# av-savchenko/HSE_FaceRec_tf

Measured on AMD Instinct MI355X. Metric: faces/sec embedding-extract (MobileNet-192, bs=256), higher is better.
Workload: dtype f32

## Files before the change

### hse_facerec_tf_amd/_lib.py

```python
from __future__ import annotations

import ctypes
import os
from ctypes import POINTER, c_char_p, c_float, c_int, c_longlong, c_size_t, c_void_p

_HERE = os.path.dirname(os.path.abspath(__file__))
LIB_PATH = os.path.join(_HERE, os.environ.get("HSEFR_LIB", "libhsefr.so"))

OK, ERR_INVALID, ERR_UNSUPPORTED, ERR_HIP, ERR_NOMEM, ERR_SHAPE = 0, -1, -2, -3, -4, -5

_lib = None

_fp = c_void_p
SIGNATURES = {
    "hsefr_version": (c_int, []),
    "hsefr_last_error_string": (c_char_p, []),
    "hsefr_engine_set_graph_batch": (c_int, [c_void_p, c_int]),
    "hsefr_engine_graph_launches": (c_longlong, [c_void_p]),
    "hsefr_engine_create": (c_int, [c_void_p, c_size_t, c_int, POINTER(c_void_p)]),
    "hsefr_plan_validate": (c_int, [c_void_p, c_size_t]),
    "hsefr_plan_describe": (c_int, [c_void_p, c_size_t, c_int, c_char_p, c_size_t]),
    "hsefr_engine_workspace_bytes": (c_size_t, [c_void_p]),
    "hsefr_engine_max_batch": (c_int, [c_void_p]),
    "hsefr_engine_forward": (c_int, [c_void_p, _fp, c_int, _fp, _fp, _fp, c_void_p]),
    "hsefr_engine_buffer": (c_void_p, [c_void_p, c_int]),
    "hsefr_engine_copy_buffer": (c_int, [c_void_p, c_int, _fp, c_size_t, c_void_p]),
    "hsefr_engine_set_profiling": (c_int, [c_void_p, c_int]),
    "hsefr_engine_profiled_calls": (c_longlong, [c_void_p]),
    "hsefr_engine_op_times_ms": (c_int, [c_void_p, c_int, POINTER(c_float), c_int]),
    "hsefr_engine_destroy": (c_int, [c_void_p]),
    "hsefr_conv_c3_bias_act": (c_int, [_fp, _fp, _fp, _fp] + [c_int] * 12 + [c_void_p]),
    "hsefr_dwconv3x3_bn_relu6": (c_int, [_fp, _fp, _fp, _fp, _fp] + [c_int] * 10 + [c_void_p]),
    "hsefr_dwconv3x3_bn_relu6_split": (c_int, [_fp, _fp, _fp, _fp, _fp] + [c_int] * 11 + [c_void_p]),
    "hsefr_pwconv1x1_presplit_gap": (c_int, [_fp, c_void_p, _fp, _fp, _fp, c_longlong, c_int, c_int, c_int, c_int, c_void_p]),
    "hsefr_pwconv1x1_presplit_dw": (c_int, [_fp, c_void_p, _fp, _fp, _fp, _fp, c_longlong] + [c_int] * 7 + [c_void_p]),
    "hsefr_pwconv1x1_presplit": (c_int, [_fp, c_void_p, _fp, _fp, _fp, c_longlong, c_int, c_int, c_int, c_void_p]),
    "hsefr_pwconv1x1_bias_relu6": (c_int, [_fp, _fp, _fp, _fp, c_longlong, c_int, c_int, c_int, c_void_p]),
    "hsefr_stem2_fused": (c_int, [_fp] * 6 + [c_void_p] + [_fp] * 6 + [c_int] * 13 + [c_void_p]),
    "hsefr_stem3_fused": (c_int, [_fp, c_void_p] + [_fp] * 5 + [c_void_p] + [_fp] * 7 + [c_int] * 14 + [c_void_p]),
    "hsefr_stem4_fused": (c_int, [_fp, c_int, c_void_p] + [_fp] * 5 + [c_void_p] + [_fp] * 7 + [c_int] * 6 + [c_void_p]),
    "hsefr_stem5_stream": (c_int, [_fp, c_int, c_void_p] + [_fp] * 5 + [c_void_p] + [_fp] * 7 + [c_int] * 6 + [c_void_p]),
    "hsefr_engine_accepts_u8": (c_int, [c_void_p]),
    "hsefr_engine_forward_u8": (c_int, [c_void_p, _fp, c_int, _fp, _fp, _fp, c_void_p]),
    "hsefr_engine_input_overflow": (c_int, [c_void_p, POINTER(c_int), c_void_p]),
    "hsefr_engine_input_overflow_async": (c_int, [c_void_p, POINTER(c_int), c_void_p]),
    "hsefr_dwpw_f16split": (c_int, [_fp, _fp, _fp, _fp, c_void_p, _fp, _fp, _fp] + [c_int] * 12 + [c_void_p]),
    "hsefr_pwconv1x1_f16split": (c_int, [_fp, c_void_p, _fp, _fp, _fp, c_longlong, c_int, c_int, c_int, c_int, c_void_p]),
    "hsefr_dwpw_fused": (c_int, [_fp] * 7 + [c_int] * 10 + [c_void_p]),
    "hsefr_gap": (c_int, [_fp, _fp, c_int, c_int, c_int, c_void_p]),
    "hsefr_dense": (c_int, [_fp, _fp, _fp, _fp, c_int, c_int, c_int, c_int, c_void_p]),
    "hsefr_softmax": (c_int, [_fp, _fp, c_int, c_int, c_void_p]),
    "hsefr_heads_fused": (c_int, [_fp] * 11 + [c_int] * 3 + [c_void_p]),
    "hsefr_conv_bf16": (c_int, [_fp, _fp, _fp, _fp, _fp, _fp] + [c_int] * 13 + [c_void_p]),
    "hsefr_conv1x1_proj_bf16": (c_int, [_fp] * 9 + [c_int] * 10 + [c_void_p]),
    "hsefr_conv1x1_sres_bf16": (c_int, [_fp] * 6 + [c_int] * 9 + [c_void_p]),
    "hsefr_conv1x1_pair_bf16": (c_int, [_fp] * 14 + [c_longlong] + [c_int] * 6 + [c_void_p]),
    "hsefr_conv1x1_pair_sub2_bf16": (c_int, [_fp] * 14 + [c_int] * 9 + [c_void_p]),
    "hsefr_stem7x7_bf16": (c_int, [_fp, _fp, _fp, _fp, _fp] + [c_int] * 6 + [c_void_p]),
    "hsefr_stem7x7_pool_bf16": (c_int, [_fp, c_void_p, _fp, _fp, c_void_p] + [c_int] * 7 + [c_void_p]),
    "hsefr_maxpool3x3s2_bf16": (c_int, [_fp, _fp] + [c_int] * 8 + [c_void_p]),
    "hsefr_gap_bf16": (c_int, [_fp, _fp, c_int, c_int, c_int, c_void_p]),
    "hsefr_preprocess_pil_u8": (c_int, [_fp, _fp, _fp] + [c_int] * 5 + [_fp, _fp, _fp, c_int, _fp, _fp, _fp, c_int, c_int,
                                        POINTER(ctypes.c_double), c_void_p]),
    "hsefr_preprocess_cv_u8": (c_int, [_fp, _fp] + [c_int] * 5 + [_fp] * 6 + [c_int, POINTER(ctypes.c_double), c_void_p]),
    "hsefr_l2_normalize": (c_int, [_fp, _fp, c_int, c_int, c_void_p]),
    "hsefr_conv2d_direct": (c_int, [_fp] * 5 + [c_int] * 12 + [c_void_p]),
    "hsefr_conv2d_f32": (c_int, [_fp] * 6 + [c_int] * 13 + [c_void_p]),
    "hsefr_conv2d_f32_mfma": (c_int, [_fp] * 6 + [c_int] * 13 + [c_void_p]),
    "hsefr_maxpool_f32": (c_int, [_fp, _fp] + [c_int] * 10 + [c_void_p]),
    "hsefr_mtcnn_pyramid_level": (c_int, [_fp, _fp, c_int, c_int, c_int, c_int, c_void_p]),
    "hsefr_mtcnn_post_capacity": (c_int, []),
    "hsefr_mtcnn_stage1_level": (c_int, [_fp, _fp, c_int, c_int, ctypes.c_double, ctypes.c_float, _fp, _fp, c_void_p]),
    "hsefr_mtcnn_stage1_finish": (c_int, [_fp, _fp, _fp, _fp, c_int, c_int, c_void_p]),
    "hsefr_mtcnn_stage_finish": (c_int, [c_int, _fp, c_int, _fp, _fp, _fp, ctypes.c_float, _fp, _fp, _fp, _fp, c_int, c_int, c_void_p]),
    "hsefr_mtcnn_nms": (c_int, [_fp, c_int, ctypes.c_double, c_int, _fp, _fp, c_void_p]),
    "hsefr_mtcnn_crops": (c_int, [_fp, _fp, _fp, c_int, c_int, c_int, c_int, c_void_p]),
    "hsefr_pairwise_dist": (c_int, [_fp, _fp, c_int, c_int, c_int, _fp, c_void_p]),
    "hsefr_single_linkage": (c_int, [_fp, c_int, c_int, _fp, _fp, _fp, _fp, _fp, _fp, c_void_p]),
    "hsefr_hier_linkage": (c_int, [_fp, c_int, c_int, _fp, _fp, _fp, c_int, _fp, _fp, _fp, _fp, c_void_p]),
    "hsefr_dbscan": (c_int, [_fp, c_int, c_int, _fp, _fp, _fp, ctypes.c_double, c_int, _fp, _fp, c_void_p]),
    "hsefr_rank_order": (c_int, [_fp, c_int, c_int, _fp, _fp, _fp, ctypes.c_double, ctypes.c_double, _fp, POINTER(c_int), c_void_p]),
    "hsefr_rank_order_sweep": (c_int, [_fp, c_int, c_int, _fp, _fp, _fp, POINTER(ctypes.c_double), c_int, _fp, POINTER(c_int), c_void_p]),
    "hsefr_nn1": (c_int, [_fp, _fp, c_int, c_int, c_int, _fp, _fp, c_void_p]),
    "hsefr_knn": (c_int, [_fp, _fp, c_int, c_int, c_int, c_int, _fp, _fp, _fp, _fp, c_void_p]),
    "hsefr_nn1_fallbacks": (c_longlong, []),
}

DEV_SIGNATURES = {
    "hsefr_debug_set": (c_int, [c_char_p, c_int]),
    "hsefr_debug_read_stamps": (c_int, [c_int, c_void_p, ctypes.c_size_t]),
    "hsefr_debug_clock_probe": (c_int, [_fp, c_int, c_int, c_void_p]),
    "hsefr_debug_copy": (c_int, [_fp, _fp, c_size_t, c_void_p]),
    "hsefr_stem_fused": (c_int, [_fp] * 6 + [c_void_p, _fp, _fp, _fp] + [c_int] * 9 + [c_void_p]),
}


class HsefrError(RuntimeError):
    pass

# ... 93 lines not shown
```

### hse_facerec_tf_amd/csrc/common.h

```cpp
#pragma once
#include <hip/hip_runtime.h>
#include <stdarg.h>
#include <stdio.h>

#include "../../include/hsefr.h"
#ifdef HSEFR_DEV
#include "hsefr_dev.h"
#endif

namespace hsefr {

void set_error(const char* fmt, ...);

#define HSEFR_HIP_CHECK(expr)                                                          \
    do {                                                                               \
        hipError_t _e = (expr);                                                        \
        if (_e != hipSuccess) {                                                        \
            ::hsefr::set_error("%s failed: %s (%s:%d)", #expr, hipGetErrorString(_e),  \
                               __FILE__, __LINE__);                                    \
            return HSEFR_ERR_HIP;                                                      \
        }                                                                              \
    } while (0)

#define HSEFR_REQUIRE(cond, code, ...)     \
// ... 190 lines not shown
                             int ph, int pw, int pool_pad_t, int pool_pad_l, hipStream_t s, const void* wfrag = nullptr);
bool stem7s_stream_supported(long long n, int h, int w, int ph, int pw);
int launch_stem7s_stream(const float* x, const void* wt, const float* scale, const float* shift, void* y, int n, int h, int w, int ph, int pw,
                         int pool_pad_t, int pool_pad_l, hipStream_t s, const void* wfrag = nullptr);
constexpr size_t STEM7S_WFRAG_BYTES = 4 * 7 * 64 * 16;
int stem7s_reorder_weights(const void* wt, void* wfrag, hipStream_t s);
int launch_maxpool3x3s2_bf16(const void* x, void* y, int n, int h, int w, int c, int oh, int ow, int pad_t, int pad_l,
                             hipStream_t s);
int launch_gap_bf16(const void* x, float* y, int n, int hw, int c, hipStream_t s);

int launch_pil_resize(const unsigned char* in, unsigned char* tmp, float* out, int n, int H, int W, int oh, int ow, const int* xmin,
                      const int* xcnt, const int* xcoef, int xk, const int* ymin, const int* ycnt, const int* ycoef, int yk,
                      int mode, const double* mean, hipStream_t s);
int launch_cv_resize(const unsigned char* in, float* out, int n, int H, int W, int oh, int ow, const int* x0, const int* x1,
                     const int* wx1, const int* y0, const int* y1, const int* wy1, int mode, const double* mean, hipStream_t s);

int launch_area_level(const unsigned char* src, float* dst, int sh, int sw, int dh, int dw, hipStream_t s);
int launch_area_crops(const unsigned char* src, const int* boxes, float* dst, int sh, int sw, int n, int size, hipStream_t s);
int launch_pairwise_dist(const float* x, const float* y, int n, int m, int d, float* out, hipStream_t s);
struct DistSource {
    const float* x;
    int n, d;
    const float* born;
    const float* year;
    const double* dense;
};
int launch_single_linkage(const DistSource& src, int* edge_a, int* edge_b, double* edge_h, hipStream_t s);
int launch_dbscan(const DistSource& src, double eps, int min_samples, int* labels, unsigned char* core, hipStream_t s);
int launch_rank_order(const DistSource& src, const double* thresholds, int pairs, int* labels, int* iterations, hipStream_t s);
int launch_hier_linkage(const DistSource& src, int method, int* merge_a, int* merge_b, double* merge_h, int* merge_round, hipStream_t s);

bool dwpw_fused_supported(int c, int cout, int stride, int act_dw, int act_pw);
int launch_dwpw_fused(const float* x, const float* wd, const float* dscale, const float* dshift, const float* wp_t,
                      const float* pshift, float* y, int n, int h, int w, int c, int stride, int pad_t, int pad_l, int oh,
                      int ow, int cout, int act_dw, int act_pw, hipStream_t s);

int launch_conv2d_direct(const float* x, const float* w, const float* bias, const float* alpha, float* y, int n, int h, int wd, int c,
                         int oh, int ow, int cout, int kh, int kw, int stride, int pad_t, int pad_l, hipStream_t s);
int launch_conv_f32_mfma(const float* x, const float* w, const float* scale, const float* shift, const float* res, float* y, int n, int h,
                         int wd, int c, int oh, int ow, int cout, int kh, int kw, int stride, int pad_t, int pad_l, int act, hipStream_t s,
                         int res_stride = 0, int res_h = 0, int res_w = 0);
bool conv_f32_mfma_supported(int c, int cout);
int launch_conv2d_f32(const float* x, const float* w, const float* scale, const float* shift, const float* res, float* y, int n, int h,
                      int wd, int c, int oh, int ow, int cout, int kh, int kw, int stride, int pad_t, int pad_l, int act, hipStream_t s);
int launch_maxpool_f32(const float* x, float* y, int n, int h, int w, int c, int oh, int ow, int k, int stride, int pad_t, int pad_l,
                       hipStream_t s);

int launch_dwpw_f16s(const float* x, const float* wd, const float* dscale, const float* dshift, const void* wsplit,
                     const float* descale, const float* pshift, float* y, int n, int h, int w, int c, int stride, int pad_t,
                     int pad_l, int oh, int ow, int cout, int a_log2, int act, hipStream_t s);
bool dwpw_f16s_supported(int c, int cout, int stride);
bool dwpw_s2_covered(int c, int cout, int stride);
bool dwpw_s2_off();
int launch_stem_fused(const float* x, const float* cw, const float* cshift, const float* wd, const float* dscale,
                      const float* dshift, const void* wsplit, const float* descale, const float* pshift, float* y, int n,
                      int h, int w, int cpad_t, int cpad_l, int oh, int ow, int a_log2, int act, hipStream_t s);
int launch_stem2_fused(const float* x, const float* cw, const float* cshift, const float* wd1, const float* d1scale,
                       const float* d1shift, const void* wsplit, const float* descale, const float* pshift, const float* wd2,
                       const float* d2scale, const float* d2shift, float* y, int n, int h, int w, int cpad_t, int cpad_l,
                       int h1, int w1, int pad_t2, int pad_l2, int oh2, int ow2, int a_log2, int act, hipStream_t s);
int launch_stem3_fused(const float* x, const void* cw_split, const float* cdescale, const float* cshift, const float* wd1,
                       const float* d1scale, const float* d1shift, const void* wsplit, const float* descale, const float* pshift,
                       const float* wd2, const float* d2scale, const float* d2shift, float* y, int* overflow, int n, int h, int w,
                       int cpad_t, int cpad_l, int h1, int w1, int pad_t2, int pad_l2, int oh2, int ow2, int in_log2, int a_log2,
                       int act, hipStream_t s);
bool stem3_fused_supported(int cin, int c1, int c2, int conv_stride, int dw1_stride, int dw2_stride, int kh, int kw);
int launch_stem4_fused(const void* x, int x_is_u8, const void* cw4, const float* cdescale, const float* cshift, const float* wd1,
                       const float* d1scale, const float* d1shift, const void* wsplit, const float* descale, const float* pshift,
                       const float* wd2, const float* d2scale, const float* d2shift, float* y, int* overflow, int n, int h, int w,
                       int in_log2, int a_log2, int act, hipStream_t s);
bool stem4_fused_supported(int cin, int c1, int c2, int conv_stride, int dw1_stride, int dw2_stride, int kh, int kw, int h, int w);
int launch_stem5_stream(const void* x, int x_is_u8, const void* cw4, const float* cdescale, const float* cshift, const float* wd1,
                        const float* d1scale, const float* d1shift, const void* wsplit, const float* descale, const float* pshift,
                        const float* wd2, const float* d2scale, const float* d2shift, float* y, int* overflow, int n, int h, int w,
                        int in_log2, int a_log2, int act, hipStream_t s);
bool stem5_stream_supported(int cin, int c1, int c2, int conv_stride, int dw1_stride, int dw2_stride, int kh, int kw, int h, int w);
bool stem2_fused_supported(int cin, int c1, int c2, int conv_stride, int dw1_stride, int dw2_stride, int kh, int kw);
bool stem_fused_supported(int cin, int cmid, int cout, int conv_stride, int dw_stride, int kh, int kw);
int read_pws_stamps(void* host_out, size_t bytes);
int read_stem_stamps(void* host_out, size_t bytes);
#ifdef HSEFR_STEM_STAMPS
unsigned long long* stamp_buffer(hipStream_t s);
#define STEM_STAMP(i) do { const unsigned long long _t = __builtin_amdgcn_s_memtime(); st[i] += _t - tprev; tprev = _t; } while (0)
#define STEM_STAMP_DECL unsigned long long st[8] = {0, 0, 0, 0, 0, 0, 0, 0}; unsigned long long tprev = __builtin_amdgcn_s_memtime(); \
    const unsigned long long tstart = tprev; unsigned npatch = 0
#define STEM_STAMP_COUNT ++npatch
#define STEM_STAMP_FLUSH(buf, lane, wave) do { if ((lane) == 0 && (buf) && blockIdx.x < 512) { unsigned long long* o = (buf) + (blockIdx.x * 4 + (wave)) * 10; \
    for (int i_ = 0; i_ < 8; ++i_) o[i_] = st[i_]; o[8] = __builtin_amdgcn_s_memtime() - tstart; o[9] = npatch; } } while (0)
#else
#define STEM_STAMP(i) do { } while (0)
#define STEM_STAMP_DECL do { } while (0)
#define STEM_STAMP_COUNT do { } while (0)
#define STEM_STAMP_FLUSH(buf, lane, wave) do { } while (0)
#endif
#ifdef HSEFR_DEV
void set_stem4_grid(int v);
void set_stem5_grid(int v);
void set_stem5_segs(int v);
void set_c11(int v);
void set_c11_tile(int v);
void set_c11_bres(int v);
void set_c11_adv(int v);
int read_c11_stamps(void* host_out, size_t bytes);
void set_dwpw_s2_off(int v);
void set_dwpws_tw(int v);
void set_dwpws_bn(int v);
void set_pw_tile(int v);
void set_pws_tile(int v);
void set_ps_mb(int v);
void set_ps_grid(int v);
void set_psdw_mode(int v);
void set_cd_rb(int v);
void set_w3_off(int v);
void set_w2_off(int v);
void set_w4_off(int v);
void set_w4_bres(int v);
void set_pair_off(int v);
void set_stem7s(int v);
void set_pair_ablate(int v);
void set_pair_nt(int v);
void set_nn1_y_mb(int v);
int read_w4_stamps(void* host_out, size_t bytes);
int read_s7_stamps(void* host_out, size_t bytes);
int read_w2_stamps(void* host_out, size_t bytes);
int read_w3_stamps(void* host_out, size_t bytes);
int read_cd_stamps(void* host_out, size_t bytes);
void set_cd_off(int v);
int read_ps_stamps(void* host_out, size_t bytes);
void set_pw_ablate(int v);
void set_pw_dma(int v);
void set_dw_th(int v);
void set_dw_variant(int v);
void set_dw_look(int v);
void set_dw_look2(int v);
void set_copy_variant(int v);
void set_clock_mode(int v);
void set_c3_impl(int v);
int launch_clock_probe(unsigned long long* out, int blocks, int iters, hipStream_t s);
int launch_copy(const void* src, void* dst, size_t bytes, hipStream_t s);
#endif

}
```

### hse_facerec_tf_amd/csrc/dwpw_f16s.hip

```cpp
#include <type_traits>

#include "common.h"

namespace hsefr {

namespace {

typedef float f32x4 __attribute__((ext_vector_type(4)));
typedef float f32x16 __attribute__((ext_vector_type(16)));
typedef _Float16 f16x4 __attribute__((ext_vector_type(4)));
typedef _Float16 f16x8 __attribute__((ext_vector_type(8)));

struct DwPwSParams {
    const float4* x;
    const float4* wd;
    const float4* dscale;
    const float4* dshift;
    const float* wsplit;
    const float* descale;
    const float* pshift;
    float* y;
    int H, W, C4, KT, OH, OW, Cout, pad_t, pad_l, tiles_w, tiles_h, tiles_n;
    unsigned total;
    float a_scale;
    int reverse;
    int nimg;
    unsigned m_n, m_w, m_h;
    unsigned long long* stamps;
};

constexpr int ROWB = 128;
__device__ __forceinline__ int swzb(int row, int chunk) { return row * ROWB + 16 * (chunk ^ ((row >> 1) & 7) ^ ((row & 1) << 2)); }
__device__ __forceinline__ float4 fma4(float4 a, float4 b, float4 c) {
    return make_float4(fmaf(a.x, b.x, c.x), fmaf(a.y, b.y, c.y), fmaf(a.z, b.z, c.z), fmaf(a.w, b.w, c.w));
}
__device__ __forceinline__ float relu6(float v) { return fminf(fmaxf(v, 0.f), 6.f); }
__device__ __forceinline__ unsigned fastdiv(unsigned x, unsigned m) { return m ? __umulhi(x, m) : x; }

template <int STRIDE, int TW, int BN, int OCC, int ACT>
__global__ __launch_bounds__(256, OCC) void dwpw_f16s_kernel(DwPwSParams p) {
    constexpr int TH = 128 / TW;
    constexpr int U = TW * 8;
    constexpr int RG = 256 / U;
    constexpr int RPT = TH / RG;
    static_assert(RPT == 4, "patch shapes 8x16 and 16x8");
    constexpr int WN = BN / 2, NI = WN / 32, BP = BN / 32;
    __shared__ __attribute__((aligned(16))) unsigned char As[128 * ROWB];
    __shared__ __attribute__((aligned(16))) unsigned char Bs[BN * ROWB];

    const int tid = threadIdx.x;
    const int lane = tid & 63, wave = tid >> 6;
    const int wm = wave >> 1, wn = wave & 1;
    const int li = lane & 31, lh = lane >> 5;
    const int srow = tid >> 3, skq = tid & 7;
    const int u = tid % U, tw = u >> 3, c4l = u & 7;
    const int row0 = (tid / U) * RPT;
    const int arow = wm * 64 + li, brow = wn * WN + li;

    for (unsigned t = blockIdx.x; t < p.total; t += gridDim.x) {
        const unsigned lt = xcd_remap_dir(t, p.total, p.reverse);
        const int n0 = (lt % p.tiles_n) * BN;
        const unsigned pt = lt / p.tiles_n;
        const int ow0 = (pt % p.tiles_w) * TW;
        const int oh0 = ((pt / p.tiles_w) % p.tiles_h) * TH;
        const int n = pt / (p.tiles_w * p.tiles_h);

        const int ow = min(ow0 + tw, p.OW - 1);
        const int iw0 = ow * STRIDE - p.pad_l;
        const float ml = iw0 >= 0 ? 1.f : 0.f, mm = (iw0 + 1 >= 0 && iw0 + 1 < p.W) ? 1.f : 0.f, mr = iw0 + 2 < p.W ? 1.f : 0.f;
        const int cl = max(iw0, 0) * p.C4, cm = min(max(iw0 + 1, 0), p.W - 1) * p.C4, cr = min(iw0 + 2, p.W - 1) * p.C4;
        const float4* ximg = p.x + (size_t)n * p.H * p.W * p.C4;
        const int ih0 = (oh0 + row0) * STRIDE - p.pad_t;
        const float* bsrc = p.wsplit + (size_t)(n0 + srow) * p.KT * 32 + 4 * skq;

        f32x16 acc[2][NI];
#pragma unroll
        for (int mi = 0; mi < 2; ++mi)
#pragma unroll
            for (int ni = 0; ni < NI; ++ni)
#pragma unroll
                for (int r = 0; r < 16; ++r) acc[mi][ni][r] = 0.f;
// ... 71 lines not shown
                f16x8 ah[2], al[2], bh[NI], bl[NI];
#pragma unroll
                for (int mi = 0; mi < 2; ++mi) {
                    ah[mi] = *(const f16x8*)(&As[swzb(arow + mi * 32, 2 * s + lh)]);
                    al[mi] = *(const f16x8*)(&As[swzb(arow + mi * 32, 4 + 2 * s + lh)]);
                }
#pragma unroll
                for (int ni = 0; ni < NI; ++ni) {
                    bh[ni] = *(const f16x8*)(&Bs[swzb(brow + ni * 32, 2 * s + lh)]);
                    bl[ni] = *(const f16x8*)(&Bs[swzb(brow + ni * 32, 4 + 2 * s + lh)]);
                }
#pragma unroll
                for (int mi = 0; mi < 2; ++mi)
#pragma unroll
                    for (int ni = 0; ni < NI; ++ni) {
                        acc[mi][ni] = __builtin_amdgcn_mfma_f32_32x32x16_f16(al[mi], bh[ni], acc[mi][ni], 0, 0, 0);
                        acc[mi][ni] = __builtin_amdgcn_mfma_f32_32x32x16_f16(ah[mi], bl[ni], acc[mi][ni], 0, 0, 0);
                        acc[mi][ni] = __builtin_amdgcn_mfma_f32_32x32x16_f16(ah[mi], bh[ni], acc[mi][ni], 0, 0, 0);
                    }
            }
        }
        const bool full = oh0 + TH <= p.OH && ow0 + TW <= p.OW;
        float* ybase = p.y + ((size_t)n * p.OH * p.OW) * p.Cout;
#pragma unroll
        for (int ni = 0; ni < NI; ++ni) {
            const int col = n0 + wn * WN + ni * 32 + li;
            const float ds = p.descale[col], sh = p.pshift[col];
#pragma unroll
            for (int mi = 0; mi < 2; ++mi) {
                const int Rb = wm * 64 + mi * 32 + 4 * lh;
                if (full) {
#pragma unroll
                    for (int r = 0; r < 16; ++r) {
                        const int R = Rb + (r & 3) + 8 * (r >> 2);
                        ybase[((size_t)(oh0 + R / TW) * p.OW + ow0 + (R % TW)) * p.Cout + col] = apply_act<ACT>(fmaf(acc[mi][ni][r], ds, sh));
                    }
                } else {
#pragma unroll
                    for (int r = 0; r < 16; ++r) {
                        const int R = Rb + (r & 3) + 8 * (r >> 2);
                        const int oh = oh0 + R / TW, owc = ow0 + (R % TW);
                        if (oh < p.OH && owc < p.OW)
                            ybase[((size_t)oh * p.OW + owc) * p.Cout + col] = apply_act<ACT>(fmaf(acc[mi][ni][r], ds, sh));
                    }
                }
            }
        }
    }
}

constexpr int HALO_B = 192 * 128;
constexpr int CMAX2 = 512;

template <int TW, int BN, int HS, int ACT>
__global__ __launch_bounds__(256 + 64 * (BN == 256 ? 8 : 4), BN == 256 ? 1 : 2) void dwpw3_f16s_kernel(DwPwSParams p) {
    constexpr int NCW = BN == 256 ? 8 : 4;
    constexpr int CWN = NCW / 2;
    constexpr int NTHR = 256 + 64 * NCW;
    constexpr int TH = 128 / TW, HC = TW + 2;
    constexpr int WCAP = 256;
    constexpr int B_ST = BN * ROWB;
    constexpr int B_OFF = HS * HALO_B, A_OFF = B_OFF + 2 * B_ST, W_OFF = A_OFF + 2 * 128 * ROWB, E_OFF = W_OFF + 11 * WCAP * 4;
    constexpr int WN = BN / CWN, NI = WN / 32;
    constexpr int BPW = BN / 8 / NCW;
    static_assert(BPW == 4 && NI == 2, "a consumer's slice of the weight stage is its 4 KB epilogue scratch");
    constexpr bool HALO_BY_CONSUMER = false;
    constexpr int HPW = 24 / (HALO_BY_CONSUMER ? NCW : 4);
    static_assert(E_OFF + 2 * CMAX2 * 4 <= 160 * 1024, "LDS budget");
    __shared__ __attribute__((aligned(1024))) unsigned char smem[E_OFF + 2 * CMAX2 * 4];

    const int tid = threadIdx.x;
    const int lane = tid & 63;
    const int wave = __builtin_amdgcn_readfirstlane(tid >> 6);
    const int C = p.C4 * 4, KT = p.KT;
    {
        float4* wl = (float4*)(smem + W_OFF);
        for (int i = tid; i < 9 * p.C4; i += NTHR) wl[i] = p.wd[i];
        for (int i = tid; i < p.C4; i += NTHR) { wl[9 * p.C4 + i] = p.dscale[i]; wl[10 * p.C4 + i] = p.dshift[i]; }
        float* el = (float*)(smem + E_OFF);
        for (int i = tid; i < p.Cout; i += NTHR) { el[i] = p.descale[i]; el[CMAX2 + i] = p.pshift[i]; }
    }
    const __amdgpu_buffer_rsrc_t rx = make_rsrc(p.x, (long long)p.nimg * p.H * p.W * C * 4);
    const __amdgpu_buffer_rsrc_t rw = make_rsrc(p.wsplit, (long long)p.Cout * C * 4);
    const __amdgpu_buffer_rsrc_t ry = make_rsrc(p.y, (long long)p.nimg * p.OH * p.OW * p.Cout * 4);
    const unsigned OOB = 0xFFFFFFF0u;
    const unsigned nitem = (p.total - blockIdx.x + gridDim.x - 1) / gridDim.x;
    const int nsteps = (int)(nitem * KT);
    struct Item { int n, oh0, ow0, n0; };
    auto decode = [&](unsigned i) {
        const unsigned lt = xcd_remap_dir(blockIdx.x + (i < nitem ? i : nitem - 1) * gridDim.x, p.total, p.reverse);
        Item it;
        const unsigned pt = fastdiv(lt, p.m_n);
        it.n0 = (lt - pt * p.tiles_n) * BN;
        const unsigned pr = fastdiv(pt, p.m_w);
        it.ow0 = (pt - pr * p.tiles_w) * TW;
        it.n = fastdiv(pr, p.m_h);
        it.oh0 = (pr - it.n * p.tiles_h) * TH;
        return it;
    };
    const unsigned lds0 = (unsigned)(unsigned long long)(__attribute__((address_space(3))) unsigned char*)smem;
    auto piece = [&](const __amdgpu_buffer_rsrc_t& r, unsigned lds_addr, unsigned voff, unsigned soff) {
        asm volatile("s_mov_b32 m0, %0\n\ts_nop 0\n\tbuffer_load_dwordx4 %1, %2, %3 offen lds" ::"s"(__builtin_amdgcn_readfirstlane(lds_addr)), "v"(voff),
                     "s"(r), "s"(__builtin_amdgcn_readfirstlane(soff))
                     : "memory", "m0");
    };
    const int hw = HALO_BY_CONSUMER ? wave - 4 : wave & 3;
    unsigned hv[HPW];
    unsigned pf_i = 0;
    int pf_kc = 0, pf_step = 0;
    auto setup_halo = [&](unsigned i) {
        const Item it = decode(i);
#pragma unroll
        for (int j = 0; j < HPW; ++j) {
            const int q = (hw * HPW + j) * 8 + (lane >> 3);
            const int hr = q / HC, hc = q - hr * HC;
            const int ih = it.oh0 - p.pad_t + hr, iw = it.ow0 - p.pad_l + hc;
            const bool ok = q < (TH + 2) * HC && ih >= 0 && ih < p.H && iw >= 0 && iw < p.W;
            hv[j] = ok ? ((unsigned)((it.n * p.H + ih) * p.W + iw) * (unsigned)C + 4u * (lane & 7)) * 4u : OOB;
        }
    };
    auto halo_dma = [&]() {
        const unsigned base = lds0 + (pf_step % HS) * HALO_B;
        const unsigned so = (unsigned)pf_kc * 128u;
#pragma unroll
        for (int j = 0; j < HPW; ++j) piece(rx, base + (hw * HPW + j) * 1024, hv[j], so);
        ++pf_step;
        if (++pf_kc == KT) {
            pf_kc = 0;
            setup_halo(++pf_i);
        }
    };
    STEM_STAMP_DECL;

    if (wave < 4) {
        const int quad = tid & 7, col = (tid >> 3) % TW, r0 = 4 * (tid / (8 * TW));
        const unsigned char* hsrc0 = smem + ((r0 * HC + col) * 128 + quad * 16);
        if (!HALO_BY_CONSUMER) {
            setup_halo(0);
#pragma unroll
            for (int i = 0; i < HS - 1; ++i)
                if (i < nsteps) halo_dma();
        }
        asm volatile("s_waitcnt vmcnt(0)" ::: "memory");
        __syncthreads();
        int dkc = 0;
        for (int g = -1; g < nsteps; ++g) {
            const bool issued = !HALO_BY_CONSUMER && pf_step < nsteps;
            if (issued) halo_dma();
            STEM_STAMP(1);
            if (g + 1 < nsteps) {
                const f32x4* wl = (const f32x4*)(smem + W_OFF) + dkc * 8 + quad;
                f32x4 wk[9];
#pragma unroll
                for (int i = 0; i < 9; ++i) wk[i] = wl[i * p.C4];
                const f32x4 dsc = wl[9 * p.C4], dsh = wl[10 * p.C4];
                const unsigned char* hs = hsrc0 + ((g + 1) % HS) * HALO_B;
                unsigned char* At = smem + A_OFF + ((g + 1) & 1) * (128 * ROWB);
                f32x4 h[6][3];
#pragma unroll
                for (int a = 0; a < 6; ++a)
#pragma unroll
                    for (int b = 0; b < 3; ++b) h[a][b] = *(const f32x4*)(hs + (a * HC + b) * 128);
                auto row_sum = [&](int a, int b) {
                    f32x4 t = h[a][0] * wk[b];
                    t = __builtin_elementwise_fma(h[a][1], wk[b + 1], t);
                    return __builtin_elementwise_fma(h[a][2], wk[b + 2], t);
                };
#pragma unroll
                for (int j = 0; j < 4; ++j) {
                    const f32x4 sa = row_sum(j, 0), sb = row_sum(j + 1, 3), sc = row_sum(j + 2, 6);
                    const f32x4 sacc = (sa + sb) + sc;
                    const f32x4 o = __builtin_elementwise_fma(sacc, dsc, dsh);
                    f32x4 v;
#pragma unroll
                    for (int e = 0; e < 4; ++e) v[e] = relu6(o[e]);
                    v = v * p.a_scale;
                    const f16x4 hi = __builtin_convertvector(v, f16x4);
                    const f16x4 lo = __builtin_convertvector(v - __builtin_convertvector(hi, f32x4), f16x4);
                    const int R = (r0 + j) * TW + col;
                    *(f16x4*)(At + swzb(R, quad >> 1) + 8 * (quad & 1)) = hi;
                    *(f16x4*)(At + swzb(R, 4 + (quad >> 1)) + 8 * (quad & 1)) = lo;
                }
                if (++dkc == KT) { dkc = 0; STEM_STAMP_COUNT; }
            }
            STEM_STAMP(2);
            if (HS >= 3 && issued) asm volatile("s_waitcnt vmcnt(%0)" ::"n"(HPW) : "memory");
            else asm volatile("s_waitcnt vmcnt(0)" ::: "memory");
            STEM_STAMP(0);
            __syncthreads();
            STEM_STAMP(3);
        }
        STEM_STAMP_FLUSH(p.stamps, lane, wave);
    } else {
        const int cw = wave - 4, wm = cw / CWN, wn = cw % CWN;
        const int li = lane & 31, lh = lane >> 5;
        const int arow = wm * 64 + li, brow = wn * WN + li;
        const int erow = lane >> 3, ech = lane & 7;
        unsigned bv[BPW];
        unsigned pb_i = 0;
        int pb_kc = 0, pb_step = 0;
        auto setup_b = [&](unsigned i) {
            const Item it = decode(i);
#pragma unroll
            for (int j = 0; j < BPW; ++j) {
                const int r = (cw * BPW + j) * 8 + (lane >> 3);
                bv[j] = ((unsigned)(it.n0 + r) * (unsigned)C + 4u * ((lane & 7) ^ ((r >> 1) & 7) ^ ((r & 1) << 2))) * 4u;
            }
        };
        auto b_dma = [&]() {
            const unsigned base = lds0 + B_OFF + (pb_step & 1) * B_ST;
            const unsigned so = (unsigned)pb_kc * 128u;
#pragma unroll
            for (int j = 0; j < BPW; ++j) piece(rw, base + (cw * BPW + j) * 1024, bv[j], so);
            ++pb_step;
            if (++pb_kc == KT) {
                pb_kc = 0;
                setup_b(++pb_i);
            }
        };
        f32x16 acc[2][NI];
        auto zero_acc = [&]() {
#pragma unroll
            for (int mi = 0; mi < 2; ++mi)
#pragma unroll
                for (int ni = 0; ni < NI; ++ni)
#pragma unroll
                    for (int r = 0; r < 16; ++r) acc[mi][ni][r] = 0.f;
        };
        auto epilogue = [&](const Item& cur, int stage) {
            unsigned char* scr = smem + B_OFF + stage * B_ST + cw * (BPW * 1024);
            const float* el = (const float*)(smem + E_OFF);
            unsigned sv[2][4];
#pragma unroll
            for (int mi = 0; mi < 2; ++mi)
#pragma unroll
                for (int i = 0; i < 4; ++i) {
                    const int R = wm * 64 + mi * 32 + erow + 8 * i;
                    const int oh = cur.oh0 + R / TW, ow = cur.ow0 + R % TW;
                    sv[mi][i] = (oh < p.OH && ow < p.OW)
                                    ? ((unsigned)((cur.n * p.OH + oh) * p.OW + ow) * (unsigned)p.Cout + (unsigned)(cur.n0 + wn * WN + 4 * ech)) * 4u
                                    : OOB;
                }
#pragma unroll
            for (int ni = 0; ni < NI; ++ni) {
                const int nl = cur.n0 + wn * WN + ni * 32 + 4 * ech;
                const f32x4 ds = *(const f32x4*)(el + nl), sh = *(const f32x4*)(el + CMAX2 + nl);
// ... 44 lines not shown
                zero_acc();
                cur = decode(++ci);
                pending = false;
                STEM_STAMP_COUNT;
            }
            STEM_STAMP(5);
            if (pb_step < nsteps) b_dma();
            const bool halo_issued = HALO_BY_CONSUMER && pf_step < nsteps;
            if (halo_issued) halo_dma();
            STEM_STAMP(1);
            if (g >= 0) {
                const unsigned char* As = smem + A_OFF + (g & 1) * (128 * ROWB);
                const unsigned char* Bs = smem + B_OFF + (g & 1) * B_ST;
#pragma unroll
                for (int s = 0; s < 2; ++s) {
                    f16x8 ah[2], al[2], bh[NI], bl[NI];
#pragma unroll
                    for (int mi = 0; mi < 2; ++mi) {
                        ah[mi] = *(const f16x8*)(As + swzb(arow + mi * 32, 2 * s + lh));
                        al[mi] = *(const f16x8*)(As + swzb(arow + mi * 32, 4 + 2 * s + lh));
                    }
#pragma unroll
                    for (int ni = 0; ni < NI; ++ni) {
                        bh[ni] = *(const f16x8*)(Bs + swzb(brow + ni * 32, 2 * s + lh));
                        bl[ni] = *(const f16x8*)(Bs + swzb(brow + ni * 32, 4 + 2 * s + lh));
                    }
#pragma unroll
                    for (int mi = 0; mi < 2; ++mi)
#pragma unroll
                        for (int ni = 0; ni < NI; ++ni) {
                            acc[mi][ni] = __builtin_amdgcn_mfma_f32_32x32x16_f16(bh[ni], al[mi], acc[mi][ni], 0, 0, 0);
                            acc[mi][ni] = __builtin_amdgcn_mfma_f32_32x32x16_f16(bl[ni], ah[mi], acc[mi][ni], 0, 0, 0);
                            acc[mi][ni] = __builtin_amdgcn_mfma_f32_32x32x16_f16(bh[ni], ah[mi], acc[mi][ni], 0, 0, 0);
                        }
                }
                if (++ckc == KT) { ckc = 0; pending = true; }
            }
            STEM_STAMP(4);
            if (HS >= 3 && halo_issued) asm volatile("s_waitcnt vmcnt(%0)" ::"n"(HPW) : "memory");
            else asm volatile("s_waitcnt vmcnt(0)" ::: "memory");
            STEM_STAMP(0);
            __syncthreads();
            STEM_STAMP(3);
        }
        if (pending) { epilogue(cur, (nsteps - 1) & 1); STEM_STAMP_COUNT; }
#ifdef HSEFR_STEM_STAMPS
        if (lane == 0 && p.stamps && blockIdx.x < 256 && cw < 4) {
            unsigned long long* o = p.stamps + ((blockIdx.x + 256) * 4 + cw) * 10;
            for (int i_ = 0; i_ < 8; ++i_) o[i_] = st[i_];
            o[8] = __builtin_amdgcn_s_memtime() - tstart;
            o[9] = npatch;
        }
#endif
    }
}

constexpr unsigned S2_GRID = 256;
constexpr int S2_C = 128, S2_COUT = 256, S2_KT = S2_C / 32, S2_T = 8, S2_M = S2_T * S2_T;
constexpr int S2_B_ST = S2_COUT * ROWB;
constexpr int S2_A_ST = S2_M * ROWB;
constexpr int S2_SCR = 16 * ROWB;
constexpr int S2_A_OFF = S2_KT * S2_B_ST, S2_S_OFF = S2_A_OFF + 2 * S2_A_ST, S2_W_OFF = S2_S_OFF + 4 * S2_SCR;
constexpr int S2_E_OFF = S2_W_OFF + 11 * S2_C * 4, S2_LDS = S2_E_OFF + 2 * S2_COUT * 4;
static_assert(S2_LDS <= 160 * 1024, "LDS budget");

template <int ACT>
__global__ __launch_bounds__(512, 1) void dwpws2_f16s_kernel(DwPwSParams p) {
    __shared__ __attribute__((aligned(1024))) unsigned char smem[S2_LDS];
    const int tid = threadIdx.x;
    const int lane = tid & 63;
    const int wave = __builtin_amdgcn_readfirstlane(tid >> 6);
    const __amdgpu_buffer_rsrc_t rx = make_rsrc(p.x, (long long)p.nimg * p.H * p.W * S2_C * 4);
    const __amdgpu_buffer_rsrc_t rw = make_rsrc(p.wsplit, (long long)S2_COUT * S2_C * 4);
    const __amdgpu_buffer_rsrc_t ry = make_rsrc(p.y, (long long)p.nimg * p.OH * p.OW * S2_COUT * 4);
    const unsigned OOB = 0xFFFFFFF0u;
    {
        const unsigned lds0 = (unsigned)(unsigned long long)(__attribute__((address_space(3))) unsigned char*)smem;
#pragma unroll
        for (int j = 0; j < 16; ++j) {
            const int pc = wave * 16 + j;
            const int r = (pc & 31) * 8 + (lane >> 3);
            const unsigned v = ((unsigned)r * (unsigned)S2_C + 4u * ((lane & 7) ^ ((r >> 1) & 7) ^ ((r & 1) << 2))) * 4u;
            asm volatile("s_mov_b32 m0, %0\n\ts_nop 0\n\tbuffer_load_dwordx4 %1, %2, %3 offen lds" ::"s"(__builtin_amdgcn_readfirstlane(lds0 + pc * 1024)),
                         "v"(v), "s"(rw), "s"(__builtin_amdgcn_readfirstlane((unsigned)(pc >> 5) * 128u))
                         : "memory", "m0");
        }
        float4* wl = (float4*)(smem + S2_W_OFF);
        for (int i = tid; i < 11 * (S2_C / 4); i += 512)
            wl[i] = i < 9 * (S2_C / 4) ? p.wd[i] : (i < 10 * (S2_C / 4) ? p.dscale[i - 9 * (S2_C / 4)] : p.dshift[i - 10 * (S2_C / 4)]);
        float* el = (float*)(smem + S2_E_OFF);
        for (int i = tid; i < S2_COUT; i += 512) { el[i] = p.descale[i]; el[S2_COUT + i] = p.pshift[i]; }
        asm volatile("s_waitcnt vmcnt(0)" ::: "memory");
    }
    const unsigned nitem = (p.total - blockIdx.x + gridDim.x - 1) / gridDim.x;
    const int nsteps = (int)(nitem * S2_KT);
    struct Item { int n, oh0, ow0; };
    auto decode = [&](unsigned i) {
        const unsigned lt = xcd_remap_dir(blockIdx.x + (i < nitem ? i : nitem - 1) * gridDim.x, p.total, p.reverse);
        Item it;
        const unsigned pr = fastdiv(lt, p.m_w);
        it.ow0 = (lt - pr * p.tiles_w) * S2_T;
        it.n = fastdiv(pr, p.m_h);
        it.oh0 = (pr - it.n * p.tiles_h) * S2_T;
        return it;
    };
    typedef std::integral_constant<int, 0> S0;
    typedef std::integral_constant<int, 1> S1;
// ... 144 lines not shown
                            const f32x4 z = __builtin_elementwise_fma(rv[i], ds, sh);
                            f32x4 o;
#pragma unroll
                            for (int e = 0; e < 4; ++e) o[e] = apply_act<ACT>(z[e]);
                            bstore16_welded(o, ry, sv[mi][hb][i], __builtin_amdgcn_readfirstlane((unsigned)(ni * 32) * 4u));
                        }
                    }
            }
        };
        zero_acc();
        Item cur = decode(0);
        unsigned ci = 0;
        int ckc = 0;
        bool pending = false;
        for (int g = 0; g < nsteps; ++g) {
            if (pending) {
                epilogue(cur);
                zero_acc();
                cur = decode(++ci);
                pending = false;
            }
            __syncthreads();
            const unsigned char* As = smem + S2_A_OFF + (g & 1) * S2_A_ST;
            const unsigned char* Bs = smem + ckc * S2_B_ST;
#pragma unroll
            for (int s = 0; s < 2; ++s) {
                f16x8 ah[2], al[2], bh[2], bl[2];
#pragma unroll
                for (int mi = 0; mi < 2; ++mi) {
                    ah[mi] = *(const f16x8*)(As + swzb(li + mi * 32, 2 * s + lh));
                    al[mi] = *(const f16x8*)(As + swzb(li + mi * 32, 4 + 2 * s + lh));
                }
#pragma unroll
                for (int ni = 0; ni < 2; ++ni) {
                    bh[ni] = *(const f16x8*)(Bs + swzb(brow + ni * 32, 2 * s + lh));
                    bl[ni] = *(const f16x8*)(Bs + swzb(brow + ni * 32, 4 + 2 * s + lh));
                }
#pragma unroll
                for (int mi = 0; mi < 2; ++mi)
#pragma unroll
                    for (int ni = 0; ni < 2; ++ni) {
                        acc[mi][ni] = __builtin_amdgcn_mfma_f32_32x32x16_f16(bh[ni], al[mi], acc[mi][ni], 0, 0, 0);
                        acc[mi][ni] = __builtin_amdgcn_mfma_f32_32x32x16_f16(bl[ni], ah[mi], acc[mi][ni], 0, 0, 0);
                        acc[mi][ni] = __builtin_amdgcn_mfma_f32_32x32x16_f16(bh[ni], ah[mi], acc[mi][ni], 0, 0, 0);
                    }
            }
            if (++ckc == S2_KT) { ckc = 0; pending = true; }
        }
        epilogue(cur);
    }
}

HSEFR_KNOB(g_s2_off, 0);
HSEFR_KNOB(g_tw, 0);
HSEFR_KNOB(g_bn, 0);

template <int STRIDE, int TW, int BN, int OCC>
int launch_t(DwPwSParams& p, int n, int act, hipStream_t s) {
    constexpr int TH = 128 / TW;
    p.tiles_w = (p.OW + TW - 1) / TW;
    p.tiles_h = (p.OH + TH - 1) / TH;
    p.tiles_n = p.Cout / BN;
    const long long total = (long long)n * p.tiles_w * p.tiles_h * p.tiles_n;
    HSEFR_REQUIRE(total < (1ll << 31), HSEFR_ERR_UNSUPPORTED, "dwpw_f16split: grid too large");
    p.total = (unsigned)total;
    const unsigned cap = 256u * OCC;
    const unsigned g = p.total < cap ? p.total : cap;
#define HSEFR_DWPWS(A) HSEFR_LAUNCH((dwpw_f16s_kernel<STRIDE, TW, BN, OCC, A>), dim3(g), dim3(256), 0, s, p)
    if (act == HSEFR_ACT_RELU6) HSEFR_DWPWS(HSEFR_ACT_RELU6);
    else if (act == HSEFR_ACT_RELU) HSEFR_DWPWS(HSEFR_ACT_RELU);
    else if (act == HSEFR_ACT_NONE) HSEFR_DWPWS(HSEFR_ACT_NONE);
    else { set_error("dwpw_f16split: act %d", act); return HSEFR_ERR_UNSUPPORTED; }
#undef HSEFR_DWPWS
    return launch_status("dwpw_f16split");
}

template <int STRIDE, int TW>
int launch_bn(DwPwSParams& p, int n, int bn, int act, hipStream_t s) {
    if (bn == 64) return launch_t<STRIDE, TW, 64, 2>(p, n, act, s);
#ifdef HSEFR_DEV
    if (bn == 256) return launch_t<STRIDE, TW, 256, 2>(p, n, act, s);
#endif
    return launch_t<STRIDE, TW, 128, 2>(p, n, act, s);
}

template <int TW, int BN, int HS>
int launch_v3(DwPwSParams& p, int n, int act, hipStream_t s) {
    constexpr int TH = 128 / TW;
    p.tiles_w = (p.OW + TW - 1) / TW;
    p.tiles_h = (p.OH + TH - 1) / TH;
    p.tiles_n = p.Cout / BN;
    const long long total = (long long)n * p.tiles_w * p.tiles_h * p.tiles_n;
    HSEFR_REQUIRE(total < (1ll << 31) / 16, HSEFR_ERR_UNSUPPORTED, "dwpw_f16split: grid too large");
    p.total = (unsigned)total;
    auto magic = [](unsigned d) { return d == 1 ? 0u : (unsigned)((0x100000000ull + d - 1) / d); };
    p.m_n = magic(p.tiles_n); p.m_w = magic(p.tiles_w); p.m_h = magic(p.tiles_h);
    HSEFR_REQUIRE(total * (long long)(p.tiles_n > p.tiles_w ? (p.tiles_n > p.tiles_h ? p.tiles_n : p.tiles_h) : (p.tiles_w > p.tiles_h ? p.tiles_w : p.tiles_h)) < (1ll << 32),
                  HSEFR_ERR_UNSUPPORTED, "dwpw_f16split: grid too large for the quotient multipliers");
    const unsigned g = p.total < 256u ? p.total : 256u;
#define HSEFR_DWPW3(A) HSEFR_LAUNCH((dwpw3_f16s_kernel<TW, BN, HS, A>), dim3(g), dim3(256 + 64 * (BN == 256 ? 8 : 4)), 0, s, p)
    if (act == HSEFR_ACT_RELU6) HSEFR_DWPW3(HSEFR_ACT_RELU6);
    else if (act == HSEFR_ACT_RELU) HSEFR_DWPW3(HSEFR_ACT_RELU);
    else if (act == HSEFR_ACT_NONE) HSEFR_DWPW3(HSEFR_ACT_NONE);
    else { set_error("dwpw_f16split: act %d", act); return HSEFR_ERR_UNSUPPORTED; }
#undef HSEFR_DWPW3
    return launch_status("dwpw_f16split");
}

int launch_s2(DwPwSParams& p, int n, int act, hipStream_t s) {
    p.tiles_w = (p.OW + S2_T - 1) / S2_T;
    p.tiles_h = (p.OH + S2_T - 1) / S2_T;
    p.tiles_n = 1;
    const long long total = (long long)n * p.tiles_w * p.tiles_h;
    HSEFR_REQUIRE(total < (1ll << 31) / 16, HSEFR_ERR_UNSUPPORTED, "dwpw_f16split: grid too large");
    p.total = (unsigned)total;
    auto magic = [](unsigned d) { return d == 1 ? 0u : (unsigned)((0x100000000ull + d - 1) / d); };
    p.m_n = 0; p.m_w = magic(p.tiles_w); p.m_h = magic(p.tiles_h);
    HSEFR_REQUIRE(total * (long long)(p.tiles_w > p.tiles_h ? p.tiles_w : p.tiles_h) < (1ll << 32), HSEFR_ERR_UNSUPPORTED,
                  "dwpw_f16split: grid too large for the quotient multipliers");
    const unsigned g = p.total < S2_GRID ? p.total : S2_GRID;
#define HSEFR_DWPWS2(A) HSEFR_LAUNCH((dwpws2_f16s_kernel<A>), dim3(g), dim3(512), 0, s, p)
    if (act == HSEFR_ACT_RELU6) HSEFR_DWPWS2(HSEFR_ACT_RELU6);
    else if (act == HSEFR_ACT_RELU) HSEFR_DWPWS2(HSEFR_ACT_RELU);
    else if (act == HSEFR_ACT_NONE) HSEFR_DWPWS2(HSEFR_ACT_NONE);
    else { set_error("dwpw_f16split: act %d", act); return HSEFR_ERR_UNSUPPORTED; }
#undef HSEFR_DWPWS2
    return launch_status("dwpw_f16split");
}

}

#ifdef HSEFR_DEV
void set_dwpw_s2_off(int v) { g_s2_off = v; }
void set_dwpws_tw(int v) { g_tw = v; }
void set_dwpws_bn(int v) { g_bn = v; }
#endif

bool dwpw_s2_off() { return g_s2_off != 0; }

bool dwpw_s2_covered(int c, int cout, int stride) { return stride == 2 && c == S2_C && cout == S2_COUT; }

bool dwpw_f16s_supported(int c, int cout, int stride) {
    return c > 0 && c % 32 == 0 && cout > 0 && cout % 64 == 0 && (stride == 1 || stride == 2);
}

int launch_dwpw_f16s(const float* x, const float* wd, const float* dscale, const float* dshift, const void* wsplit,
                     const float* descale, const float* pshift, float* y, int n, int h, int w, int c, int stride, int pad_t,
                     int pad_l, int oh, int ow, int cout, int a_log2, int act, hipStream_t s) {
    HSEFR_REQUIRE(dwpw_f16s_supported(c, cout, stride), HSEFR_ERR_UNSUPPORTED,
                  "dwpw_f16split: c=%d cout=%d stride=%d not covered (c %% 32, cout %% 64, stride 1|2)", c, cout, stride);
    HSEFR_REQUIRE(n >= 0 && h > 0 && w > 0 && oh > 0 && ow > 0, HSEFR_ERR_INVALID, "dwpw_f16split: bad shape");
    HSEFR_REQUIRE(a_log2 > 0 && a_log2 <= 12, HSEFR_ERR_INVALID, "dwpw_f16split: a_log2=%d (the depthwise result is in [0,6]: 1..12)", a_log2);
    if (n == 0) return HSEFR_OK;
    DwPwSParams p;
    p.x = (const float4*)x; p.wd = (const float4*)wd; p.dscale = (const float4*)dscale; p.dshift = (const float4*)dshift;
    p.wsplit = (const float*)wsplit; p.descale = descale; p.pshift = pshift; p.y = y;
    p.H = h; p.W = w; p.C4 = c / 4; p.KT = c / 32; p.OH = oh; p.OW = ow; p.Cout = cout; p.pad_t = pad_t; p.pad_l = pad_l;
    p.a_scale = ldexpf(1.f, a_log2);
    p.reverse = sweep_reverse();
    p.nimg = n;
    p.stamps = nullptr;
#ifdef HSEFR_STEM_STAMPS
    p.stamps = stamp_buffer(s);
#endif
    const long long in_bytes = (long long)n * h * w * c * 4, out_bytes = (long long)n * oh * ow * cout * 4;
    if (stride == 1 && c <= 256 && cout <= CMAX2 && cout % 128 == 0 && in_bytes < (1ll << 32) - 16 && out_bytes < (1ll << 32) - 16) {
        auto padded = [&](int tw) { const int th = 128 / tw; return (long long)((ow + tw - 1) / tw * tw) * ((oh + th - 1) / th * th); };
        int tw = padded(16) <= padded(8) ? 16 : 8;
        if (g_tw == 8 || g_tw == 16) tw = g_tw;
        int bn = cout % 256 == 0 ? 256 : 128;
        if ((g_bn == 128 || g_bn == 256) && cout % g_bn == 0) bn = g_bn;
        if (bn == 256) return tw == 16 ? launch_v3<16, 256, 2>(p, n, act, s) : launch_v3<8, 256, 2>(p, n, act, s);
        return tw == 16 ? launch_v3<16, 128, 3>(p, n, act, s) : launch_v3<8, 128, 3>(p, n, act, s);
    }
    if (dwpw_s2_covered(c, cout, stride) && !g_s2_off && in_bytes < (1ll << 32) - 16 && out_bytes < (1ll << 32) - 16)
        return launch_s2(p, n, act, s);
    int bn = cout % 128 == 0 ? 128 : 64;
    if (g_bn && cout % g_bn == 0) bn = g_bn;
    int tw = (ow % 16 == 0 || ow % 8 != 0) ? 16 : 8;
    if (ow <= 8) tw = 8;
    if (g_tw == 8 || g_tw == 16) tw = g_tw;
    if (stride == 1) return tw == 16 ? launch_bn<1, 16>(p, n, bn, act, s) : launch_bn<1, 8>(p, n, bn, act, s);
    return tw == 16 ? launch_bn<2, 16>(p, n, bn, act, s) : launch_bn<2, 8>(p, n, bn, act, s);
}

}
```

### hse_facerec_tf_amd/csrc/engine.hip

```cpp
#include <math.h>
#include <string.h>

#include <cxxabi.h>
#include <dlfcn.h>
#include <elf.h>

#include <map>
#include <new>
#include <string>
#include <vector>

#include "common.h"

namespace hsefr {

static thread_local char g_err[512] = "";

void set_error(const char* fmt, ...) {
    va_list ap;
    va_start(ap, fmt);
    vsnprintf(g_err, sizeof(g_err), fmt, ap);
    va_end(ap);
}

// ... 212 lines not shown
                HSEFR_REQUIRE(o.w_off != HSEFR_NO_OFFSET && o.scale_off != HSEFR_NO_OFFSET && o.shift_off != HSEFR_NO_OFFSET &&
                                  o.aux > 0 && o.aux <= 24,
                              HSEFR_ERR_INVALID, "plan op %u: split-f16 pointwise needs split rows, descale, shift and a_log2 in (0, 24]", i);
                break;
            case HSEFR_OP_STEM3_F16S: {
                const StemAux a = stem_aux(o.aux);
                HSEFR_REQUIRE(stem3_fused_supported(o.cin, 32, o.cout, o.stride, 1, 2, o.kh, stem_kw(o.kw).k) && a.a_log2 > 0 && a.a_log2 <= 12 &&
                                  a.in_log2 >= -8 && a.in_log2 <= 14 &&
                                  o.w_off != HSEFR_NO_OFFSET && o.w2_off != HSEFR_NO_OFFSET && o.shift2_off != HSEFR_NO_OFFSET &&
                                  o.w_off + HSEFR_STEM_PACK_STEM3_END * 4 <= h.blob_bytes && o.w2_off + 64 * 128 <= h.blob_bytes &&
                                  o.shift2_off + 128 * 4 <= h.blob_bytes && o.in_buf == HSEFR_BUF_INPUT,
                              HSEFR_ERR_UNSUPPORTED, "plan op %u: bounded fused stem cin=%d cout=%d stride=%d not covered", i, o.cin, o.cout, o.stride);
                break;
            }
            case HSEFR_OP_STEM2_F16S:
                HSEFR_REQUIRE(stem2_fused_supported(o.cin, 32, o.cout, o.stride, 1, 2, o.kh, stem_kw(o.kw).k) && o.aux > 0 && o.aux <= 12 &&
                                  o.w_off != HSEFR_NO_OFFSET && o.w2_off != HSEFR_NO_OFFSET && o.shift2_off != HSEFR_NO_OFFSET &&
                                  o.w_off + HSEFR_STEM_PACK_STEM2_END * 4 <= h.blob_bytes && o.in_buf == HSEFR_BUF_INPUT,
                              HSEFR_ERR_UNSUPPORTED, "plan op %u: fused stem+dw2 cin=%d cout=%d stride=%d not covered", i, o.cin, o.cout, o.stride);
                break;
            case HSEFR_OP_STEM_F16S:
#ifndef HSEFR_DEV
                set_error("plan op %u: HSEFR_OP_STEM_F16S (round 1's fused stem) runs on development builds of the library only", i);
                return HSEFR_ERR_UNSUPPORTED;
#else
                HSEFR_REQUIRE(stem_fused_supported(o.cin, 32, o.cout, o.stride, 1, o.kh, o.kw) && o.aux > 0 && o.aux <= 12 &&
                                  o.w_off != HSEFR_NO_OFFSET && o.w2_off != HSEFR_NO_OFFSET && o.shift2_off != HSEFR_NO_OFFSET &&
                                  o.w_off + HSEFR_STEM_PACK_DW2 * 4 <= h.blob_bytes && o.in_buf == HSEFR_BUF_INPUT,
                              HSEFR_ERR_UNSUPPORTED, "plan op %u: fused stem cin=%d cout=%d stride=%d not covered", i, o.cin, o.cout, o.stride);
                break;
#endif
            case HSEFR_OP_DWPW_F16S:
                if (!need(o.w_off, 9 * ci * 4, "depthwise kernel") || !need(o.scale_off, ci * 4, "scale") || !need(o.shift_off, ci * 4, "shift") ||
                    !need(o.w2_off, ci * co * 4, "split rows") || !need(o.shift2_off, 2 * co * 4, "descale | shift"))
                    return HSEFR_ERR_INVALID;
                HSEFR_REQUIRE(dwpw_f16s_supported(o.cin, o.cout, o.stride) && o.aux > 0 && o.aux <= 12 &&
                                  o.w_off != HSEFR_NO_OFFSET && o.scale_off != HSEFR_NO_OFFSET && o.shift_off != HSEFR_NO_OFFSET &&
                                  o.w2_off != HSEFR_NO_OFFSET && o.shift2_off != HSEFR_NO_OFFSET,
                              HSEFR_ERR_UNSUPPORTED, "plan op %u: split-f16 fused block cin=%d cout=%d stride=%d a_log2=%d not covered",
                              i, o.cin, o.cout, o.stride, o.aux);
                break;
            case HSEFR_OP_DWPW_F32:
                if (!need(o.w_off, 9 * ci * 4, "depthwise kernel") || !need(o.scale_off, ci * 4, "scale") || !need(o.shift_off, ci * 4, "shift") ||
                    !need(o.w2_off, ci * co * 4, "pointwise kernel") || !need(o.shift2_off, co * 4, "pointwise shift"))
                    return HSEFR_ERR_INVALID;
                HSEFR_REQUIRE(dwpw_fused_supported(o.cin, o.cout, o.stride, HSEFR_ACT_RELU6, (int)o.act), HSEFR_ERR_UNSUPPORTED,
                              "plan op %u: fused depthwise-pointwise block cin=%d cout=%d not covered", i, o.cin, o.cout);
                break;
            default:
                set_error("plan op %u: unknown kind %u", i, o.kind);
                return HSEFR_ERR_UNSUPPORTED;
        }
    }
    for (uint32_t i = 0; i < h.n_ops; ++i) {
        const hsefr_plan_op& o = ops[i];
        HSEFR_REQUIRE((o.flags & ~(HSEFR_OPF_PAIR_NEXT | HSEFR_OPF_HEADS | HSEFR_OPF_OUT_SUB2 | HSEFR_OPF_DWPW_NEXT)) == 0, HSEFR_ERR_INVALID,
                      "plan op %u: unknown flags 0x%x", i, o.flags);
        HSEFR_REQUIRE(!(o.flags & HSEFR_OPF_OUT_SUB2) || (o.flags & HSEFR_OPF_PAIR_NEXT), HSEFR_ERR_INVALID, "plan op %u: OUT_SUB2 without PAIR_NEXT", i);
        if (o.flags & HSEFR_OPF_PAIR_NEXT) {
            HSEFR_REQUIRE(i + 1 < h.n_ops, HSEFR_ERR_INVALID, "plan op %u: PAIR_NEXT on the last op", i);
            const hsefr_plan_op& b = ops[i + 1];
            const bool proj = o.w2_off != HSEFR_NO_OFFSET;
            const Geometry g = geometry(o.aux);
            const int c2 = proj ? g.c2 : 0;
            const bool sub2 = (o.flags & HSEFR_OPF_OUT_SUB2) != 0;
            HSEFR_REQUIRE(o.kind == HSEFR_OP_CONV_BF16 && b.kind == HSEFR_OP_CONV_BF16 && o.kh == 1 && o.kw == 1 && o.stride == 1 && o.pad_t == 0 &&
                              o.pad_l == 0 && (sub2 ? (o.oh == (o.h + 1) / 2 && o.ow == (o.w + 1) / 2 && o.h > 1 && o.w > 1) : (o.oh == o.h && o.ow == o.w)) &&
                              b.kh == 1 && b.kw == 1 && b.stride == 1 && b.pad_t == 0 && b.pad_l == 0 &&
                              b.h == o.h && b.w == o.w && b.oh == b.h && b.ow == b.w && b.cin == o.cout && b.in_buf == o.out_buf &&
                              b.res_buf == HSEFR_BUF_NONE && b.w2_off == HSEFR_NO_OFFSET && b.flags == 0 && o.res_buf >= 0 &&
                              (!proj || (g.stride2 == 1 && g.h2 == o.h && g.w2 == o.w)),
                          HSEFR_ERR_INVALID, "plan op %u: PAIR_NEXT needs two 1x1 stride-1 bf16 convolutions at the same pixels, the first with a residual "
                          "or a same-pixel projected shortcut, the second reading the first", i);
            HSEFR_REQUIRE(b.out_buf != o.in_buf && b.out_buf != o.res_buf && b.out_buf != o.out_buf, HSEFR_ERR_INVALID,
                          "plan op %u: PAIR_NEXT: the second output (buffer %d) aliases an operand of the first", i, b.out_buf);
            HSEFR_REQUIRE(conv1x1_pair_bf16_shape_supported(o.cin, o.cout, b.cout, c2), HSEFR_ERR_UNSUPPORTED,
                          "plan op %u: PAIR_NEXT %d -> %d -> %d (projection from %d) not covered", i, o.cin, o.cout, b.cout, c2);
        }
        if (o.flags & HSEFR_OPF_DWPW_NEXT) {
            HSEFR_REQUIRE(o.flags == HSEFR_OPF_DWPW_NEXT && i + 1 < h.n_ops, HSEFR_ERR_INVALID, "plan op %u: DWPW_NEXT on the last op or beside another flag", i);
            const hsefr_plan_op& b = ops[i + 1];
            HSEFR_REQUIRE(o.kind == HSEFR_OP_DWCONV3X3 && o.stride == 2 && o.act == HSEFR_ACT_RELU6 && o.aux == 0 && o.cout == o.cin &&
                              b.kind == HSEFR_OP_PWCONV_F16S && b.in_buf == o.out_buf && b.flags == 0 && b.h == o.oh && b.w == o.ow && b.oh == b.h &&
                              b.ow == b.w && b.cin == o.cin && b.aux > 0 && b.aux <= 12,
                          HSEFR_ERR_INVALID, "plan op %u: DWPW_NEXT needs a stride-2 depthwise 3x3 with ReLU6 and fp32 output, and behind it a split-f16 "
                          "pointwise op without flags that reads it at the same pixels (a_log2 in [1, 12])", i);
            HSEFR_REQUIRE(dwpw_s2_covered(o.cin, b.cout, o.stride), HSEFR_ERR_INVALID, "plan op %u: DWPW_NEXT %d -> %d channels not covered (128 -> 256)", i,
                          o.cin, b.cout);
            HSEFR_REQUIRE(b.out_buf != o.out_buf, HSEFR_ERR_INVALID, "plan op %u: DWPW_NEXT: the second output (buffer %d) aliases the depthwise tensor", i,
                          b.out_buf);
            HSEFR_REQUIRE(b.out_buf != o.in_buf || (uint64_t)bufs[o.in_buf].elems_per_image * bufs[o.in_buf].elem_bytes ==
                                                       (uint64_t)bufs[o.out_buf].elems_per_image * bufs[o.out_buf].elem_bytes,
                          HSEFR_ERR_INVALID, "plan op %u: DWPW_NEXT: buffers %d and %d exchange roles and must have one size", i, o.in_buf, o.out_buf);
            for (uint32_t k = i + 2; k < h.n_ops; ++k) {
                HSEFR_REQUIRE(ops[k].in_buf != o.out_buf && ops[k].res_buf != o.out_buf, HSEFR_ERR_INVALID,
                              "plan op %u: DWPW_NEXT: op %u also reads the depthwise tensor (buffer %d)", i, k, o.out_buf);
                if (ops[k].out_buf == o.out_buf) break;
            }
            for (int sl = 0; sl < HSEFR_N_OUTPUT_SLOTS; ++sl)
                HSEFR_REQUIRE(h.out_buffer[sl] != o.out_buf && (b.out_buf != o.in_buf || h.out_buffer[sl] != o.in_buf), HSEFR_ERR_INVALID,
                              "plan op %u: DWPW_NEXT: the depthwise tensor (or the buffer it exchanges roles with) is output slot %d", i, sl);
        }
        if (o.flags & HSEFR_OPF_HEADS) {
            HSEFR_REQUIRE(i + 3 < h.n_ops, HSEFR_ERR_INVALID, "plan op %u: HEADS needs three ops behind it", i);
            const hsefr_plan_op &a = ops[i + 1], &sm = ops[i + 2], &g = ops[i + 3];
            HSEFR_REQUIRE(o.kind == HSEFR_OP_DENSE && o.act == HSEFR_ACT_RELU && o.cout == 256 && o.cin > 0 && o.cin % 256 == 0 && o.cin <= 2048 &&
                              o.shift_off != HSEFR_NO_OFFSET && a.kind == HSEFR_OP_DENSE && a.act == HSEFR_ACT_NONE && a.cin == 256 && a.cout >= 1 &&
                              a.cout <= 128 && a.in_buf == o.out_buf && a.shift_off != HSEFR_NO_OFFSET && sm.kind == HSEFR_OP_SOFTMAX &&
                              sm.in_buf == a.out_buf && sm.cout == a.cout && g.kind == HSEFR_OP_DENSE && g.act == HSEFR_ACT_SIGMOID && g.cin == 256 &&
                              g.cout == 1 && g.in_buf == o.out_buf && g.shift_off != HSEFR_NO_OFFSET && a.flags == 0 && sm.flags == 0 && g.flags == 0,
                          HSEFR_ERR_INVALID, "plan op %u: HEADS needs DENSE k -> 256 + ReLU, DENSE 256 -> a (<= 128) + bias, SOFTMAX, DENSE 256 -> 1 + sigmoid", i);
            const int outs[4] = {o.out_buf, a.out_buf, sm.out_buf, g.out_buf};
            for (int x = 0; x < 4; ++x) {
                HSEFR_REQUIRE(outs[x] != o.in_buf, HSEFR_ERR_INVALID, "plan op %u: HEADS: an output aliases the pooled features", i);
                for (int y = x + 1; y < 4; ++y)
                    HSEFR_REQUIRE(outs[x] != outs[y], HSEFR_ERR_INVALID, "plan op %u: HEADS: two of the four tensors share buffer %d", i, outs[x]);
            }
        }
    }
    for (int s = 0; s < HSEFR_N_OUTPUT_SLOTS; ++s) {
        HSEFR_REQUIRE(h.out_buffer[s] == HSEFR_BUF_NONE || (h.out_buffer[s] >= 0 && h.out_buffer[s] < (int)h.n_buffers),
                      HSEFR_ERR_INVALID, "plan: output slot %d names buffer %d", s, h.out_buffer[s]);
        if (h.out_buffer[s] == HSEFR_BUF_NONE) continue;
        const int b = h.out_buffer[s];
        uint32_t producers = 0;
        for (uint32_t i = 0; i < h.n_ops; ++i) producers += (ops[i].out_buf == b);
        HSEFR_REQUIRE(producers == 1, HSEFR_ERR_INVALID, "plan: output slot %d: buffer %d has %u producing ops (must be exactly 1)", s, b,
                      producers);
        HSEFR_REQUIRE((uint64_t)bufs[b].elems_per_image * bufs[b].elem_bytes == (uint64_t)h.out_elems[s] * 4, HSEFR_ERR_INVALID,
                      "plan: output slot %d: buffer %d holds %llu x %u bytes per image, the slot declares %u fp32 elements", s, b,
                      (unsigned long long)bufs[b].elems_per_image, (unsigned)bufs[b].elem_bytes, h.out_elems[s]);
    }
    return HSEFR_OK;
}

namespace hsefr {
#ifdef HSEFR_STEM_STAMPS
static unsigned long long* g_stamp_buf = nullptr;
unsigned long long* stamp_buffer(hipStream_t s) {
    if (!g_stamp_buf && hipMalloc((void**)&g_stamp_buf, 512 * 4 * 10 * 8) != hipSuccess) return nullptr;
    (void)hipMemsetAsync(g_stamp_buf, 0, 512 * 4 * 10 * 8, s);
    return g_stamp_buf;
}
int read_stem_stamps(void* host_out, size_t bytes) {
    HSEFR_REQUIRE(g_stamp_buf && bytes <= 512 * 4 * 10 * 8, HSEFR_ERR_INVALID, "read_stem_stamps: nothing recorded / too many bytes");
    HSEFR_HIP_CHECK(hipMemcpy(host_out, g_stamp_buf, bytes, hipMemcpyDeviceToHost));
    return HSEFR_OK;
}
#else
int read_stem_stamps(void* host_out, size_t bytes) {
    (void)host_out; (void)bytes;
    set_error("read_stem_stamps: library built without -DHSEFR_STEM_STAMPS");
    return HSEFR_ERR_UNSUPPORTED;
}
// ... 56 lines not shown
    if (!g_route_sink->empty() && g_route_sink->back() != '\t') *g_route_sink += " + ";
    *g_route_sink += t;
}
static thread_local int g_sweep_reverse = 0;
int sweep_reverse() { return g_sweep_reverse; }
void set_sweep_reverse(int v) { g_sweep_reverse = v; }
}
HSEFR_KNOB(g_sweep_alternate, 1);
HSEFR_KNOB(g_stem5, 1);
HSEFR_KNOB(g_heads_off, 0);
HSEFR_KNOB(g_stem4, 1);

#pragma GCC visibility push(default)
extern "C" {

int hsefr_version(void) { return HSEFR_VERSION; }

const char* hsefr_last_error_string(void) { return g_err; }

#ifdef HSEFR_DEV
int hsefr_debug_set(const char* key, int value) {
    HSEFR_REQUIRE(key, HSEFR_ERR_INVALID, "debug_set: null key");
    if (!strcmp(key, "pw_tile")) { set_pw_tile(value); return HSEFR_OK; }
    if (!strcmp(key, "pws_tile")) { set_pws_tile(value); return HSEFR_OK; }
    if (!strcmp(key, "ps_mb")) { set_ps_mb(value); return HSEFR_OK; }
    if (!strcmp(key, "ps_grid")) { set_ps_grid(value); return HSEFR_OK; }
    if (!strcmp(key, "psdw_mode")) { set_psdw_mode(value); return HSEFR_OK; }
    if (!strcmp(key, "cd_rb")) { set_cd_rb(value); return HSEFR_OK; }
    if (!strcmp(key, "cd_off")) { set_cd_off(value); return HSEFR_OK; }
    if (!strcmp(key, "w3_off")) { set_w3_off(value); return HSEFR_OK; }
    if (!strcmp(key, "w2_off")) { set_w2_off(value); return HSEFR_OK; }
    if (!strcmp(key, "w4_off")) { set_w4_off(value); return HSEFR_OK; }
    if (!strcmp(key, "w4_bres")) { set_w4_bres(value); return HSEFR_OK; }
    if (!strcmp(key, "nn1_y_mb")) { set_nn1_y_mb(value); return HSEFR_OK; }
    if (!strcmp(key, "c11")) { set_c11(value); return HSEFR_OK; }
    if (!strcmp(key, "c11_tile")) { set_c11_tile(value); return HSEFR_OK; }
    if (!strcmp(key, "c11_bres")) { set_c11_bres(value); return HSEFR_OK; }
    if (!strcmp(key, "c11_adv")) { set_c11_adv(value); return HSEFR_OK; }
    if (!strcmp(key, "stem4_grid")) { set_stem4_grid(value); return HSEFR_OK; }
    if (!strcmp(key, "stem4")) { g_stem4 = value; return HSEFR_OK; }
    if (!strcmp(key, "stem5")) { g_stem5 = value; return HSEFR_OK; }
    if (!strcmp(key, "stem5_grid")) { set_stem5_grid(value); return HSEFR_OK; }
    if (!strcmp(key, "stem5_segs")) { set_stem5_segs(value); return HSEFR_OK; }
    if (!strcmp(key, "pair_off")) { set_pair_off(value); return HSEFR_OK; }
    if (!strcmp(key, "stem7s")) { set_stem7s(value); return HSEFR_OK; }
    if (!strcmp(key, "pair_ablate")) { set_pair_ablate(value); return HSEFR_OK; }
    if (!strcmp(key, "pair_nt")) { set_pair_nt(value); return HSEFR_OK; }
    if (!strcmp(key, "heads_off")) { g_heads_off = value; return HSEFR_OK; }
    if (!strcmp(key, "dw_look")) { set_dw_look(value); return HSEFR_OK; }
    if (!strcmp(key, "dw_look2")) { set_dw_look2(value); return HSEFR_OK; }
    if (!strcmp(key, "sweep_alternate")) { g_sweep_alternate = value; return HSEFR_OK; }
    if (!strcmp(key, "clock_mode")) { set_clock_mode(value); return HSEFR_OK; }
    if (!strcmp(key, "dwpw_s2_off")) { set_dwpw_s2_off(value); return HSEFR_OK; }
    if (!strcmp(key, "dwpws_tw")) { set_dwpws_tw(value); return HSEFR_OK; }
    if (!strcmp(key, "dwpws_bn")) { set_dwpws_bn(value); return HSEFR_OK; }
    if (!strcmp(key, "pw_ablate")) { set_pw_ablate(value); return HSEFR_OK; }
    if (!strcmp(key, "pw_dma")) { set_pw_dma(value); return HSEFR_OK; }
    if (!strcmp(key, "dw_th")) { set_dw_th(value); return HSEFR_OK; }
    if (!strcmp(key, "dw_variant")) { set_dw_variant(value); return HSEFR_OK; }
    if (!strcmp(key, "copy_variant")) { set_copy_variant(value); return HSEFR_OK; }
    if (!strcmp(key, "c3_impl")) { set_c3_impl(value); return HSEFR_OK; }
    set_error("debug_set: unknown key %s", key);
    return HSEFR_ERR_INVALID;
}

int hsefr_debug_copy(const void* d_src, void* d_dst, size_t bytes, hsefr_stream_t stream) {
    HSEFR_REQUIRE(bytes == 0 || (d_src && d_dst), HSEFR_ERR_INVALID, "debug_copy: null pointer");
    return launch_copy(d_src, d_dst, bytes, (hipStream_t)stream);
}

int hsefr_debug_read_stamps(int kernel, void* host_out, size_t bytes) {
    switch (kernel) {
        case HSEFR_STAMPS_PWS: return read_pws_stamps(host_out, bytes);
        case HSEFR_STAMPS_STEM: return read_stem_stamps(host_out, bytes);
        case HSEFR_STAMPS_PS: return read_ps_stamps(host_out, bytes);
        case HSEFR_STAMPS_CD: return read_cd_stamps(host_out, bytes);
        case HSEFR_STAMPS_C11: return read_c11_stamps(host_out, bytes);
        case HSEFR_STAMPS_W4: return read_w4_stamps(host_out, bytes);
        case HSEFR_STAMPS_W2: return read_w2_stamps(host_out, bytes);
        case HSEFR_STAMPS_W3: return read_w3_stamps(host_out, bytes);
        case HSEFR_STAMPS_S7: return read_s7_stamps(host_out, bytes);
        default: set_error("debug_read_stamps: unknown kernel id %d", kernel); return HSEFR_ERR_INVALID;
    }
}

int hsefr_debug_clock_probe(unsigned long long* d_out, int blocks, int iters, hsefr_stream_t stream) {
    return launch_clock_probe(d_out, blocks, iters, (hipStream_t)stream);
}
#endif

static int check_plan_blob(const void* plan, size_t plan_bytes, hsefr_plan_header& h, std::vector<hsefr_plan_buffer>& bufs,
                           std::vector<hsefr_plan_op>& ops, const char*& blob) {
    HSEFR_REQUIRE(plan, HSEFR_ERR_INVALID, "plan: null pointer");
    HSEFR_REQUIRE(plan_bytes >= sizeof(hsefr_plan_header), HSEFR_ERR_INVALID, "engine_create: plan too short");
    memcpy(&h, plan, sizeof(h));
    HSEFR_REQUIRE(h.magic == HSEFR_PLAN_MAGIC && h.version == 2, HSEFR_ERR_INVALID, "engine_create: bad plan magic/version");
    const unsigned long long tables = sizeof(h) + (unsigned long long)h.n_buffers * sizeof(hsefr_plan_buffer) +
                                      (unsigned long long)h.n_ops * sizeof(hsefr_plan_op);
    HSEFR_REQUIRE(tables <= plan_bytes && h.blob_bytes == plan_bytes - tables, HSEFR_ERR_INVALID,
                  "engine_create: plan is %zu bytes, header implies %llu + %llu", plan_bytes, tables, (unsigned long long)h.blob_bytes);
    HSEFR_REQUIRE(h.n_buffers > 0 && h.n_ops > 0, HSEFR_ERR_INVALID, "engine_create: plan without %s", h.n_ops ? "buffers" : "ops");
    const char* p = (const char*)plan + sizeof(h);
    try {
        bufs.resize(h.n_buffers);
        ops.resize(h.n_ops);
    } catch (const std::bad_alloc&) {
// ... 63 lines not shown
            set_error("engine_create: hipMalloc(%zu) for activation buffer %u failed", bytes, i);
            return fail(HSEFR_ERR_NOMEM);
        }
        e->device_bytes += bytes;
    }
    *out = e;
    return HSEFR_OK;
}

size_t hsefr_engine_workspace_bytes(const hsefr_engine* e) { return e ? e->device_bytes : 0; }
int hsefr_engine_max_batch(const hsefr_engine* e) { return e ? e->max_batch : 0; }

void* hsefr_engine_buffer(hsefr_engine* e, int buffer) {
    if (!e || buffer < 0 || buffer >= (int)e->d_bufs.size()) return nullptr;
    return e->d_bufs[buffer];
}

int hsefr_engine_copy_buffer(hsefr_engine* e, int buffer, void* d_dst, size_t bytes, hsefr_stream_t stream) {
    HSEFR_REQUIRE(e && d_dst, HSEFR_ERR_INVALID, "copy_buffer: null argument");
    HSEFR_REQUIRE(buffer >= 0 && buffer < (int)e->d_bufs.size(), HSEFR_ERR_INVALID, "copy_buffer: buffer %d", buffer);
    const size_t cap = (size_t)e->bufs[buffer].elems_per_image * e->bufs[buffer].elem_bytes * e->max_batch;
    HSEFR_REQUIRE(bytes <= cap, HSEFR_ERR_SHAPE, "copy_buffer: %zu bytes exceed buffer %d (%zu)", bytes, buffer, cap);
    HSEFR_HIP_CHECK(hipMemcpyAsync(d_dst, e->d_bufs[buffer], bytes, hipMemcpyDeviceToDevice, (hipStream_t)stream));
    return HSEFR_OK;
}

int hsefr_engine_set_profiling(hsefr_engine* e, int depth) {
    HSEFR_REQUIRE(e && depth >= 0, HSEFR_ERR_INVALID, "set_profiling: bad argument");
    for (auto ev : e->events) (void)hipEventDestroy(ev);
    e->events.clear();
    e->prof_depth = 0;
    e->prof_calls = 0;
    if (depth > 0) {
        e->events.resize((size_t)depth * (e->ops.size() + 1));
        for (auto& ev : e->events) HSEFR_HIP_CHECK(hipEventCreate(&ev));
        e->prof_depth = depth;
    }
    return HSEFR_OK;
}

long long hsefr_engine_profiled_calls(const hsefr_engine* e) { return e ? e->prof_calls : 0; }

int hsefr_engine_op_times_ms(hsefr_engine* e, int slot, float* ms, int n_ops) {
    HSEFR_REQUIRE(e && ms, HSEFR_ERR_INVALID, "op_times: null argument");
    HSEFR_REQUIRE(e->prof_depth > 0 && slot >= 0 && slot < e->prof_depth && slot < e->prof_calls, HSEFR_ERR_INVALID,
                  "op_times: slot %d has no profiled forward (depth %d, calls %lld)", slot, e->prof_depth, e->prof_calls);
    HSEFR_REQUIRE(n_ops == (int)e->ops.size(), HSEFR_ERR_INVALID, "op_times: expected %zu ops", e->ops.size());
    hipEvent_t* ev = e->events.data() + (size_t)slot * (e->ops.size() + 1);
    HSEFR_HIP_CHECK(hipEventSynchronize(ev[n_ops]));
    for (int i = 0; i < n_ops; ++i) HSEFR_HIP_CHECK(hipEventElapsedTime(&ms[i], ev[i], ev[i + 1]));
    return HSEFR_OK;
}

static int run_ops(hsefr_engine* e, const std::vector<void*>& tab_in, const void* d_input, int n, const std::vector<char>& needed,
                   hipStream_t s, hipEvent_t* pev, bool input_u8 = false, bool every_tensor = false) {
    std::vector<void*> tab(tab_in);
    const bool prof = pev != nullptr;
    unsigned launches = 0;
    if (prof) HSEFR_HIP_CHECK(hipEventRecord(pev[0], s));
    for (size_t i = 0; i < e->ops.size(); ++i) {
        const hsefr_plan_op& o = e->ops[i];
        if (!needed[i]) {
            if (prof) HSEFR_HIP_CHECK(hipEventRecord(pev[i + 1], s));
            continue;
        }
        const void* in = buf_ptr(tab, o.in_buf, d_input);
        void* out = buf_ptr(tab, o.out_buf, d_input);
        int rc = HSEFR_OK;
        size_t covered = 0;
        set_sweep_reverse(g_sweep_alternate ? (int)(launches++ & 1) : 0);
        const bool sub2 = (o.flags & HSEFR_OPF_OUT_SUB2) != 0;
        const Geometry g = geometry(o.aux);
        const int c2 = o.w2_off != HSEFR_NO_OFFSET ? g.c2 : 0;
        const bool pair_ok = (o.flags & HSEFR_OPF_PAIR_NEXT) && needed[i + 1] &&
                             conv1x1_pair_bf16_supported((long long)n * o.h * o.w, o.cin, o.cout, e->ops[i + 1].cout, c2);
        HSEFR_REQUIRE(!sub2 || pair_ok, HSEFR_ERR_UNSUPPORTED, "forward: op %zu stores its output at every second pixel (OUT_SUB2) and cannot run without the pair launch", i);
        if (pair_ok) {
            const hsefr_plan_op& b = e->ops[i + 1];
            const bool proj = o.w2_off != HSEFR_NO_OFFSET;
            const float* ssp = (const float*)blob_ptr(e, o.shift2_off);
            rc = launch_conv1x1_pair_bf16(in, blob_ptr(e, o.w_off), (const float*)blob_ptr(e, o.scale_off), (const float*)blob_ptr(e, o.shift_off),
                                          proj ? nullptr : tab[o.res_buf], proj ? tab[o.res_buf] : nullptr, proj ? blob_ptr(e, o.w2_off) : nullptr,
                                          proj ? ssp : nullptr, proj ? ssp + o.cout : nullptr, out, blob_ptr(e, b.w_off),
                                          (const float*)blob_ptr(e, b.scale_off), (const float*)blob_ptr(e, b.shift_off), tab[b.out_buf],
                                          (long long)n * o.h * o.w, o.cin, o.cout, b.cout, c2, o.act, b.act, s, sub2 ? 2 : 1, o.h, o.w);
            covered = 1;
        } else if ((o.flags & HSEFR_OPF_HEADS) && !g_heads_off && needed[i + 1] && needed[i + 2] && needed[i + 3]) {
            const hsefr_plan_op &a = e->ops[i + 1], &sm = e->ops[i + 2], &g = e->ops[i + 3];
            rc = launch_heads_fused((const float*)in, (const float*)blob_ptr(e, o.w_off), (const float*)blob_ptr(e, o.shift_off),
                                    (const float*)blob_ptr(e, a.w_off), (const float*)blob_ptr(e, a.shift_off), (const float*)blob_ptr(e, g.w_off),
                                    (const float*)blob_ptr(e, g.shift_off), (float*)out, (float*)tab[a.out_buf], (float*)tab[sm.out_buf],
                                    (float*)tab[g.out_buf], n, o.cin, a.cout, s);
            covered = 3;
        } else if ((o.flags & HSEFR_OPF_DWPW_NEXT) && !every_tensor && !dwpw_s2_off() && needed[i + 1]) {
            const hsefr_plan_op& b = e->ops[i + 1];
            if (b.out_buf == o.in_buf) std::swap(tab[o.in_buf], tab[o.out_buf]);
            rc = launch_dwpw_f16s((const float*)in, (const float*)blob_ptr(e, o.w_off), (const float*)blob_ptr(e, o.scale_off),
                                  (const float*)blob_ptr(e, o.shift_off), blob_ptr(e, b.w_off), (const float*)blob_ptr(e, b.scale_off),
                                  (const float*)blob_ptr(e, b.shift_off), (float*)tab[b.out_buf], n, o.h, o.w, o.cin, o.stride, o.pad_t, o.pad_l,
                                  o.oh, o.ow, b.cout, b.aux, b.act, s);
            covered = 1;
        } else
        switch (o.kind) {
            case HSEFR_OP_CONV_C3:
                rc = launch_conv_c3((const float*)in, (const float*)blob_ptr(e, o.w_off),
                                    (const float*)blob_ptr(e, o.shift_off), (float*)out, n, o.h, o.w, o.kh, o.kw,
                                    o.stride, o.pad_t, o.pad_l, o.oh, o.ow, o.cout, o.act, s);
                break;
            case HSEFR_OP_DWCONV3X3:
                if (o.aux > 0)
                    rc = launch_dwconv3x3_split((const float*)in, (const float*)blob_ptr(e, o.w_off),
                                                (const float*)blob_ptr(e, o.scale_off), (const float*)blob_ptr(e, o.shift_off),
                                                out, n, o.h, o.w, o.cin, o.stride, o.pad_t, o.pad_l, o.oh, o.ow, o.act, o.aux, s);
                else
                    rc = launch_dwconv3x3((const float*)in, (const float*)blob_ptr(e, o.w_off),
                                          (const float*)blob_ptr(e, o.scale_off), (const float*)blob_ptr(e, o.shift_off),
                                          (float*)out, n, o.h, o.w, o.cin, o.stride, o.pad_t, o.pad_l, o.oh, o.ow, o.act, s);
                break;
            case HSEFR_OP_PWCONV_PS_GAP:
                rc = launch_pwconv_ps_gap(in, blob_ptr(e, o.w_off), (const float*)blob_ptr(e, o.scale_off), (const float*)blob_ptr(e, o.shift_off),
                                          (float*)out, (long long)n * o.h * o.w, o.cin, o.cout, o.act, o.h * o.w, s);
                break;
            case HSEFR_OP_PWCONV_PS_DW:
                rc = launch_pwconv_ps_dw(in, blob_ptr(e, o.w_off), (const float*)blob_ptr(e, o.scale_off), (const float*)blob_ptr(e, o.shift_off),
                                         (const float*)blob_ptr(e, o.w2_off), out, (long long)n * o.h * o.w, o.cin, o.cout, o.act, o.w,
                                         o.h * o.w, o.stride, ps_dw_aux(o.aux).out_log2, s);
                break;
            case HSEFR_OP_PWCONV_PS:
                rc = launch_pwconv_ps(in, blob_ptr(e, o.w_off), (const float*)blob_ptr(e, o.scale_off),
                                      (const float*)blob_ptr(e, o.shift_off), (float*)out, (long long)n * o.h * o.w, o.cin, o.cout,
                                      o.act, s);
                break;
            case HSEFR_OP_PWCONV_F32:
                rc = launch_pwconv_f32((const float*)in, (const float*)blob_ptr(e, o.w_off),
                                       (const float*)blob_ptr(e, o.shift_off), (float*)out,
                                       (long long)n * o.h * o.w, o.cin, o.cout, o.act, s);
                break;
            case HSEFR_OP_PWCONV_F16S:
                rc = launch_pwconv_f16s((const float*)in, blob_ptr(e, o.w_off), (const float*)blob_ptr(e, o.scale_off),
                                        (const float*)blob_ptr(e, o.shift_off), (float*)out, (long long)n * o.h * o.w,
                                        o.cin, o.cout, o.aux, o.act, s);
                break;
            case HSEFR_OP_GAP:
                rc = launch_gap((const float*)in, (float*)out, n, o.h * o.w, o.cin, s);
                break;
            case HSEFR_OP_DENSE:
                rc = launch_dense((const float*)in, (const float*)blob_ptr(e, o.w_off),
                                  (const float*)blob_ptr(e, o.shift_off), (float*)out, n, o.cin, o.cout, o.act, s);
                break;
            case HSEFR_OP_SOFTMAX:
                rc = launch_softmax((const float*)in, (float*)out, n, o.cout, s);
                break;
            case HSEFR_OP_CONV_BF16:
// ... 183 lines not shown
            e->graphs.push_back({n, mask, exec});
        }
        HSEFR_HIP_CHECK(hipMemcpyAsync(e->d_in_stage, d_input, in_bytes * n, hipMemcpyDeviceToDevice, s));
        HSEFR_HIP_CHECK(hipGraphLaunch(exec, s));
        e->graph_launches++;
        for (int sl = 0; sl < HSEFR_N_OUTPUT_SLOTS; ++sl) {
            if (!outs[sl]) continue;
            const size_t bytes = (size_t)e->hdr.out_elems[sl] * sizeof(float) * n;
            HSEFR_HIP_CHECK(hipMemcpyAsync(outs[sl], e->d_bufs[e->hdr.out_buffer[sl]], bytes, hipMemcpyDeviceToDevice, s));
        }
    } else {
        std::vector<void*> tab(e->d_bufs);
        const void* src_of[HSEFR_N_OUTPUT_SLOTS] = {nullptr, nullptr, nullptr};
        for (int sl = 0; sl < HSEFR_N_OUTPUT_SLOTS; ++sl) {
            if (!outs[sl]) continue;
            const int b = e->hdr.out_buffer[sl];
            if (tab[b] != e->d_bufs[b]) { src_of[sl] = tab[b]; continue; }
            if (((uintptr_t)outs[sl] & 15) == 0) tab[b] = outs[sl];
            else src_of[sl] = e->d_bufs[b];
        }
        for (int sl = 0; sl < HSEFR_N_OUTPUT_SLOTS; ++sl)
            if (outs[sl] && src_of[sl] == e->d_bufs[e->hdr.out_buffer[sl]]) src_of[sl] = tab[e->hdr.out_buffer[sl]];
        const int rc = run_ops(e, tab, d_input, n, needed, s, prof ? pev : nullptr, input_u8, mask == 0);
        if (rc != HSEFR_OK) return rc;
        for (int sl = 0; sl < HSEFR_N_OUTPUT_SLOTS; ++sl)
            if (outs[sl] && src_of[sl])
                HSEFR_HIP_CHECK(hipMemcpyAsync(outs[sl], src_of[sl], (size_t)e->hdr.out_elems[sl] * sizeof(float) * n,
                                               hipMemcpyDeviceToDevice, s));
    }
    if (prof) e->prof_calls++;
    return HSEFR_OK;
}

int hsefr_plan_describe(const void* plan, size_t plan_bytes, int n, char* out, size_t out_bytes) {
    HSEFR_REQUIRE(out && out_bytes > 0 && n > 0, HSEFR_ERR_INVALID, "plan_describe: bad argument");
    out[0] = 0;
    hsefr_engine e;
    const char* blob = nullptr;
    int rc = check_plan_blob(plan, plan_bytes, e.hdr, e.bufs, e.ops, blob);
    if (rc != HSEFR_OK) return rc;
    e.max_batch = n;
    e.d_blob = reinterpret_cast<char*>(uintptr_t(1) << 40);
    e.d_overflow = reinterpret_cast<int*>(uintptr_t(1) << 39);
    e.d_bufs.resize(e.hdr.n_buffers);
    for (uint32_t i = 0; i < e.hdr.n_buffers; ++i) e.d_bufs[i] = reinterpret_cast<void*>((uintptr_t(2) << 40) + (uintptr_t(i) << 32));
    std::string text;
    std::vector<char> only(e.ops.size(), 0);
    for (size_t i = 0; i < e.ops.size(); ++i) {
        std::fill(only.begin(), only.end(), 0);
        only[i] = 1;
        const size_t span = (e.ops[i].flags & HSEFR_OPF_PAIR_NEXT)                      ? 1
                            : (e.ops[i].flags & HSEFR_OPF_HEADS)                        ? 3
                            : ((e.ops[i].flags & HSEFR_OPF_DWPW_NEXT) && !dwpw_s2_off()) ? 1
                                                                                        : 0;
        for (size_t k = 1; k <= span && i + k < e.ops.size(); ++k) only[i + k] = 1;
        std::string line = std::to_string(i) + "\t" + std::to_string(e.ops[i].kind) + "\t";
        g_route_sink = &line;
        rc = run_ops(&e, e.d_bufs, reinterpret_cast<const void*>(uintptr_t(3) << 40), n, only, nullptr, nullptr,
                     false);
        g_route_sink = nullptr;
        if (rc != HSEFR_OK) { e.d_blob = nullptr; e.d_overflow = nullptr; e.d_bufs.clear(); return rc; }
        text += line + "\n";
        for (size_t k = 1; k <= span && i + k < e.ops.size(); ++k)
            text += std::to_string(i + k) + "\t" + std::to_string(e.ops[i + k].kind) + "\t(inside op " + std::to_string(i) + ")\n";
        i += span;
    }
    e.d_blob = nullptr; e.d_overflow = nullptr; e.d_bufs.clear();
    HSEFR_REQUIRE(text.size() + 1 <= out_bytes, HSEFR_ERR_INVALID, "plan_describe: the table needs %zu bytes, the buffer holds %zu", text.size() + 1, out_bytes);
    memcpy(out, text.c_str(), text.size() + 1);
    return HSEFR_OK;
}

int hsefr_engine_input_overflow(hsefr_engine* e, int* host_flag, hsefr_stream_t stream) {
    HSEFR_REQUIRE(e && host_flag, HSEFR_ERR_INVALID, "input_overflow: null argument");
    HSEFR_HIP_CHECK(hipMemcpyAsync(host_flag, e->d_overflow, sizeof(int), hipMemcpyDeviceToHost, (hipStream_t)stream));
    HSEFR_HIP_CHECK(hipMemsetAsync(e->d_overflow, 0, sizeof(int), (hipStream_t)stream));
    HSEFR_HIP_CHECK(hipStreamSynchronize((hipStream_t)stream));
    return HSEFR_OK;
}

int hsefr_engine_input_overflow_async(hsefr_engine* e, int* pinned_host_flag, hsefr_stream_t stream) {
    HSEFR_REQUIRE(e && pinned_host_flag, HSEFR_ERR_INVALID, "input_overflow_async: null argument");
    HSEFR_HIP_CHECK(hipMemcpyAsync(pinned_host_flag, e->d_overflow, sizeof(int), hipMemcpyDeviceToHost, (hipStream_t)stream));
    HSEFR_HIP_CHECK(hipMemsetAsync(e->d_overflow, 0, sizeof(int), (hipStream_t)stream));
    return HSEFR_OK;
}

int hsefr_engine_set_graph_batch(hsefr_engine* e, int max_n) {
    HSEFR_REQUIRE(e && max_n >= 0 && max_n <= e->max_batch, HSEFR_ERR_INVALID, "set_graph_batch: bad argument");
    for (auto& g : e->graphs) (void)hipGraphExecDestroy(g.exec);
    e->graphs.clear();
    if (e->d_in_stage) {
        (void)hipFree(e->d_in_stage);
        e->d_in_stage = nullptr;
        e->device_bytes -= (size_t)e->hdr.in_h * e->hdr.in_w * e->hdr.in_c * sizeof(float) * e->graph_max_n;
        (void)hipStreamDestroy(e->cap_stream);
        e->cap_stream = nullptr;
    }
    e->graph_max_n = max_n;
    return HSEFR_OK;
}

long long hsefr_engine_graph_launches(const hsefr_engine* e) { return e ? e->graph_launches : 0; }

int hsefr_engine_destroy(hsefr_engine* e) {
    if (!e) return HSEFR_OK;
// ... 75 lines not shown
}

int hsefr_stem3_fused(const float* x, const void* cw_split, const float* cdescale, const float* conv_shift, const float* wd1,
                      const float* d1scale, const float* d1shift, const void* w_split, const float* descale, const float* pshift,
                      const float* wd2, const float* d2scale, const float* d2shift, float* y, int* d_overflow, int n, int h, int w,
                      int cpad_t, int cpad_l, int h1, int w1, int pad_t2, int pad_l2, int oh2, int ow2, int in_log2, int a_log2,
                      int act, hsefr_stream_t stream) {
    HSEFR_REQUIRE(n == 0 || (x && cw_split && cdescale && conv_shift && wd1 && d1scale && d1shift && w_split && descale && pshift && wd2 &&
                             d2scale && d2shift && y), HSEFR_ERR_INVALID, "stem3_fused: null pointer");
    return launch_stem3_fused(x, cw_split, cdescale, conv_shift, wd1, d1scale, d1shift, w_split, descale, pshift, wd2, d2scale, d2shift, y,
                              d_overflow, n, h, w, cpad_t, cpad_l, h1, w1, pad_t2, pad_l2, oh2, ow2, in_log2, a_log2, act, (hipStream_t)stream);
}

int hsefr_stem4_fused(const void* x, int x_is_u8, const void* cw4, const float* cdescale, const float* conv_shift, const float* wd1,
                      const float* d1scale, const float* d1shift, const void* w_split, const float* descale, const float* pshift,
                      const float* wd2, const float* d2scale, const float* d2shift, float* y, int* d_overflow, int n, int h, int w,
                      int in_log2, int a_log2, int act, hsefr_stream_t stream) {
    HSEFR_REQUIRE(n == 0 || (x && cw4 && cdescale && conv_shift && wd1 && d1scale && d1shift && w_split && descale && pshift && wd2 &&
                             d2scale && d2shift && y), HSEFR_ERR_INVALID, "stem4_fused: null pointer");
    return launch_stem4_fused(x, x_is_u8, cw4, cdescale, conv_shift, wd1, d1scale, d1shift, w_split, descale, pshift, wd2, d2scale, d2shift, y,
                              d_overflow, n, h, w, in_log2, a_log2, act, (hipStream_t)stream);
}

int hsefr_stem5_stream(const void* x, int x_is_u8, const void* cw4, const float* cdescale, const float* conv_shift, const float* wd1,
                       const float* d1scale, const float* d1shift, const void* w_split, const float* descale, const float* pshift,
                       const float* wd2, const float* d2scale, const float* d2shift, float* y, int* d_overflow, int n, int h, int w,
                       int in_log2, int a_log2, int act, hsefr_stream_t stream) {
    HSEFR_REQUIRE(n == 0 || (x && cw4 && cdescale && conv_shift && wd1 && d1scale && d1shift && w_split && descale && pshift && wd2 &&
                             d2scale && d2shift && y), HSEFR_ERR_INVALID, "stem5_stream: null pointer");
    return launch_stem5_stream(x, x_is_u8, cw4, cdescale, conv_shift, wd1, d1scale, d1shift, w_split, descale, pshift, wd2, d2scale, d2shift, y,
                               d_overflow, n, h, w, in_log2, a_log2, act, (hipStream_t)stream);
}

#ifdef HSEFR_DEV
int hsefr_stem_fused(const float* x, const float* conv_w, const float* conv_shift, const float* wd, const float* dscale,
                     const float* dshift, const void* w_split, const float* descale, const float* pshift, float* y, int n,
                     int h, int w, int cpad_t, int cpad_l, int oh, int ow, int a_log2, int act, hsefr_stream_t stream) {
    HSEFR_REQUIRE(n == 0 || (x && conv_w && conv_shift && wd && dscale && dshift && w_split && descale && pshift && y),
                  HSEFR_ERR_INVALID, "stem_fused: null pointer");
    return launch_stem_fused(x, conv_w, conv_shift, wd, dscale, dshift, w_split, descale, pshift, y, n, h, w, cpad_t, cpad_l,
                             oh, ow, a_log2, act, (hipStream_t)stream);
}
#endif

int hsefr_dwpw_f16split(const float* x, const float* wd, const float* dscale, const float* dshift, const void* w_split,
                        const float* descale, const float* pshift, float* y, int n, int h, int w, int c, int stride,
                        int pad_t, int pad_l, int oh, int ow, int cout, int a_log2, int act, hsefr_stream_t stream) {
    HSEFR_REQUIRE(n == 0 || (x && wd && dscale && dshift && w_split && descale && pshift && y), HSEFR_ERR_INVALID,
                  "dwpw_f16split: null pointer");
    return launch_dwpw_f16s(x, wd, dscale, dshift, w_split, descale, pshift, y, n, h, w, c, stride, pad_t, pad_l, oh, ow, cout,
                            a_log2, act, (hipStream_t)stream);
}

int hsefr_dwpw_fused(const float* x, const float* wd, const float* dscale, const float* dshift, const float* wp_t,
                     const float* pshift, float* y, int n, int h, int w, int c, int stride, int pad_t, int pad_l, int oh,
                     int ow, int cout, hsefr_stream_t stream) {
    HSEFR_REQUIRE(n == 0 || (x && wd && dscale && dshift && wp_t && pshift && y), HSEFR_ERR_INVALID, "dwpw_fused: null pointer");
    return launch_dwpw_fused(x, wd, dscale, dshift, wp_t, pshift, y, n, h, w, c, stride, pad_t, pad_l, oh, ow, cout,
                             HSEFR_ACT_RELU6, HSEFR_ACT_RELU6, (hipStream_t)stream);
}

int hsefr_gap(const float* x, float* y, int n, int hw, int c, hsefr_stream_t stream) {
    HSEFR_REQUIRE(n == 0 || (x && y), HSEFR_ERR_INVALID, "gap: null pointer");
    return launch_gap(x, y, n, hw, c, (hipStream_t)stream);
}

int hsefr_dense(const float* x, const float* wgt, const float* bias, float* y, int n, int k, int cout, int act,
                hsefr_stream_t stream) {
    HSEFR_REQUIRE(n == 0 || (x && wgt && y), HSEFR_ERR_INVALID, "dense: null pointer");
    return launch_dense(x, wgt, bias, y, n, k, cout, act, (hipStream_t)stream);
}

int hsefr_heads_fused(const float* x, const float* w1, const float* b1, const float* wa, const float* ba, const float* wg, const float* bg,
                      float* hidden, float* logits, float* age_probs, float* gender, int n, int k, int a, hsefr_stream_t stream) {
    HSEFR_REQUIRE(n == 0 || (x && w1 && b1 && wa && ba && wg && bg && hidden && logits && age_probs && gender), HSEFR_ERR_INVALID,
                  "heads_fused: null pointer");
    return launch_heads_fused(x, w1, b1, wa, ba, wg, bg, hidden, logits, age_probs, gender, n, k, a, (hipStream_t)stream);
}

int hsefr_softmax(const float* x, float* y, int n, int c, hsefr_stream_t stream) {
    HSEFR_REQUIRE(n == 0 || (x && y), HSEFR_ERR_INVALID, "softmax: null pointer");
    return launch_softmax(x, y, n, c, (hipStream_t)stream);
}

int hsefr_conv_bf16(const void* x, const void* wgt_t, const float* scale, const float* shift, const void* res, void* y,
                    int n, int h, int w, int c, int oh, int ow, int cout, int kh, int kw, int stride, int pad_t,
                    int pad_l, int act, hsefr_stream_t stream) {
    HSEFR_REQUIRE(n == 0 || (x && wgt_t && scale && shift && y), HSEFR_ERR_INVALID, "conv_bf16: null pointer");
    return launch_conv_bf16(x, wgt_t, scale, shift, res, y, n, h, w, c, oh, ow, cout, kh, kw, stride, pad_t, pad_l, act,
                            (hipStream_t)stream);
}

int hsefr_conv1x1_proj_bf16(const void* x, const void* wgt_t, const float* scale, const float* shift, const void* x2, const void* wgt2_t,
                            const float* scale2, const float* shift2, void* y, int n, int oh, int ow, int c, int cout, int c2, int stride2,
                            int h2, int w2, int act, hsefr_stream_t stream) {
    HSEFR_REQUIRE(n == 0 || (x && wgt_t && scale && shift && x2 && wgt2_t && scale2 && shift2 && y), HSEFR_ERR_INVALID, "conv1x1_proj_bf16: null pointer");
    return launch_conv1x1_proj_bf16(x, wgt_t, scale, shift, x2, wgt2_t, scale2, shift2, y, n, oh, ow, c, cout, c2, stride2, h2, w2, act,
                                    (hipStream_t)stream);
}

int hsefr_conv1x1_sres_bf16(const void* x, const void* wgt_t, const float* scale, const float* shift, const void* res, void* y, int n, int oh,
                            int ow, int c, int cout, int res_stride, int h2, int w2, int act, hsefr_stream_t stream) {
    HSEFR_REQUIRE(n == 0 || (x && wgt_t && scale && shift && res && y), HSEFR_ERR_INVALID, "conv1x1_sres_bf16: null pointer");
    return launch_conv1x1_sres_bf16(x, wgt_t, scale, shift, res, y, n, oh, ow, c, cout, res_stride, h2, w2, act, (hipStream_t)stream);
}

// ... 216 lines not shown
```

### hse_facerec_tf_amd/csrc/fuzz_plan.cc

```cpp
#include <stdint.h>
#include <stdio.h>
#include <stdlib.h>
#include <string.h>

#include <string>
#include <vector>

#include "../../include/hsefr.h"

static uint64_t rng_state = 0x9E3779B97F4A7C15ull;
static uint64_t rnd() {
    rng_state ^= rng_state << 13;
    rng_state ^= rng_state >> 7;
    rng_state ^= rng_state << 17;
    return rng_state;
}

static long long n_ok = 0, n_err = 0, n_silent = 0;

static void run_one(const void* blob, size_t bytes, const char* what) {
    int rc = hsefr_plan_validate(blob, bytes);
    if (rc == HSEFR_OK) {
        ++n_ok;
        static char table[1 << 18];
        const int rd = hsefr_plan_describe(blob, bytes, 4, table, sizeof(table));
        if (rd != HSEFR_OK && !hsefr_last_error_string()[0]) { ++n_silent; fprintf(stderr, "no message for status %d (%s, plan_describe)\n", rd, what); }
        hsefr_engine* e = nullptr;
        rc = hsefr_engine_create(blob, bytes, 4, &e);
        if (rc == HSEFR_OK) hsefr_engine_destroy(e);
        else if (!hsefr_last_error_string()[0]) { ++n_silent; fprintf(stderr, "no message for status %d (%s, engine_create)\n", rc, what); }
        return;
    }
    ++n_err;
    if (rc > 0 || rc < HSEFR_ERR_SHAPE || !hsefr_last_error_string()[0]) {
        ++n_silent;
        fprintf(stderr, "status %d without a message / outside hsefr_status (%s)\n", rc, what);
    }
    hsefr_engine* e = nullptr;
    const int rc2 = hsefr_engine_create(blob, bytes, 4, &e);
    if (rc2 == HSEFR_OK) { fprintf(stderr, "engine_create accepted what plan_validate refused (%s)\n", what); abort(); }
}

int main(int argc, char** argv) {
    if (argc < 3) { fprintf(stderr, "usage: fuzz_plan <mutants per seed> <plan file>...\n"); return 2; }
    const long long per_seed = atoll(argv[1]);
    static const int32_t edge32[] = {0, 1, -1, -2, -3, 2, 3, 7, 8, 63, 64, 65, 127, 128, 255, 256, 511, 512, 4095, 4096, 65535, 65536, 0x7fffffff,
                                     (int32_t)0x80000000, (int32_t)0xffff0000, 1 << 20, 1 << 24, 1 << 30};
    static const uint64_t edge64[] = {0ull, 1ull, 15ull, 16ull, 17ull, 0xffffffffull, 0x100000000ull, 0x7fffffffffffffffull, 0x8000000000000000ull,
                                      0xffffffffffffffffull, 0xfffffffffffffff0ull};
    for (int f = 2; f < argc; ++f) {
        FILE* fp = fopen(argv[f], "rb");
        if (!fp) { perror(argv[f]); return 2; }
        fseek(fp, 0, SEEK_END);
        const size_t bytes = (size_t)ftell(fp);
        fseek(fp, 0, SEEK_SET);
        std::vector<unsigned char> seed(bytes);
        if (fread(seed.data(), 1, bytes, fp) != bytes) { fprintf(stderr, "short read\n"); return 2; }
        fclose(fp);
        if (bytes < sizeof(hsefr_plan_header)) { fprintf(stderr, "%s: not a plan\n", argv[f]); return 2; }
        hsefr_plan_header h;
        memcpy(&h, seed.data(), sizeof(h));
        const size_t tables = sizeof(h) + (size_t)h.n_buffers * sizeof(hsefr_plan_buffer) + (size_t)h.n_ops * sizeof(hsefr_plan_op);
        if (hsefr_plan_validate(seed.data(), bytes) != HSEFR_OK) {
            fprintf(stderr, "%s: the seed itself is refused: %s\n", argv[f], hsefr_last_error_string());
            return 1;
        }
        unsigned char* w = (unsigned char*)malloc(bytes);
        memcpy(w, seed.data(), bytes);
        char what[160];
        for (long long it = 0; it < per_seed; ++it) {
            const unsigned mode = (unsigned)(rnd() % 10);
            if (mode == 0) {
                size_t cut = (rnd() & 1) ? (size_t)(rnd() % (tables + 64 < bytes ? tables + 64 : bytes)) : (size_t)(rnd() % bytes);
                unsigned char* t = (unsigned char*)malloc(cut ? cut : 1);
                memcpy(t, seed.data(), cut);
                snprintf(what, sizeof(what), "%s truncated to %zu", argv[f], cut);
                run_one(t, cut, what);
                free(t);
                continue;
            }
            const int nmut = 1 + (int)(rnd() % 3);
            size_t where[3];
            unsigned char saved[3][8];
            size_t len[3];
            for (int m = 0; m < nmut; ++m) {
                size_t off;
                if (mode == 1) {
                    off = (size_t)(rnd() % tables);
                    len[m] = 1;
                    memcpy(saved[m], w + off, 1);
                    w[off] ^= (unsigned char)(1u << (rnd() % 8));
                } else if (mode == 2 && bytes > tables) {
                    off = tables + (size_t)(rnd() % (bytes - tables));
                    len[m] = 1;
                    memcpy(saved[m], w + off, 1);
                    w[off] = (unsigned char)rnd();
                } else if (mode <= 6) {
                    off = (size_t)(rnd() % (tables / 4)) * 4;
                    len[m] = 4;
// ... 31 lines not shown
```

### hse_facerec_tf_amd/lowering.py

```python
from __future__ import annotations

import struct
from dataclasses import dataclass, field
from typing import Dict, List, Optional, Sequence, Tuple

import numpy as np

from .graphdef import Graph, GraphNode

ACT_NONE, ACT_RELU, ACT_RELU6, ACT_SIGMOID = 0, 1, 2, 3
OP_CONV_C3, OP_DWCONV3X3, OP_PWCONV_F32, OP_GAP, OP_DENSE, OP_SOFTMAX = 1, 2, 3, 4, 5, 6
OP_CONV_BF16, OP_MAXPOOL_BF16, OP_GAP_BF16, OP_STEM7X7_BF16, OP_DWPW_F32 = 7, 8, 9, 10, 11
OP_PWCONV_F16S = 12
OP_DWPW_F16S = 13
OP_STEM_F16S = 14
OP_STEM2_F16S = 15
OP_STEM3_F16S = 17
OP_CONV_F32, OP_MAXPOOL_F32 = 18, 19
OP_STEM7X7_POOL_BF16 = 20
OP_PWDW_PS = 21
OP_PWGAP_PS = 22
OP_PWCONV_PS = 16
_BF16_OUT = (OP_CONV_BF16, OP_MAXPOOL_BF16, OP_STEM7X7_BF16, OP_STEM7X7_POOL_BF16)
OUT_FEATURES, OUT_AGE, OUT_GENDER = 0, 1, 2
BUF_INPUT, BUF_NONE = -1, -2
PLAN_MAGIC = 0x314C505246455348
NO_OFFSET = 0xFFFFFFFFFFFFFFFF

_HEADER = struct.Struct("<QIIIIII3i3IQ")
_BUFFER = struct.Struct("<QII")
_OP = struct.Struct("<II3i3i3i3i2iii5Q")
OPF_PAIR_NEXT, OPF_HEADS, OPF_OUT_SUB2, OPF_DWPW_NEXT = 1, 2, 4, 8
AUX_C2_SHIFT, AUX_C2_BITS, AUX_STRIDE2_SHIFT, AUX_STRIDE2_BITS = 0, 12, 12, 2
AUX_H2_SHIFT, AUX_H2_BITS, AUX_W2_SHIFT, AUX_W2_BITS = 14, 9, 23, 9
AUX_LOG2_BITS, AUX_OUT_LOG2_SHIFT, AUX_IN_LOG2_SHIFT, AUX_IN_LOG2_BIAS, AUX_U8_BIT = 8, 8, 8, 64, 16
AUX_POOL_PAD_L_SHIFT = 4
STEM_KW_PAD_T2_BIT, STEM_KW_PAD_L2_BIT = 4, 5
STEM_PACK_CONV, STEM_PACK_CONV_SHIFT, STEM_PACK_DW1, STEM_PACK_DW1_SCALE, STEM_PACK_DW1_SHIFT = 0, 864, 896, 1184, 1216
STEM_PACK_DW2, STEM_PACK_DW2_SCALE, STEM_PACK_DW2_SHIFT, STEM_PACK_STEM2_END = 1248, 1824, 1888, 1952
STEM_PACK_CONV_SPLIT, STEM_PACK_CONV_DESCALE, STEM_PACK_CONV4, STEM_PACK_CONV4_U8 = 1952, 2976, 3008, 5056
STEM_PACK_U8_SHIFT, STEM_PACK_U8_DESCALE, STEM_PACK_STEM3_END = 7104, 7232, 7264
STEM_SHIFT2_DESCALE, STEM_SHIFT2_SHIFT = 0, 64


PRODUCT_KERNEL_FAMILIES = frozenset({
    "stem5_stream_kernel", "stem4_fused_kernel", "stem3_fused_kernel", "stem2_fused_kernel", "conv3x3_c3_kernel", "conv3x3_c3_mfma_kernel",
    "dwconv3x3_kernel", "pwconv_f32_dma_kernel", "pwconv_f32_kernel", "pwconv_f16s_kernel", "pwconv_ps_kernel", "dwpw_fused_kernel",
    "dwpw_f16s_kernel", "dwpw2_f16s_kernel", "dwpw3_f16s_kernel", "dwpws2_f16s_kernel", "gap_kernel", "dense_kernel", "softmax_kernel", "heads_kernel",
    "stem7s_stream_kernel", "stem7x7_pool_bf16_kernel", "stem7x7_bf16_kernel", "maxpool3x3s2_bf16_kernel", "conv_bf16_kernel", "conv1x1_bf16_kernel",
    "conv1x1_w4_bf16_kernel", "conv1x1_pair_bf16_kernel", "conv3x3_w2_bf16_kernel", "conv_dma_bf16_kernel", "gap_bf16_kernel",
    "conv_f32_mfma_kernel", "conv2d_f32_kernel", "maxpool_f32_kernel"})


class LoweringError(NotImplementedError):
    """The graph uses a construct the engine has no kernel for (analogue of TF's
    'No OpKernel was registered' error)."""


def dequantize_min_first_u8(q: np.ndarray, range_min, range_max) -> np.ndarray:
    lo = np.float32(range_min)
    hi = np.float32(range_max)
    if lo == hi:
        return np.full(q.shape, lo, dtype=np.float32)
    step = np.float32(np.float64(hi - lo) / 255.0)
    lo_snapped = np.float32(np.round(lo / step) * step)
    return q.astype(np.float32) * step + lo_snapped


def tf_same_padding(size: int, k: int, stride: int) -> Tuple[int, int]:
    out = (size + stride - 1) // stride
    total = max((out - 1) * stride + k - size, 0)
    return out, total // 2


F16S_ACT_LOG2_RELU6 = 12


def split_pointwise_weights(w_t: np.ndarray, a_log2: int = F16S_ACT_LOG2_RELU6) -> Tuple[np.ndarray, np.ndarray]:
    w = np.ascontiguousarray(w_t, dtype=np.float32)
    cout, k = w.shape
    if k % 32:
        raise LoweringError("split_pointwise_weights: k=%d must be a multiple of 32" % k)
    amax = np.abs(w).max(axis=1).astype(np.float64)
    e = np.zeros(cout, np.int64)
    nz = amax > 0
    e[nz] = 14 - np.frexp(amax[nz])[1]
    e = np.clip(e, -100, 100)
    ws = np.ldexp(w.astype(np.float64), e[:, None]).astype(np.float32)
    hi = ws.astype(np.float16)
    lo = (ws - hi.astype(np.float32)).astype(np.float16)
    assert np.isfinite(hi.astype(np.float32)).all()
    img = np.empty((cout, k // 32, 64), np.uint16)
    img[:, :, :32] = hi.view(np.uint16).reshape(cout, k // 32, 32)
    img[:, :, 32:] = lo.view(np.uint16).reshape(cout, k // 32, 32)
    descale = np.ldexp(np.ones(cout, np.float64), -(e + a_log2)).astype(np.float32)
    return img, descale


def stem4_conv_image(w_hwio: np.ndarray, in_log2: int, reverse_channels: bool = False) -> Tuple[np.ndarray, np.ndarray]:
    w = np.asarray(w_hwio, dtype=np.float32).reshape(3, 3, 3, 32)
    if reverse_channels:
# ... 624 lines not shown
            L.shift = (beta - mean * k) if L.shift is None else (L.shift * k + beta - mean * k)
        elif op == "Relu" and not L.sealed and L.act == ACT_NONE:
            L.act = ACT_RELU
        elif op == "Relu6" and not L.sealed and L.act == ACT_NONE:
            L.act = ACT_RELU6
        elif op == "Minimum" and not L.sealed and L.act == ACT_RELU and float(np.asarray(consts[0]).reshape(-1)[0]) == 6.0:
            L.act = ACT_RELU6
        elif op == "Maximum" and L.act in (ACT_RELU, ACT_RELU6) and float(np.asarray(consts[0]).reshape(-1)[0]) == 0.0:
            pass
        elif op == "Sigmoid" and not L.sealed and L.act == ACT_NONE and L.kind == OP_DENSE:
            L.act = ACT_SIGMOID
        else:
            raise LoweringError("%s: cannot fuse op %s into layer %s (act=%d sealed=%s)" %
                                (node.name, op, L.name, L.act, L.sealed))
        L.version += 1
        self.where[node.name] = idx
        return idx

    def is_final(self, name: str) -> bool:
        li = self.where[name]
        return li >= 0 and self.ver.get(name, 0) == self.layers[li].version


def assign_buffers(layers: List[Layer], pinned) -> List[int]:
    last_use = list(range(len(layers)))
    for i, L in enumerate(layers):
        for s in (L.src, L.res):
            if s >= 0:
                last_use[s] = i
    for i, L in enumerate(layers):
        span = 1 if L.flags & OPF_PAIR_NEXT else 3 if L.flags & OPF_HEADS else 0
        for j in range(i, min(i + span, len(layers) - 1) + 1 if span else i):
            for s in (layers[j].src, layers[j].res, j):
                if s >= 0:
                    last_use[s] = max(last_use[s], i + span)
    buffers: List[int] = []
    free: List[int] = []
    for i, L in enumerate(layers):
        need = L.out_bytes
        pick = None
        if i not in pinned and free:
            fits = [b for b in free if buffers[b] >= need]
            pick = min(fits, key=lambda b: buffers[b]) if fits else max(free, key=lambda b: buffers[b])
            free.remove(pick)
            buffers[pick] = max(buffers[pick], need)
        if pick is None:
            buffers.append(need)
            pick = len(buffers) - 1
        L.out_buf = pick
        for j in range(i + 1):
            if last_use[j] == i and j not in pinned and layers[j].out_buf not in free:
                free.append(layers[j].out_buf)
    for i, L in enumerate(layers):
        if L.flags & OPF_DWPW_NEXT and L.src >= 0 and i + 1 < len(layers) and layers[i + 1].out_buf == layers[L.src].out_buf:
            a, b = layers[L.src].out_buf, L.out_buf
            buffers[a] = buffers[b] = max(buffers[a], buffers[b])
    return buffers


def consumers_of(layers: List[Layer]) -> Dict[int, List[Tuple[int, str]]]:
    consumers: Dict[int, List[Tuple[int, str]]] = {}
    for i, L in enumerate(layers):
        for how in ("src", "res"):
            s = getattr(L, how)
            if s >= 0:
                consumers.setdefault(s, []).append((i, how))
    return consumers


def sole_reader(consumers: Dict[int, List[Tuple[int, str]]], i: int, keep: Sequence[int]) -> int:
    cons = consumers.get(i, [])
    return cons[0][0] if i not in keep and len(cons) == 1 and cons[0][1] == "src" else -1


def rebuild(layers: List[Layer], drop, put: Dict[int, Layer]) -> Tuple[List[Layer], Dict[int, int]]:
    new_layers: List[Layer] = []
    remap: Dict[int, int] = {}
    for i, L in enumerate(layers):
        if i in drop:
            remap[i] = -1
        else:
            remap[i] = len(new_layers)
            new_layers.append(put.get(i, L))
    for L in new_layers:
        for how in ("src", "res"):
            s = getattr(L, how)
            if s >= 0:
                if remap[s] < 0:
                    raise LoweringError("%s still reads %s (as %s), which a fusion pass removed" % (L.name, layers[s].name, how))
                setattr(L, how, remap[s])
    return new_layers, remap


def dwpw_fusable(dw: Layer, pw: Layer) -> bool:
    return (dw.kind == OP_DWCONV3X3 and pw.kind == OP_PWCONV_F32 and dw.act == ACT_RELU6 and pw.act == ACT_RELU6 and
            dw.in_shape[2] in (32, 64) and pw.out_shape[2] in (64, 128) and dw.stride in (1, 2))


def fuse_dwpw(layers: List[Layer], keep: Sequence[int]) -> Tuple[List[Layer], Dict[int, int]]:
    consumers = consumers_of(layers)
    put: Dict[int, Layer] = {}
    drop = set()
    for i, dw in enumerate(layers):
        j = sole_reader(consumers, i, keep)
        if dw.kind == OP_DWCONV3X3 and j >= 0 and dwpw_fusable(dw, layers[j]):
            pw = layers[j]
            put[j] = Layer(OP_DWPW_F32, pw.name, dw.src, dw.in_shape, pw.out_shape, w=dw.w, scale=dw.scale, shift=dw.shift,
# ... 179 lines not shown
        L1, L2, L3 = layers[i1], layers[i2], layers[i3]
        S = Layer(OP_STEM2_F16S, L3.name, -1, L0.in_shape, L3.out_shape, w=L1.w, scale=L1.scale, shift=L1.shift, act=L3.act, kh=3, kw=3,
                  stride=2, pad_t=L0.pad_t, pad_l=L0.pad_l, sealed=True, w2=L2.w, shift2=L2.shift, a_log2=F16S_ACT_LOG2_RELU6,
                  w0=L0.w, shift0=L0.shift, w3=L3.w, scale3=L3.scale, shift3=L3.shift, pad3=(L3.pad_t, L3.pad_l))
        return rebuild(layers, {i0, i1, i2}, {i3: S})
    return rebuild(layers, set(), {})


BLOCK_F16S_AUTO = ((128, 128), (256, 256))


def block_f16s_fusable(dw: Layer, pw: Layer, which: str) -> bool:
    c, cout = dw.in_shape[2], pw.out_shape[2]
    if not (dw.kind == OP_DWCONV3X3 and pw.kind == OP_PWCONV_F32 and pw.a_log2 > 0 and dw.act == ACT_RELU6 and
            pw.act in (ACT_NONE, ACT_RELU, ACT_RELU6) and dw.stride in (1, 2) and c % 32 == 0 and cout % 64 == 0):
        return False
    return which == "all" or (dw.stride == 1 and (c, cout) in BLOCK_F16S_AUTO)


def fuse_block_f16s(layers: List[Layer], keep: Sequence[int], which: str) -> Tuple[List[Layer], Dict[int, int]]:
    consumers = consumers_of(layers)
    put: Dict[int, Layer] = {}
    drop = set()
    for i, dw in enumerate(layers):
        j = sole_reader(consumers, i, keep)
        if dw.kind == OP_DWCONV3X3 and j >= 0 and block_f16s_fusable(dw, layers[j], which):
            pw = layers[j]
            put[j] = Layer(OP_DWPW_F16S, pw.name, dw.src, dw.in_shape, pw.out_shape, w=dw.w, scale=dw.scale, shift=dw.shift,
                           act=pw.act, kh=3, kw=3, stride=dw.stride, pad_t=dw.pad_t, pad_l=dw.pad_l, sealed=True,
                           w2=pw.w, shift2=pw.shift, a_log2=pw.a_log2)
            drop.add(i)
    return rebuild(layers, drop, put)


def dwpw_pair_covered(dw: Layer, pw: Layer) -> bool:
    return dw.stride == 2 and dw.in_shape[2] == 128 and pw.out_shape[2] == 256


def mark_dwpw_pairs(layers: List[Layer], keep: Sequence[int]) -> int:
    consumers = consumers_of(layers)
    n = 0
    for i, dw in enumerate(layers):
        j = sole_reader(consumers, i, keep)
        if not (dw.kind == OP_DWCONV3X3 and dw.act == ACT_RELU6 and dw.out_split == 0 and dw.flags == 0 and j == i + 1):
            continue
        pw = layers[j]
        if (pw.kind == OP_PWCONV_F32 and 0 < pw.a_log2 <= 12 and not pw.in_split and pw.flags == 0 and pw.res < 0 and
                tuple(pw.in_shape) == tuple(dw.out_shape) and dwpw_pair_covered(dw, pw)):
            dw.flags |= OPF_DWPW_NEXT
            n += 1
    return n


def choose_pointwise_math(layers: List[Layer], pw_math: str) -> None:
    if pw_math not in ("auto", "f32", "f16split"):
        raise ValueError("pw_math must be 'auto', 'f32' or 'f16split', not %r" % (pw_math,))
    if pw_math == "f32":
        return
    for L in layers:
        if L.kind != OP_PWCONV_F32:
            continue
        bounded = L.src >= 0 and layers[L.src].act == ACT_RELU6 and layers[L.src].kind not in _BF16_OUT
        if bounded and L.in_shape[2] % 32 == 0 and L.out_shape[2] % 64 == 0:
            L.a_log2 = F16S_ACT_LOG2_RELU6
        elif pw_math == "f16split":
            raise LoweringError("%s: split-f16 pointwise needs a ReLU6-bounded input, k %% 32 == 0 and cout %% 64 == 0" % L.name)


PRESPLIT_MIN_K = 256


def presplit_activations(layers: List[Layer], keep: Sequence[int]) -> int:
    consumers = consumers_of(layers)
    n = 0
    for i, L in enumerate(layers):
        if not (L.kind == OP_PWCONV_F32 and L.a_log2 > 0 and L.src >= 0):
            continue
        P = layers[L.src]
        k, cout = L.in_shape[2], L.out_shape[2]
        if (P.kind == OP_DWCONV3X3 and P.act == ACT_RELU6 and L.src not in keep and consumers.get(L.src) == [(i, "src")] and
                k % 32 == 0 and k >= PRESPLIT_MIN_K and cout % 128 == 0 and 0 < L.a_log2 <= 12):
            P.out_split = L.a_log2
            L.in_split = True
            n += 1
    return n


def pwdw_fusable(pw: Layer, dw: Layer) -> bool:
    h, w, _ = dw.in_shape
    if not (pw.kind == OP_PWCONV_F32 and pw.a_log2 > 0 and pw.in_split and pw.out_shape[2] % 128 == 0 and
            dw.kind == OP_DWCONV3X3 and dw.act == ACT_RELU6 and 0 < dw.out_split <= 12 and h * w <= 288):
        return False
    if dw.stride == 1:
        return dw.pad_t == 1 and dw.pad_l == 1 and dw.out_shape == dw.in_shape
    return (dw.stride == 2 and (h, w) in ((12, 12), (14, 14)) and (dw.pad_t, dw.pad_l) == (0, 0) and dw.out_shape[:2] == (h // 2, w // 2) and
            pw.act == ACT_RELU6)


def fuse_pwgap(layers: List[Layer], keep: Sequence[int]) -> Tuple[List[Layer], Dict[int, int]]:
    consumers = consumers_of(layers)
    for i, L in enumerate(layers):
        j = sole_reader(consumers, i, keep)
        h, w, c = L.out_shape
        if not (L.kind == OP_PWCONV_F32 and L.a_log2 > 0 and L.in_split and c % 128 == 0 and j >= 0 and
                layers[j].kind == OP_GAP and 33 <= h * w <= 288):
            continue
        G = layers[j]
        F = Layer(OP_PWGAP_PS, G.name, L.src, L.in_shape, G.out_shape, w=L.w, shift=L.shift, act=L.act, sealed=True, a_log2=L.a_log2,
                  in_split=True, tensors=list(G.tensors))
        return rebuild(layers, {i}, {j: F})
    return rebuild(layers, set(), {})


def fuse_pwdw(layers: List[Layer], keep: Sequence[int]) -> Tuple[List[Layer], Dict[int, int]]:
    consumers = consumers_of(layers)
    put: Dict[int, Layer] = {}
    drop = set()
    for i, pw in enumerate(layers):
        j = sole_reader(consumers, i, keep)
        if j >= 0 and pwdw_fusable(pw, layers[j]):
            dw = layers[j]
            put[j] = Layer(OP_PWDW_PS, dw.name, pw.src, pw.in_shape, dw.out_shape, w=pw.w, shift=pw.shift, act=pw.act, sealed=True,
                           a_log2=pw.a_log2, in_split=True, w3=dw.w, scale3=dw.scale, shift3=dw.shift, out_split=dw.out_split, kh=3, kw=3,
                           stride=dw.stride, pad_t=dw.pad_t, pad_l=dw.pad_l, tensors=list(dw.tensors))
            drop.add(i)
    return rebuild(layers, drop, put)


def lower_graph(g: Graph, input_tensor: str, outputs: Dict[int, str], input_hw: Optional[Tuple[int, int]] = None,
                feeds: Optional[Dict[str, object]] = None, fuse: bool = True, dtype: str = "f32",
                pw_math: Optional[str] = None, fuse_stem_block: Optional[bool] = None, stem_fusion: Optional[str] = None,
                block_fusion: Optional[str] = None, presplit: Optional[str] = None, input_bound: Optional[float] = None,
                pwdw_fusion: Optional[str] = None, u8_mean_bgr: Optional[Sequence[float]] = None, launch_fusion: bool = True,
                s2_fusion: Optional[str] = None) -> Plan:
    if dtype not in ("f32", "bf16", "f32g"):
        raise ValueError("dtype must be 'f32', 'bf16' or 'f32g', not %r" % (dtype,))
    in_node, _ = g.get_tensor_by_name(input_tensor)
    shape = g.placeholder_shape(in_node.name)
    if input_hw is None:
        if shape is None or len(shape) != 4 or shape[1] <= 0 or shape[2] <= 0:
            raise ValueError("input tensor %s has no static HxW; pass input_hw" % input_tensor)
        input_hw = (int(shape[1]), int(shape[2]))
    feeds_n = {}
    for k, v in (feeds or {}).items():
        feeds_n[g.get_tensor_by_name(k)[0].name] = v
    low = _Lowerer(g, in_node.name, input_hw, feeds_n, dtype)
    if shape is not None and len(shape) == 4 and shape[3] > 0:
        low.in_c = int(shape[3])
    out_layers: Dict[int, Tuple[int, int]] = {}
    low.mark_live([g.get_tensor_by_name(t)[0] for t in outputs.values()])
    for slot, tname in outputs.items():
        node, _ = g.get_tensor_by_name(tname)
        li = low.lower_node(node)
        if li < 0:
            raise LoweringError("output %s is the graph input" % tname)
        out_layers[slot] = (li, int(np.prod(low.layers[li].out_shape)))
    layers = low.layers

    for L in layers:
        if L.kind in (OP_CONV_C3, OP_PWCONV_F32, OP_DENSE) and L.scale is not None:
            L.w = (L.w * L.scale.reshape((1,) * (L.w.ndim - 1) + (-1,))).astype(np.float32)
            L.scale = None
        if L.kind in (OP_CONV_C3, OP_PWCONV_F32, OP_DWCONV3X3, OP_DENSE) and L.shift is None:
            L.shift = np.zeros(L.out_shape[2], np.float32)
        if L.kind == OP_DWCONV3X3 and L.scale is None:
            L.scale = np.ones(L.out_shape[2], np.float32)
        if L.kind == OP_CONV_F32 and L.act not in (ACT_NONE, ACT_RELU, ACT_RELU6):
            raise LoweringError("%s: activation %d on a general convolution" % (L.name, L.act))
        if L.kind in (OP_CONV_BF16, OP_STEM7X7_BF16):
            cout = L.out_shape[2]
            L.scale = np.ones(cout, np.float32) if L.scale is None else L.scale.astype(np.float32)
            L.shift = np.zeros(cout, np.float32) if L.shift is None else L.shift.astype(np.float32)
            if L.act not in (ACT_NONE, ACT_RELU, ACT_RELU6):
                raise LoweringError("%s: activation %d on a bf16 convolution" % (L.name, L.act))
            from .resnet50 import pack_conv_weight, pack_stem_weight
            L.w = pack_stem_weight(L.w) if L.kind == OP_STEM7X7_BF16 else pack_conv_weight(L.w)

    for slot, tname in outputs.items():
        nm = g.get_tensor_by_name(tname)[0].name
        if not low.is_final(nm):
            raise LoweringError("output %s is an intermediate of fused layer %s; fetch the layer's final tensor"
                                % (tname, layers[low.where[nm]].name))
    tensor_layer = {name: li for name, li in low.where.items() if li >= 0 and low.is_final(name)}

    def keep() -> List[int]:
        return [li for li, _ in out_layers.values()]

# ... 14 lines not shown
        if input_bound is not None:
            if not (input_bound > 0 and np.isfinite(input_bound)):
                raise ValueError("input_bound must be a positive finite number, not %r" % (input_bound,))
            in_log2 = int(np.floor(np.log2(32768.0 / float(input_bound))))
            in_log2 = max(-8, min(14, in_log2))
            if float(input_bound) * 2.0 ** in_log2 <= 32768.0:
                for L in layers:
                    if L.kind == OP_STEM2_F16S:
                        L.kind, L.in_log2 = OP_STEM3_F16S, in_log2
                        if u8_mean_bgr is not None:
                            if len(u8_mean_bgr) != 3 or not all(0.0 <= float(m) <= 255.0 for m in u8_mean_bgr):
                                raise ValueError("u8_mean_bgr must be three means in [0, 255], not %r" % (u8_mean_bgr,))
                            if float(input_bound) < 256.0:
                                raise ValueError("uint8 input needs input_bound >= 256 (pixels minus a mean), not %r" % (input_bound,))
                            L.u8_mean_bgr = tuple(float(m) for m in u8_mean_bgr)
    if fuse and dtype == "bf16":
        for fuse_pass in (fuse_stem_pool, fuse_proj):
            apply(fuse_pass)
        subsample_stage_tails(layers, keep())
    if fuse:
        apply(fuse_dwpw)

    if dtype == "f32":
        choose_pointwise_math(layers, pw_math)
        if want_stem:
            apply(fuse_stem)
        block_fusion = block_fusion or "auto"
        if block_fusion not in ("auto", "none", "all"):
            raise ValueError("block_fusion must be 'auto', 'none' or 'all', not %r" % (block_fusion,))
        if fuse and block_fusion != "none":
            apply(fuse_block_f16s, block_fusion)
        presplit = presplit or "auto"
        if presplit not in ("auto", "none"):
            raise ValueError("presplit must be 'auto' or 'none', not %r" % (presplit,))
        if presplit == "auto":
            presplit_activations(layers, keep())
            pwdw_fusion = pwdw_fusion or "auto"
            if pwdw_fusion not in ("auto", "none"):
                raise ValueError("pwdw_fusion must be 'auto' or 'none', not %r" % (pwdw_fusion,))
            if fuse and pwdw_fusion == "auto":
                apply(fuse_pwdw)
                apply(fuse_pwgap)
    if fuse and launch_fusion:
        if dtype == "bf16":
            mark_pairs(layers)
            compact_pair_outputs(layers, keep())
        if dtype == "f32":
            mark_heads(layers)
    s2_fusion = s2_fusion or "auto"
    if s2_fusion not in ("auto", "none"):
        raise ValueError("s2_fusion must be 'auto' or 'none', not %r" % (s2_fusion,))
    if fuse and launch_fusion and dtype == "f32" and s2_fusion == "auto":
        mark_dwpw_pairs(layers, keep())
    buffers = assign_buffers(layers, set(keep()))
    return Plan(layers, (input_hw[0], input_hw[1], low.in_c), buffers, out_layers, tensor_layer)
```

### hse_facerec_tf_amd/ops.py

```python
from __future__ import annotations

import ctypes
from typing import Optional, Tuple

import numpy as np

from . import _lib
from .lowering import ACT_NONE, ACT_RELU, ACT_RELU6, ACT_SIGMOID, tf_same_padding


def _device_guarded(fn):
    import functools

    @functools.wraps(fn)
    def wrapper(*args, **kw):
        devs = [a.device for a in list(args) + list(kw.values()) if hasattr(a, "is_cuda") and a.is_cuda]
        if not devs:
            return fn(*args, **kw)
        if any(d != devs[0] for d in devs):
            raise ValueError("%s: tensors live on different devices: %s" % (fn.__name__, sorted({str(d) for d in devs})))
        with _lib.on_device(devs[0]):
            return fn(*args, **kw)
    return wrapper

# ... 120 lines not shown
    return ys


@_device_guarded
def pwconv1x1(x, w_t, shift, act: int = ACT_RELU6):
    torch = _lib.require_gpu()
    _f32c(x, "x"), _f32c(w_t, "w_t"), _f32c(shift, "shift")
    k = x.shape[-1]
    cout = w_t.shape[0]
    m = x.numel() // k
    y = torch.empty(tuple(x.shape[:-1]) + (cout,), dtype=torch.float32, device=x.device)
    _lib.check(_lib.lib().hsefr_pwconv1x1_bias_relu6(x.data_ptr(), w_t.data_ptr(), shift.data_ptr(), y.data_ptr(),
                                                     m, k, cout, act, _lib.current_stream_ptr()),
               "hsefr_pwconv1x1_bias_relu6")
    return y


def split_weights_device(w_t, device, a_log2: int = 12):
    torch = _lib.require_gpu()
    from . import lowering
    w_np = w_t.detach().cpu().numpy() if hasattr(w_t, "detach") else w_t
    img, descale = lowering.split_pointwise_weights(w_np, a_log2)
    return torch.from_numpy(img.view(np.int16)).to(device), torch.from_numpy(descale).to(device)


@_device_guarded
def pwconv1x1_f16split(x, w_t, shift, act: int = ACT_RELU6, a_log2: int = 12, prepared=None):
    torch = _lib.require_gpu()
    _f32c(x, "x"), _f32c(shift, "shift")
    d_img, d_ds = prepared if prepared is not None else split_weights_device(w_t, x.device, a_log2)
    k = x.shape[-1]
    cout = d_img.shape[0]
    m = x.numel() // k
    y = torch.empty(tuple(x.shape[:-1]) + (cout,), dtype=torch.float32, device=x.device)
    _lib.check(_lib.lib().hsefr_pwconv1x1_f16split(x.data_ptr(), d_img.data_ptr(), d_ds.data_ptr(), shift.data_ptr(),
                                                   y.data_ptr(), m, k, cout, a_log2, act, _lib.current_stream_ptr()),
               "hsefr_pwconv1x1_f16split")
    return y


@_device_guarded
def dwpw_f16split(x, w_hwc, dscale, dshift, wp_t, pshift, stride: int = 1, act: int = ACT_RELU6, a_log2: int = 12, prepared=None):
    torch = _lib.require_gpu()
    for t, nm in ((x, "x"), (w_hwc, "w"), (dscale, "dscale"), (dshift, "dshift"), (pshift, "pshift")):
        _f32c(t, nm)
    d_img, d_ds = prepared if prepared is not None else split_weights_device(wp_t, x.device, a_log2)
    n, h, w, c = x.shape
    cout = d_img.shape[0]
    oh, ow, pt, pl = _same(h, w, 3, stride)
    y = torch.empty((n, oh, ow, cout), dtype=torch.float32, device=x.device)
    _lib.check(_lib.lib().hsefr_dwpw_f16split(x.data_ptr(), w_hwc.data_ptr(), dscale.data_ptr(), dshift.data_ptr(), d_img.data_ptr(),
                                              d_ds.data_ptr(), pshift.data_ptr(), y.data_ptr(), n, h, w, c, stride, pt, pl, oh, ow,
                                              cout, a_log2, act, _lib.current_stream_ptr()), "hsefr_dwpw_f16split")
    return y


@_device_guarded
def stem_fused(x, conv_w, conv_shift, w_hwc, dscale, dshift, wp_t, pshift, act: int = ACT_RELU6, a_log2: int = 12, prepared=None):
    torch = _lib.require_gpu()
    if not hasattr(_lib.lib(), "hsefr_stem_fused"):
        raise NotImplementedError("round 1's fused stem is part of DEVELOPMENT builds of the library only (HSEFR_LIB=libhsefr_dev.so)")
    for t, nm in ((x, "x"), (conv_w, "conv_w"), (conv_shift, "conv_shift"), (w_hwc, "w"), (dscale, "dscale"), (dshift, "dshift"),
                  (pshift, "pshift")):
        _f32c(t, nm)
    d_img, d_ds = prepared if prepared is not None else split_weights_device(wp_t, x.device, a_log2)
    n, h, w, c = x.shape
    if c != 3 or tuple(conv_w.shape) != (3, 3, 3, 32) or tuple(w_hwc.shape) != (3, 3, 32) or d_img.shape[0] != 64:
        raise NotImplementedError("stem_fused covers 3 -> 32 -> 64 channels")
    oh, ow, pt, pl = _same(h, w, 3, 2)
    y = torch.empty((n, oh, ow, 64), dtype=torch.float32, device=x.device)
    _lib.check(_lib.lib().hsefr_stem_fused(x.data_ptr(), conv_w.data_ptr(), conv_shift.data_ptr(), w_hwc.data_ptr(), dscale.data_ptr(),
                                           dshift.data_ptr(), d_img.data_ptr(), d_ds.data_ptr(), pshift.data_ptr(), y.data_ptr(),
                                           n, h, w, pt, pl, oh, ow, a_log2, act, _lib.current_stream_ptr()), "hsefr_stem_fused")
    return y


@_device_guarded
def stem2_fused(x, conv_w, conv_shift, w1_hwc, d1scale, d1shift, wp_t, pshift, w2_hwc, d2scale, d2shift, act: int = ACT_RELU6,
                a_log2: int = 12, prepared=None):
    torch = _lib.require_gpu()
    for t, nm in ((x, "x"), (conv_w, "conv_w"), (conv_shift, "conv_shift"), (w1_hwc, "w1"), (d1scale, "d1scale"), (d1shift, "d1shift"),
                  (pshift, "pshift"), (w2_hwc, "w2"), (d2scale, "d2scale"), (d2shift, "d2shift")):
        _f32c(t, nm)
    d_img, d_ds = prepared if prepared is not None else split_weights_device(wp_t, x.device, a_log2)
    n, h, w, c = x.shape
    if c != 3 or tuple(conv_w.shape) != (3, 3, 3, 32) or tuple(w1_hwc.shape) != (3, 3, 32) or d_img.shape[0] != 64 or \
            tuple(w2_hwc.shape) != (3, 3, 64):
        raise NotImplementedError("stem2_fused covers 3 -> 32 -> 64 channels")
    h1, w1, pt, pl = _same(h, w, 3, 2)
    oh2, ow2, pt2, pl2 = _same(h1, w1, 3, 2)
    y = torch.empty((n, oh2, ow2, 64), dtype=torch.float32, device=x.device)
    _lib.check(_lib.lib().hsefr_stem2_fused(x.data_ptr(), conv_w.data_ptr(), conv_shift.data_ptr(), w1_hwc.data_ptr(), d1scale.data_ptr(),
                                            d1shift.data_ptr(), d_img.data_ptr(), d_ds.data_ptr(), pshift.data_ptr(), w2_hwc.data_ptr(),
                                            d2scale.data_ptr(), d2shift.data_ptr(), y.data_ptr(), n, h, w, pt, pl, h1, w1, pt2, pl2,
                                            oh2, ow2, a_log2, act, _lib.current_stream_ptr()), "hsefr_stem2_fused")
    return y


@_device_guarded
def stem3_fused(x, conv_w, conv_shift, w1_hwc, d1scale, d1shift, wp_t, pshift, w2_hwc, d2scale, d2shift, act: int = ACT_RELU6,
                a_log2: int = 12, in_log2: int = 7, prepared=None, overflow=None):
    torch = _lib.require_gpu()
    from . import lowering
    for t, nm in ((x, "x"), (conv_shift, "conv_shift"), (w1_hwc, "w1"), (d1scale, "d1scale"), (d1shift, "d1shift"),
                  (pshift, "pshift"), (w2_hwc, "w2"), (d2scale, "d2scale"), (d2shift, "d2shift")):
        _f32c(t, nm)
# ... 506 lines not shown
```

### include/hsefr.h

```cpp
#ifndef HSEFR_H
#define HSEFR_H

#include <stddef.h>
#include <stdint.h>

#ifdef __cplusplus
extern "C" {
#endif

#define HSEFR_VERSION 141

typedef enum hsefr_status {
    HSEFR_OK = 0,
    HSEFR_ERR_INVALID = -1,
    HSEFR_ERR_UNSUPPORTED = -2,
    HSEFR_ERR_HIP = -3,
    HSEFR_ERR_NOMEM = -4,
    HSEFR_ERR_SHAPE = -5
} hsefr_status;

typedef enum hsefr_act {
    HSEFR_ACT_NONE = 0,
    HSEFR_ACT_RELU = 1,
    HSEFR_ACT_RELU6 = 2,
// ... 13 lines not shown
typedef enum hsefr_op_kind {
    HSEFR_OP_CONV_C3 = 1,
    HSEFR_OP_DWCONV3X3 = 2,
    HSEFR_OP_PWCONV_F32 = 3,
    HSEFR_OP_GAP = 4,
    HSEFR_OP_DENSE = 5,
    HSEFR_OP_SOFTMAX = 6,
    HSEFR_OP_CONV_BF16 = 7,
    HSEFR_OP_MAXPOOL_BF16 = 8,
    HSEFR_OP_GAP_BF16 = 9,
    HSEFR_OP_STEM7X7_BF16 = 10,
    HSEFR_OP_DWPW_F32 = 11,
    HSEFR_OP_PWCONV_F16S = 12,
    HSEFR_OP_DWPW_F16S = 13,
    HSEFR_OP_STEM_F16S = 14,
    HSEFR_OP_CONV_F32 = 18,
    HSEFR_OP_MAXPOOL_F32 = 19,
    HSEFR_OP_STEM7X7_POOL_BF16 = 20,
    HSEFR_OP_PWCONV_PS_DW = 21,
    HSEFR_OP_PWCONV_PS_GAP = 22,
    HSEFR_OP_STEM3_F16S = 17,
    HSEFR_OP_PWCONV_PS = 16,
    HSEFR_OP_STEM2_F16S = 15
} hsefr_op_kind;

typedef enum hsefr_output_slot {
    HSEFR_OUT_FEATURES = 0,
    HSEFR_OUT_AGE = 1,
    HSEFR_OUT_GENDER = 2,
    HSEFR_N_OUTPUT_SLOTS = 3
} hsefr_output_slot;

typedef struct hsefr_plan_header {
    uint64_t magic;
    uint32_t version;
    uint32_t n_buffers;
    uint32_t n_ops;
    uint32_t in_h, in_w, in_c;
    int32_t out_buffer[HSEFR_N_OUTPUT_SLOTS];
    uint32_t out_elems[HSEFR_N_OUTPUT_SLOTS];
    uint64_t blob_bytes;
} hsefr_plan_header;

typedef struct hsefr_plan_buffer {
    uint64_t elems_per_image;
    uint32_t elem_bytes;
    uint32_t reserved;
} hsefr_plan_buffer;

typedef enum hsefr_op_flags {
    HSEFR_OPF_PAIR_NEXT = 1,
    HSEFR_OPF_HEADS = 2,
    HSEFR_OPF_OUT_SUB2 = 4,
    HSEFR_OPF_DWPW_NEXT = 8
} hsefr_op_flags;

enum {
    HSEFR_AUX_C2_SHIFT = 0, HSEFR_AUX_C2_BITS = 12,
    HSEFR_AUX_STRIDE2_SHIFT = 12, HSEFR_AUX_STRIDE2_BITS = 2,
    HSEFR_AUX_H2_SHIFT = 14, HSEFR_AUX_H2_BITS = 9,
    HSEFR_AUX_W2_SHIFT = 23, HSEFR_AUX_W2_BITS = 9,
    HSEFR_AUX_LOG2_BITS = 8,
    HSEFR_AUX_OUT_LOG2_SHIFT = 8,
    HSEFR_AUX_IN_LOG2_SHIFT = 8,
    HSEFR_AUX_IN_LOG2_BIAS = 64,
    HSEFR_AUX_U8_BIT = 16,
    HSEFR_AUX_POOL_PAD_L_SHIFT = 4
};

enum { HSEFR_STEM_KW_PAD_T2_BIT = 4, HSEFR_STEM_KW_PAD_L2_BIT = 5 };

enum {
    HSEFR_STEM_PACK_CONV = 0,
    HSEFR_STEM_PACK_CONV_SHIFT = 864,
    HSEFR_STEM_PACK_DW1 = 896,
    HSEFR_STEM_PACK_DW1_SCALE = 1184,
    HSEFR_STEM_PACK_DW1_SHIFT = 1216,
    HSEFR_STEM_PACK_DW2 = 1248,
    HSEFR_STEM_PACK_DW2_SCALE = 1824,
    HSEFR_STEM_PACK_DW2_SHIFT = 1888,
    HSEFR_STEM_PACK_STEM2_END = 1952,
    HSEFR_STEM_PACK_CONV_SPLIT = 1952,
    HSEFR_STEM_PACK_CONV_DESCALE = 2976,
    HSEFR_STEM_PACK_CONV4 = 3008,
    HSEFR_STEM_PACK_CONV4_U8 = 5056,
    HSEFR_STEM_PACK_U8_SHIFT = 7104,
    HSEFR_STEM_PACK_U8_DESCALE = 7232,
    HSEFR_STEM_PACK_STEM3_END = 7264
};

enum { HSEFR_STEM_SHIFT2_DESCALE = 0, HSEFR_STEM_SHIFT2_SHIFT = 64 };

typedef struct hsefr_plan_op {
    uint32_t kind;
    uint32_t act;
    int32_t in_buf, out_buf, res_buf;
    int32_t h, w, cin;
    int32_t oh, ow, cout;
    int32_t kh, kw, stride;
    int32_t pad_t, pad_l;
    int32_t aux;
    int32_t flags;
    uint64_t w_off;
    uint64_t scale_off;
    uint64_t shift_off;
    uint64_t w2_off;
    uint64_t shift2_off;
// ... 14 lines not shown
int hsefr_engine_max_batch(const hsefr_engine* e);

int hsefr_engine_forward(hsefr_engine* e, const void* d_input, int n, void* d_features,
                         void* d_age_probs, void* d_gender, hsefr_stream_t stream);

int hsefr_engine_accepts_u8(const hsefr_engine* e);
int hsefr_engine_forward_u8(hsefr_engine* e, const void* d_input_u8, int n, void* d_features, void* d_age_probs, void* d_gender,
                            hsefr_stream_t stream);

void* hsefr_engine_buffer(hsefr_engine* e, int buffer);
int hsefr_engine_copy_buffer(hsefr_engine* e, int buffer, void* d_dst, size_t bytes, hsefr_stream_t stream);

int hsefr_engine_set_profiling(hsefr_engine* e, int depth);
long long hsefr_engine_profiled_calls(const hsefr_engine* e);
int hsefr_engine_op_times_ms(hsefr_engine* e, int slot, float* ms, int n_ops);

int hsefr_engine_input_overflow(hsefr_engine* e, int* host_flag, hsefr_stream_t stream);
int hsefr_engine_input_overflow_async(hsefr_engine* e, int* pinned_host_flag, hsefr_stream_t stream);
int hsefr_engine_destroy(hsefr_engine* e);


int hsefr_conv_c3_bias_act(const float* x, const float* wgt, const float* shift, float* y, int n, int h,
                           int w, int kh, int kw, int stride, int pad_t, int pad_l, int oh, int ow,
                           int cout, int act, hsefr_stream_t stream);

int hsefr_dwconv3x3_bn_relu6(const float* x, const float* wgt, const float* scale, const float* shift,
                             float* y, int n, int h, int w, int c, int stride, int pad_t, int pad_l,
                             int oh, int ow, int act, hsefr_stream_t stream);

int hsefr_dwconv3x3_bn_relu6_split(const float* x, const float* wgt, const float* scale, const float* shift, void* y_split,
                                   int n, int h, int w, int c, int stride, int pad_t, int pad_l, int oh, int ow, int act,
                                   int a_log2, hsefr_stream_t stream);

int hsefr_pwconv1x1_bias_relu6(const float* x, const float* wgt_t, const float* shift, float* y,
                               long long m, int k, int cout, int act, hsefr_stream_t stream);

int hsefr_pwconv1x1_f16split(const float* x, const void* w_split, const float* descale, const float* shift, float* y,
                             long long m, int k, int cout, int a_log2, int act, hsefr_stream_t stream);

int hsefr_pwconv1x1_presplit(const void* x_split, const void* w_split, const float* descale, const float* shift, float* y,
                             long long m, int k, int cout, int act, hsefr_stream_t stream);

int hsefr_pwconv1x1_presplit_gap(const void* x_split, const void* w_split, const float* descale, const float* shift, float* y,
                                 long long m, int k, int cout, int act, int map_hw, hsefr_stream_t stream);

int hsefr_pwconv1x1_presplit_dw(const void* x_split, const void* w_split, const float* descale, const float* shift, const float* dw_consts,
                                void* y_split, long long m, int k, int cout, int act, int map_w, int map_hw, int dw_stride, int out_log2,
                                hsefr_stream_t stream);

int hsefr_dwpw_f16split(const float* x, const float* wd, const float* dscale, const float* dshift, const void* w_split,
                        const float* descale, const float* pshift, float* y, int n, int h, int w, int c, int stride,
                        int pad_t, int pad_l, int oh, int ow, int cout, int a_log2, int act, hsefr_stream_t stream);

int hsefr_stem2_fused(const float* x, const float* conv_w, const float* conv_shift, const float* wd1, const float* d1scale,
                      const float* d1shift, const void* w_split, const float* descale, const float* pshift, const float* wd2,
                      const float* d2scale, const float* d2shift, float* y, int n, int h, int w, int cpad_t, int cpad_l,
                      int h1, int w1, int pad_t2, int pad_l2, int oh2, int ow2, int a_log2, int act, hsefr_stream_t stream);

int hsefr_stem3_fused(const float* x, const void* cw_split, const float* cdescale, const float* conv_shift, const float* wd1,
                      const float* d1scale, const float* d1shift, const void* w_split, const float* descale, const float* pshift,
                      const float* wd2, const float* d2scale, const float* d2shift, float* y, int* d_overflow, int n, int h, int w,
                      int cpad_t, int cpad_l, int h1, int w1, int pad_t2, int pad_l2, int oh2, int ow2, int in_log2, int a_log2,
                      int act, hsefr_stream_t stream);

int hsefr_stem4_fused(const void* x, int x_is_u8, const void* cw4, const float* cdescale, const float* conv_shift, const float* wd1,
                      const float* d1scale, const float* d1shift, const void* w_split, const float* descale, const float* pshift,
                      const float* wd2, const float* d2scale, const float* d2shift, float* y, int* d_overflow, int n, int h, int w,
                      int in_log2, int a_log2, int act, hsefr_stream_t stream);
int hsefr_stem5_stream(const void* x, int x_is_u8, const void* cw4, const float* cdescale, const float* conv_shift, const float* wd1,
                      const float* d1scale, const float* d1shift, const void* w_split, const float* descale, const float* pshift,
                      const float* wd2, const float* d2scale, const float* d2shift, float* y, int* d_overflow, int n, int h, int w,
                      int in_log2, int a_log2, int act, hsefr_stream_t stream);

int hsefr_dwpw_fused(const float* x, const float* wd, const float* dscale, const float* dshift, const float* wp_t,
                     const float* pshift, float* y, int n, int h, int w, int c, int stride, int pad_t, int pad_l, int oh,
                     int ow, int cout, hsefr_stream_t stream);

int hsefr_gap(const float* x, float* y, int n, int hw, int c, hsefr_stream_t stream);

int hsefr_dense(const float* x, const float* wgt, const float* bias, float* y, int n, int k, int cout,
                int act, hsefr_stream_t stream);

int hsefr_softmax(const float* x, float* y, int n, int c, hsefr_stream_t stream);

int hsefr_heads_fused(const float* x, const float* w1, const float* b1, const float* wa, const float* ba, const float* wg, const float* bg,
                      float* hidden, float* logits, float* age_probs, float* gender, int n, int k, int a, hsefr_stream_t stream);


int hsefr_conv_bf16(const void* x, const void* wgt_t, const float* scale, const float* shift, const void* res, void* y,
                    int n, int h, int w, int c, int oh, int ow, int cout, int kh, int kw, int stride, int pad_t,
                    int pad_l, int act, hsefr_stream_t stream);

int hsefr_conv1x1_proj_bf16(const void* x, const void* wgt_t, const float* scale, const float* shift, const void* x2, const void* wgt2_t,
                            const float* scale2, const float* shift2, void* y, int n, int oh, int ow, int c, int cout, int c2, int stride2,
                            int h2, int w2, int act, hsefr_stream_t stream);

int hsefr_conv1x1_sres_bf16(const void* x, const void* wgt_t, const float* scale, const float* shift, const void* res, void* y, int n, int oh,
                            int ow, int c, int cout, int res_stride, int h2, int w2, int act, hsefr_stream_t stream);

int hsefr_conv1x1_pair_bf16(const void* x, const void* w1_t, const float* scale1, const float* shift1, const void* res, const void* x2,
                            const void* wp_t, const float* scale_p, const float* shift_p, void* y1, const void* w2_t, const float* scale2,
                            const float* shift2, void* y2, long long pixels, int c, int cout1, int cout2, int c2, int act1, int act2,
                            hsefr_stream_t stream);

int hsefr_conv1x1_pair_sub2_bf16(const void* x, const void* w1_t, const float* scale1, const float* shift1, const void* res, const void* x2,
                                 const void* wp_t, const float* scale_p, const float* shift_p, void* y1, const void* w2_t, const float* scale2,
// ... 88 lines not shown
```

Before: 254,700.

## Fuse preceding pointwise conv into the dw+pw kernel for 64->128->128 blocks

Adds a pwdwpw kernel in which extra waves compute the 1x1 expansion GEMM (64->128 channels, f16 split precision) directly into the LDS halo ring. The existing dw+pw consumer waves then read that ring, so the intermediate 128-channel activation never goes through global memory and one launch is removed. The lowering marks eligible pw->dwpw pairs by default. The cost is a larger LDS footprint and a block of 768 threads. Halo rows are recomputed at tile edges.

```diff
diff --git a/hse_facerec_tf_amd/_lib.py b/hse_facerec_tf_amd/_lib.py
--- a/hse_facerec_tf_amd/_lib.py
+++ b/hse_facerec_tf_amd/_lib.py
@@ -45,6 +45,7 @@
     "hsefr_engine_input_overflow": (c_int, [c_void_p, POINTER(c_int), c_void_p]),
     "hsefr_engine_input_overflow_async": (c_int, [c_void_p, POINTER(c_int), c_void_p]),
     "hsefr_dwpw_f16split": (c_int, [_fp, _fp, _fp, _fp, c_void_p, _fp, _fp, _fp] + [c_int] * 12 + [c_void_p]),
+    "hsefr_pwdwpw_f16split": (c_int, [_fp, c_void_p, _fp, _fp, _fp, _fp, _fp, c_void_p, _fp, _fp, _fp] + [c_int] * 9 + [c_void_p]),
     "hsefr_pwconv1x1_f16split": (c_int, [_fp, c_void_p, _fp, _fp, _fp, c_longlong, c_int, c_int, c_int, c_int, c_void_p]),
     "hsefr_dwpw_fused": (c_int, [_fp] * 7 + [c_int] * 10 + [c_void_p]),
     "hsefr_gap": (c_int, [_fp, _fp, c_int, c_int, c_int, c_void_p]),
diff --git a/hse_facerec_tf_amd/csrc/common.h b/hse_facerec_tf_amd/csrc/common.h
--- a/hse_facerec_tf_amd/csrc/common.h
+++ b/hse_facerec_tf_amd/csrc/common.h
@@ -266,6 +266,13 @@
 bool dwpw_f16s_supported(int c, int cout, int stride);
 bool dwpw_s2_covered(int c, int cout, int stride);
 bool dwpw_s2_off();
+int launch_pwdwpw_f16s(const float* x0, const void* w0split, const float* descale0, const float* shift0, const float* wd, const float* dscale,
+                       const float* dshift, const void* wsplit, const float* descale, const float* pshift, float* y, int n, int h, int w,
+                       int c0, int c, int cout, int a0_log2, int a_log2, int act, hipStream_t s);
+bool pwdwpw_covered(int c0, int c, int cout, int stride);
+bool pwdwpw_launchable(int n, int h, int w, int c0, int c, int cout);
+bool pwdwpw_worth(int n, int h, int w);
+bool pwdwpw_off();
 int launch_stem_fused(const float* x, const float* cw, const float* cshift, const float* wd, const float* dscale,
                       const float* dshift, const void* wsplit, const float* descale, const float* pshift, float* y, int n,
                       int h, int w, int cpad_t, int cpad_l, int oh, int ow, int a_log2, int act, hipStream_t s);
@@ -317,6 +324,8 @@
 void set_c11_adv(int v);
 int read_c11_stamps(void* host_out, size_t bytes);
 void set_dwpw_s2_off(int v);
+void set_pwdwpw_off(int v);
+void set_pwdwpw_min_items(int v);
 void set_dwpws_tw(int v);
 void set_dwpws_bn(int v);
 void set_pw_tile(int v);
diff --git a/hse_facerec_tf_amd/csrc/dwpw_f16s.hip b/hse_facerec_tf_amd/csrc/dwpw_f16s.hip
--- a/hse_facerec_tf_amd/csrc/dwpw_f16s.hip
+++ b/hse_facerec_tf_amd/csrc/dwpw_f16s.hip
@@ -27,6 +27,11 @@
     int nimg;
     unsigned m_n, m_w, m_h;
     unsigned long long* stamps;
+    const float* x0;
+    const float* w0split;
+    const float* descale0;
+    const float* shift0;
+    float a_scale0;
 };
 
 constexpr int ROWB = 128;
@@ -204,22 +209,28 @@
 constexpr int HALO_B = 192 * 128;
 constexpr int CMAX2 = 512;
 
-template <int TW, int BN, int HS, int ACT>
-__global__ __launch_bounds__(256 + 64 * (BN == 256 ? 8 : 4), BN == 256 ? 1 : 2) void dwpw3_f16s_kernel(DwPwSParams p) {
+constexpr int FR_C0 = 64, FR_C = 128, FR_WAVES = 4;
+template <int TW, int BN, int HS, int ACT, bool FRONT>
+__device__ __forceinline__ void dwpw3_body(const DwPwSParams& p) {
     constexpr int NCW = BN == 256 ? 8 : 4;
     constexpr int CWN = NCW / 2;
-    constexpr int NTHR = 256 + 64 * NCW;
+    constexpr int NTHR = 256 + 64 * NCW + (FRONT ? 64 * FR_WAVES : 0);
     constexpr int TH = 128 / TW, HC = TW + 2;
-    constexpr int WCAP = 256;
+    constexpr int WCAP = FRONT ? FR_C : 256;
     constexpr int B_ST = BN * ROWB;
     constexpr int B_OFF = HS * HALO_B, A_OFF = B_OFF + 2 * B_ST, W_OFF = A_OFF + 2 * 128 * ROWB, E_OFF = W_OFF + 11 * WCAP * 4;
+    constexpr int E0_OFF = E_OFF + 2 * CMAX2 * 4, F_OFF = E0_OFF + 2 * FR_C * 4;
+    constexpr int F_ST = FR_C * ROWB;
+    constexpr int LDS_BYTES = FRONT ? F_OFF + (FR_C0 / 32) * F_ST : E0_OFF;
+    static_assert(!FRONT || (HS == 2 && BN == FR_C && TW == 16), "the front GEMM fills a two-slot ring of 8 x 16 patches");
     constexpr int WN = BN / CWN, NI = WN / 32;
     constexpr int BPW = BN / 8 / NCW;
     static_assert(BPW == 4 && NI == 2, "a consumer's slice of the weight stage is its 4 KB epilogue scratch");
     constexpr bool HALO_BY_CONSUMER = false;
+    constexpr bool HALO_BY_PRODUCER = !HALO_BY_CONSUMER && !FRONT;
     constexpr int HPW = 24 / (HALO_BY_CONSUMER ? NCW : 4);
-    static_assert(E_OFF + 2 * CMAX2 * 4 <= 160 * 1024, "LDS budget");
-    __shared__ __attribute__((aligned(1024))) unsigned char smem[E_OFF + 2 * CMAX2 * 4];
+    static_assert(LDS_BYTES <= 160 * 1024, "LDS budget");
+    __shared__ __attribute__((aligned(1024))) unsigned char smem[LDS_BYTES];
 
     const int tid = threadIdx.x;
     const int lane = tid & 63;
@@ -231,6 +242,15 @@
         for (int i = tid; i < p.C4; i += NTHR) { wl[9 * p.C4 + i] = p.dscale[i]; wl[10 * p.C4 + i] = p.dshift[i]; }
         float* el = (float*)(smem + E_OFF);
         for (int i = tid; i < p.Cout; i += NTHR) { el[i] = p.descale[i]; el[CMAX2 + i] = p.pshift[i]; }
+        if (FRONT) {
+            float* e0 = (float*)(smem + E0_OFF);
+            for (int i = tid; i < FR_C; i += NTHR) { e0[i] = p.descale0[i]; e0[FR_C + i] = p.shift0[i]; }
+            for (int i = tid; i < FR_C * (FR_C0 / 32) * 8; i += NTHR) {
+                const int r = i >> 4, kt = (i >> 3) & 1, c = i & 7;
+                *(f32x4*)(smem + F_OFF + kt * F_ST + swzb(r, c)) = *(const f32x4*)(p.w0split + (r * (FR_C0 / 32) + kt) * 32 + 4 * c);
+            }
+            __syncthreads();
+        }
     }
     const __amdgpu_buffer_rsrc_t rx = make_rsrc(p.x, (long long)p.nimg * p.H * p.W * C * 4);
     const __amdgpu_buffer_rsrc_t rw = make_rsrc(p.wsplit, (long long)p.Cout * C * 4);
@@ -287,7 +307,7 @@
     if (wave < 4) {
         const int quad = tid & 7, col = (tid >> 3) % TW, r0 = 4 * (tid / (8 * TW));
         const unsigned char* hsrc0 = smem + ((r0 * HC + col) * 128 + quad * 16);
-        if (!HALO_BY_CONSUMER) {
+        if (HALO_BY_PRODUCER) {
             setup_halo(0);
 #pragma unroll
             for (int i = 0; i < HS - 1; ++i)
@@ -297,7 +317,7 @@
         __syncthreads();
         int dkc = 0;
         for (int g = -1; g < nsteps; ++g) {
-            const bool issued = !HALO_BY_CONSUMER && pf_step < nsteps;
+            const bool issued = HALO_BY_PRODUCER && pf_step < nsteps;
             if (issued) halo_dma();
             STEM_STAMP(1);
             if (g + 1 < nsteps) {
@@ -343,7 +363,7 @@
             STEM_STAMP(3);
         }
         STEM_STAMP_FLUSH(p.stamps, lane, wave);
-    } else {
+    } else if (!FRONT || wave < 4 + NCW) {
         const int cw = wave - 4, wm = cw / CWN, wn = cw % CWN;
         const int li = lane & 31, lh = lane >> 5;
         const int arow = wm * 64 + li, brow = wn * WN + li;
@@ -494,7 +514,126 @@
             o[9] = npatch;
         }
 #endif
+    } else {
+        const int fw = wave - 4 - NCW;
+        const bool two = fw < FR_WAVES / 2;
+        const int li = lane & 31, lh = lane >> 5;
+        const __amdgpu_buffer_rsrc_t rx0 = make_rsrc(p.x0, (long long)p.nimg * p.H * p.W * FR_C0 * 4);
+        unsigned vo[2] = {OOB, OOB}, inside[2] = {0, 0}, inside_next[2] = {0, 0};
+        int hq0 = fw * 32 + li;
+        auto setup = [&](unsigned i) {
+            const Item it = decode(i);
+            asm volatile("" : "+v"(hq0));
+#pragma unroll
+            for (int b = 0; b < 2; ++b) {
+                const int hq = hq0 + 128 * b, hr = hq / HC, hc = hq - hr * HC;
+                const int ih = it.oh0 - p.pad_t + hr, iw = it.ow0 - p.pad_l + hc;
+                const bool ok = hq < (TH + 2) * HC && ih >= 0 && ih < p.H && iw >= 0 && iw < p.W;
+                vo[b] = ok ? (unsigned)((it.n * p.H + ih) * p.W + iw) * (unsigned)(FR_C0 * 4) + 32u * lh : OOB;
+                inside_next[b] = (unsigned)__ballot(ok);
+            }
+        };
+        f32x4 raw[4][2];
+        f16x8 ah[2][4], al[2][4];
+        auto issue = [&](int b) {
+#pragma unroll
+            for (int s = 0; s < 4; ++s) {
+                raw[s][0] = bload16(rx0, vo[b], 64u * s);
+                raw[s][1] = bload16(rx0, vo[b], 64u * s + 16u);
+            }
+        };
+        auto split = [&](auto BLK) {
+            constexpr int b = decltype(BLK)::value;
+#pragma unroll
+            for (int s = 0; s < 4; ++s) {
+                f16x4 hi[2], lo[2];
+#pragma unroll
+                for (int e = 0; e < 2; ++e) {
+                    const f32x4 v = raw[s][e] * p.a_scale0;
+                    hi[e] = __builtin_convertvector(v, f16x4);
+                    lo[e] = __builtin_convertvector(v - __builtin_convertvector(hi[e], f32x4), f16x4);
+                }
+                ah[b][s] = __builtin_shufflevector(hi[0], hi[1], 0, 1, 2, 3, 4, 5, 6, 7);
+                al[b][s] = __builtin_shufflevector(lo[0], lo[1], 0, 1, 2, 3, 4, 5, 6, 7);
+                __builtin_amdgcn_sched_barrier(0);
+            }
+            inside[b] = inside_next[b];
+        };
+        auto gemm = [&](auto B_FROM, auto B_TO, int kc, unsigned char* slot) {
+            constexpr int b0 = decltype(B_FROM)::value, b1 = decltype(B_TO)::value, nb = 2;
+            const int brow = kc * 32 + li;
+            f32x16 acc[nb];
+#pragma unroll
+            for (int b = b0; b < b1; ++b)
+#pragma unroll
+                for (int r = 0; r < 16; ++r) acc[b][r] = 0.f;
+#pragma unroll
+            for (int s = 0; s < 4; ++s) {
+                const unsigned char* Fs = smem + F_OFF + (s >> 1) * F_ST;
+                const f16x8 bh = *(const f16x8*)(Fs + swzb(brow, 2 * (s & 1) + lh));
+                const f16x8 bl = *(const f16x8*)(Fs + swzb(brow, 4 + 2 * (s & 1) + lh));
+#pragma unroll
+                for (int b = b0; b < b1; ++b) acc[b] = __builtin_amdgcn_mfma_f32_32x32x16_f16(al[b][s], bh, acc[b], 0, 0, 0);
+#pragma unroll
+                for (int b = b0; b < b1; ++b) acc[b] = __builtin_amdgcn_mfma_f32_32x32x16_f16(ah[b][s], bl, acc[b], 0, 0, 0);
+#pragma unroll
+                for (int b = b0; b < b1; ++b) acc[b] = __builtin_amdgcn_mfma_f32_32x32x16_f16(ah[b][s], bh, acc[b], 0, 0, 0);
+                __builtin_amdgcn_sched_barrier(0);
+            }
+            const float* e0 = (const float*)(smem + E0_OFF);
+            const float ds = e0[brow], sh = e0[FR_C + brow];
+#pragma unroll
+            for (int b = b0; b < b1; ++b) {
+                float* out = (float*)(slot + ((fw + 4 * b) * 32 + 4 * lh) * 128) + li;
+                const unsigned ins = inside[b] >> (4 * lh);
+#pragma unroll
+                for (int r = 0; r < 16; ++r) {
+                    const int row = 8 * (r >> 2) + (r & 3);
+                    const float v = apply_act<HSEFR_ACT_RELU6>(fmaf(acc[b][r], ds, sh));
+                    out[row * 32] = ((ins >> row) & 1u) ? v : 0.f;
+                }
+            }
+        };
+        typedef std::integral_constant<int, 0> B0;
+        typedef std::integral_constant<int, 1> B1;
+        unsigned fi = 0;
+        int fkc = 0;
+        auto fstep = [&](unsigned char* slot) {
+            typedef std::integral_constant<int, 2> B2;
+            gemm(B0(), B1(), fkc, slot);
+            if (fkc == 0) {
+                if (two) split(B1());
+                setup(++fi);
+                issue(0);
+            }
+            if (fkc == KT - 1) {
+                split(B0());
+                if (two) issue(1);
+            }
+            if (two) gemm(B1(), B2(), fkc, slot);
+            if (++fkc == KT) fkc = 0;
+        };
+        setup(0);
+        issue(0);
+        split(B0());
+        if (two) issue(1);
+        fstep(smem);
+        __syncthreads();
+        for (int g = -1; g < nsteps; ++g) {
+            if (g + 2 < nsteps) fstep(smem + ((g + 2) & 1) * HALO_B);
+            __syncthreads();
+        }
     }
+}
+
+template <int TW, int BN, int HS, int ACT>
+__global__ __launch_bounds__(256 + 64 * (BN == 256 ? 8 : 4), BN == 256 ? 1 : 2) void dwpw3_f16s_kernel(DwPwSParams p) {
+    dwpw3_body<TW, BN, HS, ACT, false>(p);
+}
+
+template <int ACT>
+__global__ __launch_bounds__(512 + 64 * FR_WAVES, 1) void pwdwpw_f16s_kernel(DwPwSParams p) {
+    dwpw3_body<16, FR_C, 2, ACT, true>(p);
 }
 
 constexpr unsigned S2_GRID = 256;
@@ -745,6 +884,8 @@
 }
 
 HSEFR_KNOB(g_s2_off, 0);
+HSEFR_KNOB(g_front_off, 0);
+HSEFR_KNOB(g_front_min, 128);
 HSEFR_KNOB(g_tw, 0);
 HSEFR_KNOB(g_bn, 0);
 
@@ -800,6 +941,27 @@
     return launch_status("dwpw_f16split");
 }
 
+int launch_front(DwPwSParams& p, int n, int act, hipStream_t s) {
+    p.tiles_w = (p.OW + 15) / 16;
+    p.tiles_h = (p.OH + 7) / 8;
+    p.tiles_n = 1;
+    const long long total = (long long)n * p.tiles_w * p.tiles_h;
+    HSEFR_REQUIRE(total < (1ll << 31) / 16, HSEFR_ERR_UNSUPPORTED, "pwdwpw_f16split: grid too large");
+    p.total = (unsigned)total;
+    auto magic = [](unsigned d) { return d == 1 ? 0u : (unsigned)((0x100000000ull + d - 1) / d); };
+    p.m_n = 0; p.m_w = magic(p.tiles_w); p.m_h = magic(p.tiles_h);
+    HSEFR_REQUIRE(total * (long long)(p.tiles_w > p.tiles_h ? p.tiles_w : p.tiles_h) < (1ll << 32), HSEFR_ERR_UNSUPPORTED,
+                  "pwdwpw_f16split: grid too large for the quotient multipliers");
+    const unsigned g = p.total < 256u ? p.total : 256u;
+#define HSEFR_PWDWPW(A) HSEFR_LAUNCH((pwdwpw_f16s_kernel<A>), dim3(g), dim3(512 + 64 * FR_WAVES), 0, s, p)
+    if (act == HSEFR_ACT_RELU6) HSEFR_PWDWPW(HSEFR_ACT_RELU6);
+    else if (act == HSEFR_ACT_RELU) HSEFR_PWDWPW(HSEFR_ACT_RELU);
+    else if (act == HSEFR_ACT_NONE) HSEFR_PWDWPW(HSEFR_ACT_NONE);
+    else { set_error("pwdwpw_f16split: act %d", act); return HSEFR_ERR_UNSUPPORTED; }
+#undef HSEFR_PWDWPW
+    return launch_status("pwdwpw_f16split");
+}
+
 int launch_s2(DwPwSParams& p, int n, int act, hipStream_t s) {
     p.tiles_w = (p.OW + S2_T - 1) / S2_T;
     p.tiles_h = (p.OH + S2_T - 1) / S2_T;
@@ -825,6 +987,8 @@
 
 #ifdef HSEFR_DEV
 void set_dwpw_s2_off(int v) { g_s2_off = v; }
+void set_pwdwpw_off(int v) { g_front_off = v; }
+void set_pwdwpw_min_items(int v) { g_front_min = v; }
 void set_dwpws_tw(int v) { g_tw = v; }
 void set_dwpws_bn(int v) { g_bn = v; }
 #endif
@@ -832,6 +996,10 @@
 bool dwpw_s2_off() { return g_s2_off != 0; }
 
 bool dwpw_s2_covered(int c, int cout, int stride) { return stride == 2 && c == S2_C && cout == S2_COUT; }
+
+bool pwdwpw_off() { return g_front_off != 0; }
+
+bool pwdwpw_covered(int c0, int c, int cout, int stride) { return stride == 1 && c0 == FR_C0 && c == FR_C && cout == FR_C; }
 
 bool dwpw_f16s_supported(int c, int cout, int stride) {
     return c > 0 && c % 32 == 0 && cout > 0 && cout % 64 == 0 && (stride == 1 || stride == 2);
@@ -853,6 +1021,7 @@
     p.reverse = sweep_reverse();
     p.nimg = n;
     p.stamps = nullptr;
+    p.x0 = nullptr; p.w0split = nullptr; p.descale0 = nullptr; p.shift0 = nullptr; p.a_scale0 = 0.f;
 #ifdef HSEFR_STEM_STAMPS
     p.stamps = stamp_buffer(s);
 #endif
@@ -877,4 +1046,35 @@
     return tw == 16 ? launch_bn<2, 16>(p, n, bn, act, s) : launch_bn<2, 8>(p, n, bn, act, s);
 }
 
-}
+bool pwdwpw_launchable(int n, int h, int w, int c0, int c, int cout) {
+    const long long px = (long long)n * h * w;
+    return pwdwpw_covered(c0, c, cout, 1) && px * c * 4 < (1ll << 32) - 16 && px * cout * 4 < (1ll << 32) - 16;
+}
+
+bool pwdwpw_worth(int n, int h, int w) { return (long long)n * ((h + 7) / 8) * ((w + 15) / 16) >= g_front_min; }
+
+int launch_pwdwpw_f16s(const float* x0, const void* w0split, const float* descale0, const float* shift0, const float* wd, const float* dscale,
+                       const float* dshift, const void* wsplit, const float* descale, const float* pshift, float* y, int n, int h, int w,
+                       int c0, int c, int cout, int a0_log2, int a_log2, int act, hipStream_t s) {
+    HSEFR_REQUIRE(pwdwpw_launchable(n, h, w, c0, c, cout), HSEFR_ERR_UNSUPPORTED,
+                  "pwdwpw_f16split: %d -> %d -> %d channels at %d x %d x %d not covered (64 -> 128 -> 128, tensors below 4 GB)", c0, c, cout, n, h, w);
+    HSEFR_REQUIRE(n >= 0 && h > 0 && w > 0, HSEFR_ERR_INVALID, "pwdwpw_f16split: bad shape");
+    HSEFR_REQUIRE(a0_log2 > 0 && a0_log2 <= 12 && a_log2 > 0 && a_log2 <= 12, HSEFR_ERR_INVALID,
+                  "pwdwpw_f16split: a_log2 = %d, %d (both tensors are in [0,6]: 1..12)", a0_log2, a_log2);
+    if (n == 0) return HSEFR_OK;
+    DwPwSParams p;
+    p.x = nullptr; p.wd = (const float4*)wd; p.dscale = (const float4*)dscale; p.dshift = (const float4*)dshift;
+    p.wsplit = (const float*)wsplit; p.descale = descale; p.pshift = pshift; p.y = y;
+    p.H = h; p.W = w; p.C4 = c / 4; p.KT = c / 32; p.OH = h; p.OW = w; p.Cout = cout; p.pad_t = 1; p.pad_l = 1;
+    p.a_scale = ldexpf(1.f, a_log2);
+    p.reverse = sweep_reverse();
+    p.nimg = n;
+    p.stamps = nullptr;
+#ifdef HSEFR_STEM_STAMPS
+    p.stamps = stamp_buffer(s);
+#endif
+    p.x0 = x0; p.w0split = (const float*)w0split; p.descale0 = descale0; p.shift0 = shift0; p.a_scale0 = ldexpf(1.f, a0_log2);
+    return launch_front(p, n, act, s);
+}
+
+}
diff --git a/hse_facerec_tf_amd/csrc/engine.hip b/hse_facerec_tf_amd/csrc/engine.hip
--- a/hse_facerec_tf_amd/csrc/engine.hip
+++ b/hse_facerec_tf_amd/csrc/engine.hip
@@ -288,9 +288,26 @@
                 return HSEFR_ERR_UNSUPPORTED;
         }
     }
+    auto unwritten_ok = [&](uint32_t i, const char* flag) -> int {
+        const hsefr_plan_op &o = ops[i], &b = ops[i + 1];
+        HSEFR_REQUIRE(b.out_buf != o.out_buf, HSEFR_ERR_INVALID, "plan op %u: %s: the second output (buffer %d) aliases the first op's tensor", i, flag,
+                      b.out_buf);
+        HSEFR_REQUIRE(b.out_buf != o.in_buf || (uint64_t)bufs[o.in_buf].elems_per_image * bufs[o.in_buf].elem_bytes ==
+                                                   (uint64_t)bufs[o.out_buf].elems_per_image * bufs[o.out_buf].elem_bytes,
+                      HSEFR_ERR_INVALID, "plan op %u: %s: buffers %d and %d exchange roles and must have one size", i, flag, o.in_buf, o.out_buf);
+        for (uint32_t k = i + 2; k < h.n_ops; ++k) {
+            HSEFR_REQUIRE(ops[k].in_buf != o.out_buf && ops[k].res_buf != o.out_buf, HSEFR_ERR_INVALID,
+                          "plan op %u: %s: op %u also reads the first op's tensor (buffer %d)", i, flag, k, o.out_buf);
+            if (ops[k].out_buf == o.out_buf) break;
+        }
+        for (int sl = 0; sl < HSEFR_N_OUTPUT_SLOTS; ++sl)
+            HSEFR_REQUIRE(h.out_buffer[sl] != o.out_buf && (b.out_buf != o.in_buf || h.out_buffer[sl] != o.in_buf), HSEFR_ERR_INVALID,
+                          "plan op %u: %s: the first op's tensor (or the buffer it exchanges roles with) is output slot %d", i, flag, sl);
+        return HSEFR_OK;
+    };
     for (uint32_t i = 0; i < h.n_ops; ++i) {
         const hsefr_plan_op& o = ops[i];
-        HSEFR_REQUIRE((o.flags & ~(HSEFR_OPF_PAIR_NEXT | HSEFR_OPF_HEADS | HSEFR_OPF_OUT_SUB2 | HSEFR_OPF_DWPW_NEXT)) == 0, HSEFR_ERR_INVALID,
+        HSEFR_REQUIRE((o.flags & ~(HSEFR_OPF_PAIR_NEXT | HSEFR_OPF_HEADS | HSEFR_OPF_OUT_SUB2 | HSEFR_OPF_DWPW_NEXT | HSEFR_OPF_PWDW_NEXT)) == 0, HSEFR_ERR_INVALID,
                       "plan op %u: unknown flags 0x%x", i, o.flags);
         HSEFR_REQUIRE(!(o.flags & HSEFR_OPF_OUT_SUB2) || (o.flags & HSEFR_OPF_PAIR_NEXT), HSEFR_ERR_INVALID, "plan op %u: OUT_SUB2 without PAIR_NEXT", i);
         if (o.flags & HSEFR_OPF_PAIR_NEXT) {
@@ -323,19 +340,20 @@
                           "pointwise op without flags that reads it at the same pixels (a_log2 in [1, 12])", i);
             HSEFR_REQUIRE(dwpw_s2_covered(o.cin, b.cout, o.stride), HSEFR_ERR_INVALID, "plan op %u: DWPW_NEXT %d -> %d channels not covered (128 -> 256)", i,
                           o.cin, b.cout);
-            HSEFR_REQUIRE(b.out_buf != o.out_buf, HSEFR_ERR_INVALID, "plan op %u: DWPW_NEXT: the second output (buffer %d) aliases the depthwise tensor", i,
-                          b.out_buf);
-            HSEFR_REQUIRE(b.out_buf != o.in_buf || (uint64_t)bufs[o.in_buf].elems_per_image * bufs[o.in_buf].elem_bytes ==
-                                                       (uint64_t)bufs[o.out_buf].elems_per_image * bufs[o.out_buf].elem_bytes,
-                          HSEFR_ERR_INVALID, "plan op %u: DWPW_NEXT: buffers %d and %d exchange roles and must have one size", i, o.in_buf, o.out_buf);
-            for (uint32_t k = i + 2; k < h.n_ops; ++k) {
-                HSEFR_REQUIRE(ops[k].in_buf != o.out_buf && ops[k].res_buf != o.out_buf, HSEFR_ERR_INVALID,
-                              "plan op %u: DWPW_NEXT: op %u also reads the depthwise tensor (buffer %d)", i, k, o.out_buf);
-                if (ops[k].out_buf == o.out_buf) break;
-            }
-            for (int sl = 0; sl < HSEFR_N_OUTPUT_SLOTS; ++sl)
-                HSEFR_REQUIRE(h.out_buffer[sl] != o.out_buf && (b.out_buf != o.in_buf || h.out_buffer[sl] != o.in_buf), HSEFR_ERR_INVALID,
-                              "plan op %u: DWPW_NEXT: the depthwise tensor (or the buffer it exchanges roles with) is output slot %d", i, sl);
+            if (const int rc = unwritten_ok(i, "DWPW_NEXT")) return rc;
+        }
+        if (o.flags & HSEFR_OPF_PWDW_NEXT) {
+            HSEFR_REQUIRE(o.flags == HSEFR_OPF_PWDW_NEXT && i + 1 < h.n_ops, HSEFR_ERR_INVALID, "plan op %u: PWDW_NEXT on the last op or beside another flag", i);
+            const hsefr_plan_op& b = ops[i + 1];
+            HSEFR_REQUIRE(o.kind == HSEFR_OP_PWCONV_F16S && o.act == HSEFR_ACT_RELU6 && o.aux > 0 && o.aux <= 12 && o.res_buf == HSEFR_BUF_NONE &&
+                              o.oh == o.h && o.ow == o.w && b.kind == HSEFR_OP_DWPW_F16S && b.in_buf == o.out_buf && b.flags == 0 &&
+                              b.res_buf == HSEFR_BUF_NONE && b.h == o.h && b.w == o.w && b.oh == b.h && b.ow == b.w && b.stride == 1 && b.pad_t == 1 &&
+                              b.pad_l == 1 && b.cin == o.cout && b.act == HSEFR_ACT_RELU6 && b.aux > 0 && b.aux <= 12,
+                          HSEFR_ERR_INVALID, "plan op %u: PWDW_NEXT needs a split-f16 pointwise op with ReLU6 and no residual (a_log2 in [1, 12]), and behind it "
+                          "a stride-1 split-f16 block op with ReLU6, without flags, that reads it at the same pixels", i);
+            HSEFR_REQUIRE(pwdwpw_covered(o.cin, o.cout, b.cout, b.stride), HSEFR_ERR_INVALID,
+                          "plan op %u: PWDW_NEXT %d -> %d -> %d channels not covered (64 -> 128 -> 128)", i, o.cin, o.cout, b.cout);
+            if (const int rc = unwritten_ok(i, "PWDW_NEXT")) return rc;
         }
         if (o.flags & HSEFR_OPF_HEADS) {
             HSEFR_REQUIRE(i + 3 < h.n_ops, HSEFR_ERR_INVALID, "plan op %u: HEADS needs three ops behind it", i);
@@ -498,6 +516,8 @@
     if (!strcmp(key, "sweep_alternate")) { g_sweep_alternate = value; return HSEFR_OK; }
     if (!strcmp(key, "clock_mode")) { set_clock_mode(value); return HSEFR_OK; }
     if (!strcmp(key, "dwpw_s2_off")) { set_dwpw_s2_off(value); return HSEFR_OK; }
+    if (!strcmp(key, "pwdwpw_off")) { set_pwdwpw_off(value); return HSEFR_OK; }
+    if (!strcmp(key, "pwdwpw_min_items")) { set_pwdwpw_min_items(value); return HSEFR_OK; }
     if (!strcmp(key, "dwpws_tw")) { set_dwpws_tw(value); return HSEFR_OK; }
     if (!strcmp(key, "dwpws_bn")) { set_dwpws_bn(value); return HSEFR_OK; }
     if (!strcmp(key, "pw_ablate")) { set_pw_ablate(value); return HSEFR_OK; }
@@ -667,9 +687,20 @@
     return HSEFR_OK;
 }
 
+
+static bool pwdw_one_launch(const hsefr_engine* e, size_t i, int n) {
+    const hsefr_plan_op& o = e->ops[i];
+    return (o.flags & HSEFR_OPF_PWDW_NEXT) && !pwdwpw_off() && pwdwpw_launchable(n, o.h, o.w, o.cin, o.cout, e->ops[i + 1].cout) &&
+           pwdwpw_worth(n, o.h, o.w);
+}
+
 static int run_ops(hsefr_engine* e, const std::vector<void*>& tab_in, const void* d_input, int n, const std::vector<char>& needed,
                    hipStream_t s, hipEvent_t* pev, bool input_u8 = false, bool every_tensor = false) {
     std::vector<void*> tab(tab_in);
+    auto exchanged_out = [&](const hsefr_plan_op& o, const hsefr_plan_op& b) {
+        if (b.out_buf == o.in_buf) std::swap(tab[o.in_buf], tab[o.out_buf]);
+        return tab[b.out_buf];
+    };
     const bool prof = pev != nullptr;
     unsigned launches = 0;
     if (prof) HSEFR_HIP_CHECK(hipEventRecord(pev[0], s));
@@ -709,11 +740,19 @@
             covered = 3;
         } else if ((o.flags & HSEFR_OPF_DWPW_NEXT) && !every_tensor && !dwpw_s2_off() && needed[i + 1]) {
             const hsefr_plan_op& b = e->ops[i + 1];
-            if (b.out_buf == o.in_buf) std::swap(tab[o.in_buf], tab[o.out_buf]);
+            float* dst = (float*)exchanged_out(o, b);
             rc = launch_dwpw_f16s((const float*)in, (const float*)blob_ptr(e, o.w_off), (const float*)blob_ptr(e, o.scale_off),
                                   (const float*)blob_ptr(e, o.shift_off), blob_ptr(e, b.w_off), (const float*)blob_ptr(e, b.scale_off),
-                                  (const float*)blob_ptr(e, b.shift_off), (float*)tab[b.out_buf], n, o.h, o.w, o.cin, o.stride, o.pad_t, o.pad_l,
+                                  (const float*)blob_ptr(e, b.shift_off), dst, n, o.h, o.w, o.cin, o.stride, o.pad_t, o.pad_l,
                                   o.oh, o.ow, b.cout, b.aux, b.act, s);
+            covered = 1;
+        } else if ((o.flags & HSEFR_OPF_PWDW_NEXT) && !every_tensor && needed[i + 1] && pwdw_one_launch(e, i, n)) {
+            const hsefr_plan_op& b = e->ops[i + 1];
+            const float* ds2 = (const float*)blob_ptr(e, b.shift2_off);
+            float* dst = (float*)exchanged_out(o, b);
+            rc = launch_pwdwpw_f16s((const float*)in, blob_ptr(e, o.w_off), (const float*)blob_ptr(e, o.scale_off), (const float*)blob_ptr(e, o.shift_off),
+                                    (const float*)blob_ptr(e, b.w_off), (const float*)blob_ptr(e, b.scale_off), (const float*)blob_ptr(e, b.shift_off),
+                                    blob_ptr(e, b.w2_off), ds2, ds2 + b.cout, dst, n, o.h, o.w, o.cin, o.cout, b.cout, o.aux, b.aux, b.act, s);
             covered = 1;
         } else
         switch (o.kind) {
@@ -1003,6 +1042,7 @@
         const size_t span = (e.ops[i].flags & HSEFR_OPF_PAIR_NEXT)                      ? 1
                             : (e.ops[i].flags & HSEFR_OPF_HEADS)                        ? 3
                             : ((e.ops[i].flags & HSEFR_OPF_DWPW_NEXT) && !dwpw_s2_off()) ? 1
+                            : (i + 1 < e.ops.size() && pwdw_one_launch(&e, i, n))         ? 1
                                                                                         : 0;
         for (size_t k = 1; k <= span && i + k < e.ops.size(); ++k) only[i + k] = 1;
         std::string line = std::to_string(i) + "\t" + std::to_string(e.ops[i].kind) + "\t";
@@ -1184,6 +1224,15 @@
                             a_log2, act, (hipStream_t)stream);
 }
 
+int hsefr_pwdwpw_f16split(const float* x, const void* w0_split, const float* descale0, const float* shift0, const float* wd, const float* dscale,
+                          const float* dshift, const void* w_split, const float* descale, const float* pshift, float* y, int n, int h, int w,
+                          int c0, int c, int cout, int a0_log2, int a_log2, int act, hsefr_stream_t stream) {
+    HSEFR_REQUIRE(n == 0 || (x && w0_split && descale0 && shift0 && wd && dscale && dshift && w_split && descale && pshift && y), HSEFR_ERR_INVALID,
+                  "pwdwpw_f16split: null pointer");
+    return launch_pwdwpw_f16s(x, w0_split, descale0, shift0, wd, dscale, dshift, w_split, descale, pshift, y, n, h, w, c0, c, cout, a0_log2,
+                              a_log2, act, (hipStream_t)stream);
+}
+
 int hsefr_dwpw_fused(const float* x, const float* wd, const float* dscale, const float* dshift, const float* wp_t,
                      const float* pshift, float* y, int n, int h, int w, int c, int stride, int pad_t, int pad_l, int oh,
                      int ow, int cout, hsefr_stream_t stream) {
diff --git a/hse_facerec_tf_amd/csrc/fuzz_plan.cc b/hse_facerec_tf_amd/csrc/fuzz_plan.cc
--- a/hse_facerec_tf_amd/csrc/fuzz_plan.cc
+++ b/hse_facerec_tf_amd/csrc/fuzz_plan.cc
@@ -44,7 +44,7 @@
 int main(int argc, char** argv) {
     if (argc < 3) { fprintf(stderr, "usage: fuzz_plan <mutants per seed> <plan file>...\n"); return 2; }
     const long long per_seed = atoll(argv[1]);
-    static const int32_t edge32[] = {0, 1, -1, -2, -3, 2, 3, 7, 8, 63, 64, 65, 127, 128, 255, 256, 511, 512, 4095, 4096, 65535, 65536, 0x7fffffff,
+    static const int32_t edge32[] = {0, 1, -1, -2, -3, 2, 3, 7, 8, 16, 63, 64, 65, 127, 128, 255, 256, 511, 512, 4095, 4096, 65535, 65536, 0x7fffffff,
                                      (int32_t)0x80000000, (int32_t)0xffff0000, 1 << 20, 1 << 24, 1 << 30};
     static const uint64_t edge64[] = {0ull, 1ull, 15ull, 16ull, 17ull, 0xffffffffull, 0x100000000ull, 0x7fffffffffffffffull, 0x8000000000000000ull,
                                       0xffffffffffffffffull, 0xfffffffffffffff0ull};
diff --git a/hse_facerec_tf_amd/lowering.py b/hse_facerec_tf_amd/lowering.py
--- a/hse_facerec_tf_amd/lowering.py
+++ b/hse_facerec_tf_amd/lowering.py
@@ -30,7 +30,7 @@
 _HEADER = struct.Struct("<QIIIIII3i3IQ")
 _BUFFER = struct.Struct("<QII")
 _OP = struct.Struct("<II3i3i3i3i2iii5Q")
-OPF_PAIR_NEXT, OPF_HEADS, OPF_OUT_SUB2, OPF_DWPW_NEXT = 1, 2, 4, 8
+OPF_PAIR_NEXT, OPF_HEADS, OPF_OUT_SUB2, OPF_DWPW_NEXT, OPF_PWDW_NEXT = 1, 2, 4, 8, 16
 AUX_C2_SHIFT, AUX_C2_BITS, AUX_STRIDE2_SHIFT, AUX_STRIDE2_BITS = 0, 12, 12, 2
 AUX_H2_SHIFT, AUX_H2_BITS, AUX_W2_SHIFT, AUX_W2_BITS = 14, 9, 23, 9
 AUX_LOG2_BITS, AUX_OUT_LOG2_SHIFT, AUX_IN_LOG2_SHIFT, AUX_IN_LOG2_BIAS, AUX_U8_BIT = 8, 8, 8, 64, 16
@@ -46,7 +46,7 @@
 PRODUCT_KERNEL_FAMILIES = frozenset({
     "stem5_stream_kernel", "stem4_fused_kernel", "stem3_fused_kernel", "stem2_fused_kernel", "conv3x3_c3_kernel", "conv3x3_c3_mfma_kernel",
     "dwconv3x3_kernel", "pwconv_f32_dma_kernel", "pwconv_f32_kernel", "pwconv_f16s_kernel", "pwconv_ps_kernel", "dwpw_fused_kernel",
-    "dwpw_f16s_kernel", "dwpw2_f16s_kernel", "dwpw3_f16s_kernel", "dwpws2_f16s_kernel", "gap_kernel", "dense_kernel", "softmax_kernel", "heads_kernel",
+    "dwpw_f16s_kernel", "dwpw2_f16s_kernel", "dwpw3_f16s_kernel", "dwpws2_f16s_kernel", "pwdwpw_f16s_kernel", "gap_kernel", "dense_kernel", "softmax_kernel", "heads_kernel",
     "stem7s_stream_kernel", "stem7x7_pool_bf16_kernel", "stem7x7_bf16_kernel", "maxpool3x3s2_bf16_kernel", "conv_bf16_kernel", "conv1x1_bf16_kernel",
     "conv1x1_w4_bf16_kernel", "conv1x1_pair_bf16_kernel", "conv3x3_w2_bf16_kernel", "conv_dma_bf16_kernel", "gap_bf16_kernel",
     "conv_f32_mfma_kernel", "conv2d_f32_kernel", "maxpool_f32_kernel"})
@@ -777,7 +777,7 @@
             if last_use[j] == i and j not in pinned and layers[j].out_buf not in free:
                 free.append(layers[j].out_buf)
     for i, L in enumerate(layers):
-        if L.flags & OPF_DWPW_NEXT and L.src >= 0 and i + 1 < len(layers) and layers[i + 1].out_buf == layers[L.src].out_buf:
+        if L.flags & (OPF_DWPW_NEXT | OPF_PWDW_NEXT) and L.src >= 0 and i + 1 < len(layers) and layers[i + 1].out_buf == layers[L.src].out_buf:
             a, b = layers[L.src].out_buf, L.out_buf
             buffers[a] = buffers[b] = max(buffers[a], buffers[b])
     return buffers
@@ -1063,6 +1063,27 @@
     return n
 
 
+def pwdw_pair_covered(pw: Layer, blk: Layer) -> bool:
+    return blk.stride == 1 and pw.in_shape[2] == 64 and pw.out_shape[2] == 128 and blk.out_shape[2] == 128
+
+
+def mark_pwdw_pairs(layers: List[Layer], keep: Sequence[int]) -> int:
+    consumers = consumers_of(layers)
+    n = 0
+    for i, pw in enumerate(layers):
+        j = sole_reader(consumers, i, keep)
+        if not (pw.kind == OP_PWCONV_F32 and 0 < pw.a_log2 <= 12 and pw.act == ACT_RELU6 and not pw.in_split and pw.out_split == 0 and
+                pw.flags == 0 and pw.res < 0 and j == i + 1):
+            continue
+        blk = layers[j]
+        if (blk.kind == OP_DWPW_F16S and blk.act == ACT_RELU6 and 0 < blk.a_log2 <= 12 and blk.flags == 0 and blk.res < 0 and
+                (blk.pad_t, blk.pad_l) == (1, 1) and tuple(blk.in_shape) == tuple(pw.out_shape) and
+                tuple(blk.out_shape[:2]) == tuple(blk.in_shape[:2]) and pwdw_pair_covered(pw, blk)):
+            pw.flags |= OPF_PWDW_NEXT
+            n += 1
+    return n
+
+
 def choose_pointwise_math(layers: List[Layer], pw_math: str) -> None:
     if pw_math not in ("auto", "f32", "f16split"):
         raise ValueError("pw_math must be 'auto', 'f32' or 'f16split', not %r" % (pw_math,))
@@ -1143,7 +1164,7 @@
                 pw_math: Optional[str] = None, fuse_stem_block: Optional[bool] = None, stem_fusion: Optional[str] = None,
                 block_fusion: Optional[str] = None, presplit: Optional[str] = None, input_bound: Optional[float] = None,
                 pwdw_fusion: Optional[str] = None, u8_mean_bgr: Optional[Sequence[float]] = None, launch_fusion: bool = True,
-                s2_fusion: Optional[str] = None) -> Plan:
+                s2_fusion: Optional[str] = None, front_fusion: Optional[str] = None) -> Plan:
     if dtype not in ("f32", "bf16", "f32g"):
         raise ValueError("dtype must be 'f32', 'bf16' or 'f32g', not %r" % (dtype,))
     in_node, _ = g.get_tensor_by_name(input_tensor)
@@ -1264,5 +1285,10 @@
         raise ValueError("s2_fusion must be 'auto' or 'none', not %r" % (s2_fusion,))
     if fuse and launch_fusion and dtype == "f32" and s2_fusion == "auto":
         mark_dwpw_pairs(layers, keep())
+    front_fusion = front_fusion or "auto"
+    if front_fusion not in ("auto", "none"):
+        raise ValueError("front_fusion must be 'auto' or 'none', not %r" % (front_fusion,))
+    if fuse and launch_fusion and dtype == "f32" and front_fusion == "auto":
+        mark_pwdw_pairs(layers, keep())
     buffers = assign_buffers(layers, set(keep()))
     return Plan(layers, (input_hw[0], input_hw[1], low.in_c), buffers, out_layers, tensor_layer)
diff --git a/hse_facerec_tf_amd/ops.py b/hse_facerec_tf_amd/ops.py
--- a/hse_facerec_tf_amd/ops.py
+++ b/hse_facerec_tf_amd/ops.py
@@ -196,6 +196,24 @@
     _lib.check(_lib.lib().hsefr_dwpw_f16split(x.data_ptr(), w_hwc.data_ptr(), dscale.data_ptr(), dshift.data_ptr(), d_img.data_ptr(),
                                               d_ds.data_ptr(), pshift.data_ptr(), y.data_ptr(), n, h, w, c, stride, pt, pl, oh, ow,
                                               cout, a_log2, act, _lib.current_stream_ptr()), "hsefr_dwpw_f16split")
+    return y
+
+
+@_device_guarded
+def pwdwpw_f16split(x, w0_t, shift0, w_hwc, dscale, dshift, wp_t, pshift, act: int = ACT_RELU6, a0_log2: int = 12, a_log2: int = 12,
+                    prepared0=None, prepared=None):
+    torch = _lib.require_gpu()
+    for t, nm in ((x, "x"), (shift0, "shift0"), (w_hwc, "w"), (dscale, "dscale"), (dshift, "dshift"), (pshift, "pshift")):
+        _f32c(t, nm)
+    d_img0, d_ds0 = prepared0 if prepared0 is not None else split_weights_device(w0_t, x.device, a0_log2)
+    d_img, d_ds = prepared if prepared is not None else split_weights_device(wp_t, x.device, a_log2)
+    n, h, w, c0 = x.shape
+    c, cout = d_img0.shape[0], d_img.shape[0]
+    y = torch.empty((n, h, w, cout), dtype=torch.float32, device=x.device)
+    _lib.check(_lib.lib().hsefr_pwdwpw_f16split(x.data_ptr(), d_img0.data_ptr(), d_ds0.data_ptr(), shift0.data_ptr(), w_hwc.data_ptr(),
+                                                dscale.data_ptr(), dshift.data_ptr(), d_img.data_ptr(), d_ds.data_ptr(), pshift.data_ptr(),
+                                                y.data_ptr(), n, h, w, c0, c, cout, a0_log2, a_log2, act, _lib.current_stream_ptr()),
+               "hsefr_pwdwpw_f16split")
     return y
 
 
diff --git a/include/hsefr.h b/include/hsefr.h
--- a/include/hsefr.h
+++ b/include/hsefr.h
@@ -89,7 +89,8 @@
     HSEFR_OPF_PAIR_NEXT = 1,
     HSEFR_OPF_HEADS = 2,
     HSEFR_OPF_OUT_SUB2 = 4,
-    HSEFR_OPF_DWPW_NEXT = 8
+    HSEFR_OPF_DWPW_NEXT = 8,
+    HSEFR_OPF_PWDW_NEXT = 16
 } hsefr_op_flags;
 
 enum {
@@ -210,6 +211,10 @@
                         const float* descale, const float* pshift, float* y, int n, int h, int w, int c, int stride,
                         int pad_t, int pad_l, int oh, int ow, int cout, int a_log2, int act, hsefr_stream_t stream);
 
+int hsefr_pwdwpw_f16split(const float* x, const void* w0_split, const float* descale0, const float* shift0, const float* wd, const float* dscale,
+                          const float* dshift, const void* w_split, const float* descale, const float* pshift, float* y, int n, int h, int w,
+                          int c0, int c, int cout, int a0_log2, int a_log2, int act, hsefr_stream_t stream);
+
 int hsefr_stem2_fused(const float* x, const float* conv_w, const float* conv_shift, const float* wd1, const float* d1scale,
                       const float* d1shift, const void* w_split, const float* descale, const float* pshift, const float* wd2,
                       const float* d2scale, const float* d2shift, float* y, int n, int h, int w, int cpad_t, int cpad_l,
```

Measured after the change: 263,400, median of 6. +3.4%, better.
